# jeuneS2/csolve

Measured on AMD Instinct MI355X. Metric: constraint propagations/sec + nodes/sec, queens-N, 1/2/4/8 MI355X, higher is better.
Workload: dtype int32

## Files before the change

csolve_amd/_lib.py:

```python
from __future__ import annotations

import ctypes as C
import os
import re

_HERE = os.path.dirname(os.path.abspath(__file__))
LIB_PATH = os.environ.get("CSOLVE_HIP_LIB") or os.path.join(_HERE, "libcsolve_hip.so")
HEADER_PATH = os.path.join(os.path.dirname(_HERE), "include", "csolve_gpu.h")


class CsolveError(RuntimeError):
    def __init__(self, code: int, message: str):
        super().__init__(f"csolve_gpu error {code}: {message}")
        self.code = code


class Val(C.Structure):
    _fields_ = [("lo", C.c_int32), ("hi", C.c_int32)]


class Node(C.Structure):
    _fields_ = [("var", C.c_int32), ("lo", C.c_int32), ("hi", C.c_int32), ("parent", C.c_int32)]


class SearchStats(C.Structure):
    _fields_ = [("nodes", C.c_uint64), ("cuts", C.c_uint64), ("props", C.c_uint64), ("revisions", C.c_uint64),
                ("solutions", C.c_uint64), ("iterations", C.c_uint64), ("restarts", C.c_uint64), ("pool", C.c_int64), ("pool_peak", C.c_int64),
                ("best", C.c_int32), ("done", C.c_int32)]


SHARD_SOLUTION_FN = C.CFUNCTYPE(None, C.c_void_p, C.c_int, C.POINTER(C.c_int32), C.c_int64, C.c_int32)


class ShardOptions(C.Structure):
    _fields_ = [("slice_iterations", C.c_int64), ("poll_iterations", C.c_int64), ("seed_states_per_rank", C.c_int64),
                ("low_water", C.c_int64), ("time_limit", C.c_double), ("on_solution", SHARD_SOLUTION_FN),
                ("user", C.c_void_p)]


class Result(C.Structure):
    _fields_ = [("status", C.c_int32), ("props", C.c_int32), ("revisions", C.c_int32), ("rounds", C.c_int32)]


MANY_DONE, MANY_LIMIT, MANY_BAD_ROOT = 0, 1, 2


class ManyResult(C.Structure):
    _fields_ = [("status", C.c_int32), ("root_props", C.c_int32), ("nodes", C.c_int64), ("cuts", C.c_int64),
                ("props", C.c_int64), ("solutions", C.c_int64)]


class ManyOptions(C.Structure):
    _fields_ = [("objective", C.c_int32), ("reserved", C.c_int32), ("max_nodes", C.c_int64)]


def declared_symbols(header: str = HEADER_PATH):
    text = re.sub(r"/\*.*?\*/", "", open(header).read(), flags=re.S)
    return sorted(set(re.findall(r"\b(csgpu_\w+)\s*\(", text)))


PLAN_FAMILIES = ("events", "traced", "rounds", "lds", "bitset", "regs0", "regs1", "regs2", "regs3", "packed",
                 "shave", "shave_trace", "server", "step_shave", "step_packed", "step_import")

_lib = None
_demangler = None


def demangle(symbol: str) -> str:
    global _demangler
    if _demangler is None:
        cxx = C.CDLL("libstdc++.so.6")
        cxx.__cxa_demangle.argtypes = [C.c_char_p, C.c_void_p, C.c_void_p, C.POINTER(C.c_int)]
        cxx.__cxa_demangle.restype = C.c_void_p
        libc = C.CDLL(None)
        libc.free.argtypes = [C.c_void_p]
        _demangler = (cxx.__cxa_demangle, libc.free)
    fn, free = _demangler
    status = C.c_int()
    p = fn(symbol.encode(), None, None, C.byref(status))
    if status.value != 0 or not p:
        raise ValueError(f"cannot demangle {symbol!r}")
    try:
        text = C.string_at(p).decode()
    finally:
        free(p)
    if text.startswith("void "):
        text = text[5:]
    depth = 0
    for i, ch in enumerate(text):
        depth += ch == "<"
        depth -= ch == ">"
        if ch == "(" and depth == 0:
            return text[:i]
    return text


def load_library():
    global _lib
    if _lib is not None:
        return _lib
    if not os.path.exists(LIB_PATH):
        raise ImportError(
            f"{LIB_PATH} is missing: build it with `python -c 'import __graft_entry__ as g; g.build()'` "
            "or `make -C csolve_amd/csrc` (hipcc --offload-arch=gfx950). There is no CPU fallback.")
    try:
        import torch
    except ImportError:
        pass
    L = C.CDLL(LIB_PATH)
    vp, i32, i64 = C.c_void_p, C.c_int32, C.c_int64
    L.csgpu_last_error.restype = C.c_char_p
    L.csgpu_device_count.restype = C.c_int
    L.csgpu_set_device.argtypes = [C.c_int]
    L.csgpu_model_from_text.argtypes = [C.c_char_p, C.c_int, C.POINTER(vp)]
    L.csgpu_model_from_file.argtypes = [C.c_char_p, C.c_int, C.POINTER(vp)]
    L.csgpu_model_from_dump.argtypes = [C.c_char_p, C.POINTER(vp)]
    L.csgpu_model_free.argtypes = [vp]
    L.csgpu_model_free.restype = None
    for f in ("csgpu_model_num_vars", "csgpu_model_num_clauses", "csgpu_model_objective",
              "csgpu_model_objective_var"):
        getattr(L, f).argtypes = [vp]
    L.csgpu_model_var_name.argtypes = [vp, C.c_int]
    L.csgpu_model_var_name.restype = C.c_char_p
    L.csgpu_model_get_domains.argtypes = [vp, vp]
    L.csgpu_model_set_domains.argtypes = [vp, vp]
    L.csgpu_model_device_info.argtypes = [vp, C.POINTER(i64)]
    L.csgpu_model_root_propagate.argtypes = [vp, C.POINTER(i32)]
    L.csgpu_model_finalize.argtypes = [vp]
    L.csgpu_model_normalize.argtypes = [vp]
    L.csgpu_model_specialize.argtypes = [vp, vp, C.POINTER(vp)]
    L.csgpu_model_build_tables.argtypes = [vp]
    L.csgpu_model_eval_clauses_host.argtypes = [vp, vp]
    L.csgpu_model_set_kernel.argtypes = [vp, C.c_int]
    L.csgpu_model_qualifies.argtypes = [vp, C.c_int]
    L.csgpu_set_linear_fast_paths.argtypes = [C.c_int]
    L.csgpu_sets_pack.argtypes = [vp, vp, vp, i64, vp]
    L.csgpu_sets_unpack.argtypes = [vp, vp, vp, i64, vp]
    L.csgpu_propagate_batch_sets.argtypes = [vp, vp, vp, vp, vp, i64, vp]
    L.csgpu_set_linear_fast_paths.restype = None
    L.csgpu_model_get_kernel.argtypes = [vp]
    L.csgpu_propagate_batch.argtypes = [vp, vp, vp, vp, vp, i64, vp]
    L.csgpu_propagate_batch_obj.argtypes = [vp, vp, vp, vp, vp, i64, i32, i32, vp]
    L.csgpu_model_forbidden_words.argtypes = [vp]
    L.csgpu_propagate_batch_fb.argtypes = [vp, vp, vp, vp, vp, vp, vp, i64, vp]
    L.csgpu_eval_batch.argtypes = [vp, vp, vp, i64, vp]
    L.csgpu_eval_clauses.argtypes = [vp, vp, vp, vp]
    L.csgpu_search_create.argtypes = [vp, i64, i64, C.POINTER(vp)]
    L.csgpu_search_free.argtypes = [vp]
    L.csgpu_search_free.restype = None
    L.csgpu_search_reset.argtypes = [vp]
    L.csgpu_search_put.argtypes = [vp, vp, i64]
    L.csgpu_search_put_host.argtypes = [vp, vp, i64]
    L.csgpu_search_take.argtypes = [vp, vp, i64, C.POINTER(i64)]
    L.csgpu_search_take_host.argtypes = [vp, vp, i64, C.POINTER(i64)]
    L.csgpu_plan_transfers.argtypes = [vp, C.c_int, i64, i64, vp, C.POINTER(C.c_int)]
    L.csgpu_shard_region_size.argtypes = [C.c_int, C.c_int, i64, C.POINTER(C.c_size_t)]
    L.csgpu_shard_region_init.argtypes = [vp, C.c_size_t, C.c_int, C.c_int, i64]
    L.csgpu_shard_barrier.argtypes = [vp]
    L.csgpu_text_num_vars.argtypes = [C.c_char_p, C.c_int, C.POINTER(C.c_int)]
    L.csgpu_shard_default_options.argtypes = [C.POINTER(ShardOptions)]
    L.csgpu_shard_default_options.restype = None
    L.csgpu_shard_run.argtypes = [vp, vp, C.c_int, vp, C.POINTER(ShardOptions), C.POINTER(SearchStats),
                                  C.POINTER(SearchStats)]
    L.csgpu_search_set_best.argtypes = [vp, i32]
    L.csgpu_model_add_conflict.argtypes = [vp, i32, vp, vp]
    L.csgpu_search_put_cost.argtypes = [vp, C.POINTER(C.c_double), C.POINTER(i64)]
    L.csgpu_objective_better.argtypes = [C.c_int, Val, i32]
    L.csgpu_objective_bound.argtypes = [C.c_int, Val, i32]
    L.csgpu_objective_bound.restype = Val
    L.csgpu_objective_best.argtypes = [C.c_int, Val, i32]
    L.csgpu_objective_best.restype = i32
    L.csgpu_luby_next.argtypes = [C.POINTER(C.c_uint64), C.POINTER(C.c_uint64)]
    L.csgpu_luby_next.restype = None
    L.csgpu_step_check.argtypes = [Val, C.c_uint32]
    L.csgpu_step_val.argtypes = [Val, C.c_uint32, C.c_uint32]
    L.csgpu_step_val.restype = i32
    L.csgpu_search_share_incumbent.argtypes = [vp, vp]
    L.csgpu_search_set_parents.argtypes = [vp, i64]
    L.csgpu_search_set_restart.argtypes = [vp, i64]
    L.csgpu_search_run.argtypes = [vp, i64, C.POINTER(SearchStats)]
    L.csgpu_search_solutions.argtypes = [vp, vp, i64]
    L.csgpu_search_best_solution.argtypes = [vp, vp]
    L.csgpu_search_solutions.restype = i64
    L.csgpu_search_set_solution_stream.argtypes = [vp, i64]
    L.csgpu_search_drain_solutions.argtypes = [vp, vp, i64, C.POINTER(i64)]
    L.csgpu_search_drain_solutions_device.argtypes = [vp, vp, i64, C.POINTER(i64), vp]
    L.csgpu_search_pending_solutions.argtypes = [vp, C.POINTER(i64), C.POINTER(i64)]
    L.csgpu_propagate_one.argtypes = [vp, vp, Node, vp, C.POINTER(Result)]
    L.csgpu_propagate_one_traced.argtypes = [vp, vp, Node, vp, C.POINTER(Result), vp, i32, C.POINTER(i32)]
    L.csgpu_propagate_one_causes.argtypes = [vp, vp, Node, vp, C.POINTER(Result), vp, i32, C.POINTER(i32)]
    L.csgpu_propagate_values.argtypes = [vp, vp, i32, vp, i32, vp, vp]
    L.csgpu_model_root_propagate_limit.argtypes = [vp, i64, C.POINTER(i32), C.POINTER(i32)]
    L.csgpu_propagate_one_chain.argtypes = [vp, vp, Node, C.POINTER(i32), C.POINTER(i32), vp, i32, C.POINTER(i32)]
    L.csgpu_search_set_strategy.argtypes = [vp, C.c_int, C.c_int]
    L.csgpu_search_set_restart_on_improvement.argtypes = [vp, C.c_int]
    L.csgpu_internal_plan_symbol.argtypes = [vp, C.c_int, C.c_char_p, C.c_size_t]
    L.csgpu_solve_many.argtypes = [vp, vp, i64, C.POINTER(ManyOptions), vp, vp, vp]
    L.csgpu_internal_many_symbol.argtypes = [vp, C.c_char_p, C.c_size_t]
    L.csgpu_internal_many_waves.argtypes = [vp, i64]
    L.csgpu_internal_many_waves.restype = i64
    L.csgpu_debug_one_timing.argtypes = [vp, C.POINTER(C.c_double), C.POINTER(C.c_uint64), C.POINTER(C.c_uint64)]
    _lib = L
    return L


def check(rc: int):
    if rc < 0:
        raise CsolveError(rc, load_library().csgpu_last_error().decode())
    return rc
```

csolve_amd/csrc/cs_capi.hip:

```cpp
#include <hip/hip_runtime.h>
#include <chrono>

#include <dlfcn.h>
#include <stdarg.h>
#include <stdio.h>
#include <stdlib.h>
#include <string.h>

#include <mutex>

#include "../../include/csolve_gpu.h"
#include "cs_kernels.hip.h"
#include "cs_shave.hip.h"
#include "cs_step.hip.h"
#include "cs_dive.hip.h"
#include "cs_chain.hip.h"
#include "cs_internal.h"

static thread_local char g_err[512] = "";

static int set_err(int code, const char *fmt, ...) {
  va_list ap;
  va_start(ap, fmt);
  vsnprintf(g_err, sizeof g_err, fmt, ap);
  va_end(ap);
  return code;
}

extern "C" int csgpu_internal_set_error(int code, const char *msg) { return set_err(code, "%s", msg); }

#define HIP_TRY(expr)                                                          \
  do {                                                                         \
    hipError_t e_ = (expr);                                                    \
    if (e_ != hipSuccess)                                                      \
      return set_err(CSGPU_E_HIP, "%s: %s", #expr, hipGetErrorString(e_));     \
  } while (0)

#define CS_TICKET_SLOTS 1024
#define CS_TICKET_STREAMS 64
#define CS_TICKET_SLOT_WORDS (CS_SHAVE_SHARDS * CS_SHAVE_TICKET_STRIDE)

#define CS_CU_LDS (160u * 1024u)

struct cs_planned {
  const void *fn;
  size_t lds;
  int waves;
  int per_cu;
};

struct cs_kernel_plan {
  cs_planned events, traced;
  cs_planned rounds;
  int rounds_cpl;
  cs_planned lds;
  cs_planned bitset;
  cs_planned regs[4];
  cs_planned packed;
  int packed_nodes;
  cs_planned shave, shave_trace;
  cs_planned server;
  cs_planned step_shave, step_packed, step_import;
  cs_planned dive;
  int full;
  int step_kind;
  int max_width;
};

struct csgpu_model {
  cs_model *host;
  int from_dump;
  int not_root;
  int finalized;
  cs_dev_image *img;
  int *d_adj_off, *d_adj, *d_clause, *d_tree_off, *d_tnode, *d_tkid, *d_tree_want, *d_lit, *d_clause_by_kind;
  cs_tables tab;
  size_t slice;
  int has_tree_adj;
  int packed_bias;
  int packed_nw;
  int kernel_choice;
  cs_kernel_plan plan;
  void *d_adj_packed;
  int lds_adj_global;
  int k2_csz;
  int shave_static;
  int step_chunk_max;
  size_t k1_tab_bytes;
  int fb_words;
  size_t dense_bytes;
  void *d_dense_tab;
  void *d_packed_tab;
  int *d_root_lo;
  int *d_root_hi;
  void *d_many_stack;
  int64_t many_stack_waves;
  unsigned *d_many_tickets;
  int *d_sym_off;
  void *d_sym_packed;
  int n_cus;
  unsigned *d_tickets;
  int ticket_slots, ticket_streams, ticket_reserved;
  void *ticket_stream[CS_TICKET_STREAMS];
  unsigned char *h_one;
  int *d_adj_clause;
  int32_t *h_trace;
  unsigned *h_trace_n;
  int trace_cap;
  cs_val *d_one_in, *d_one_out;
  cs_node_in *d_one_node;
  cs_node_out *d_one_res;
  int engines;
  int chain_state;
  cs_chain_clause *d_chain_cl;
  int *d_chain_off, *d_chain_list;
  cs_chain_frame *d_chain_frames;
  int *h_chain_out;
  unsigned char *h_box;
  size_t box_state_off, box_out_off, box_trace_off;
  hipStream_t srv_stream;
  unsigned srv_seq;
  int srv_off, srv_launched;
  double srv_seconds[4];
  uint64_t srv_calls, srv_starts;
  unsigned char *h_values, *d_values;
  size_t values_cap;
};

extern "C" const char *csgpu_last_error(void) { return g_err; }

static int wait_null_stream(void) {
  for (;;) {
    const hipError_t e = hipStreamQuery(NULL);
    if (e == hipSuccess) return CSGPU_OK;
    if (e != hipErrorNotReady) return set_err(CSGPU_E_HIP, "hipStreamQuery: %s", hipGetErrorString(e));
  }
}

extern "C" int csgpu_device_count(void) {
  int n = 0;
  hipError_t e = hipGetDeviceCount(&n);
  if (e != hipSuccess) return set_err(CSGPU_E_HIP, "hipGetDeviceCount: %s", hipGetErrorString(e));
  return n;
}

extern "C" int csgpu_set_device(int device) {
  HIP_TRY(hipSetDevice(device));
  return CSGPU_OK;
}


static int objective_sense(int objective) { return objective == CS_OBJ_MIN ? 1 : (objective == CS_OBJ_MAX ? 2 : 0); }

extern "C" int csgpu_objective_better(int objective, csgpu_val value, int32_t best) {
  return cs_objective_better(objective_sense(objective), cs_interval(value.lo, value.hi), best);
}
extern "C" csgpu_val csgpu_objective_bound(int objective, csgpu_val value, int32_t best) {
  const cs_val v = cs_objective_bound(objective_sense(objective), cs_interval(value.lo, value.hi), best);
  csgpu_val out;
  out.lo = v.lo;
  out.hi = v.hi;
  return out;
}
extern "C" int32_t csgpu_objective_best(int objective, csgpu_val value, int32_t best) {
  return cs_objective_best(objective_sense(objective), cs_interval(value.lo, value.hi), best);
}
extern "C" void csgpu_luby_next(uint64_t *threshold, uint64_t *counter) {
  if (threshold != NULL && counter != NULL) cs_luby_next(threshold, counter);
}
extern "C" int csgpu_step_check(csgpu_val bounds, uint32_t iter) {
  return cs_step_check(cs_interval(bounds.lo, bounds.hi), iter);
}
extern "C" uint64_t csgpu_branch_key(int order, int prefer_failing, csgpu_val value, int64_t prio, int32_t index) {
  return cs_branch_key_of(order, prefer_failing, cs_interval(value.lo, value.hi), prio, index);
}
extern "C" int32_t csgpu_step_val(csgpu_val bounds, uint32_t iter, uint32_t seed) {
  return cs_step_val(cs_interval(bounds.lo, bounds.hi), iter, seed);
}


static int wrap_model(cs_model *host, int from_dump, csgpu_model **out) {
  csgpu_model *m = (csgpu_model *)calloc(1, sizeof *m);
  if (m == NULL) { cs_model_free(host); return set_err(CSGPU_E_ARG, "out of memory"); }
  m->host = host;
  m->from_dump = from_dump;
  *out = m;
  return CSGPU_OK;
}

extern "C" int csgpu_model_from_text(const char *text, int weights_on, csgpu_model **out) {
  if (text == NULL || out == NULL) return set_err(CSGPU_E_ARG, "null argument");
  char err[256];
  cs_model *host = cs_model_parse(text, weights_on, err, sizeof err);
  if (host == NULL) return set_err(CSGPU_E_PARSE, "%s", err);
  return wrap_model(host, 0, out);
}

extern "C" int csgpu_model_from_file(const char *path, int weights_on, csgpu_model **out) {
  if (path == NULL || out == NULL) return set_err(CSGPU_E_ARG, "null argument");
  FILE *f = fopen(path, "rb");
  if (f == NULL) return set_err(CSGPU_E_ARG, "%s: cannot open", path);
  fseek(f, 0, SEEK_END);
  long len = ftell(f);
  fseek(f, 0, SEEK_SET);
  char *text = (char *)malloc((size_t)len + 1);
  size_t got = fread(text, 1, (size_t)len, f);
  fclose(f);
  text[got] = '\0';
  int rc = csgpu_model_from_text(text, weights_on, out);
  free(text);
  return rc;
}

extern "C" int csgpu_model_from_dump(const char *path, csgpu_model **out) {
  if (path == NULL || out == NULL) return set_err(CSGPU_E_ARG, "null argument");
  char err[256];
  cs_model *host = cs_model_load(path, err, sizeof err);
  if (host == NULL) return set_err(CSGPU_E_ARG, "%s", err);
  if (host->clause_node == NULL) {
    cs_model_free(host);
    return set_err(CSGPU_E_ARG, "%s: model file has no clause index", path);
  }
  return wrap_model(host, 1, out);
}

extern "C" int csgpu_model_from_host(cs_model *host, int lists_final, int domains_are_root, csgpu_model **out) {
  if (host == NULL || out == NULL) return set_err(CSGPU_E_ARG, "null argument");
  int rc = wrap_model(host, lists_final, out);
  if (rc == CSGPU_OK) (*out)->not_root = !domains_are_root;
  return rc;
}

extern "C" cs_model *csgpu_model_host(csgpu_model *m) { return m ? m->host : NULL; }

static void server_stop(csgpu_model *m);
static void server_reap(csgpu_model *m);
static csgpu_model *g_srv_models[16];
static void quiesce_servers(void) {
  for (int i = 0; i < 16; i++)
    if (g_srv_models[i] != NULL) server_stop(g_srv_models[i]);
}

static void free_device(csgpu_model *m) {
  (void)hipFree(m->d_chain_cl); (void)hipFree(m->d_chain_off); (void)hipFree(m->d_chain_list); (void)hipFree(m->d_chain_frames);
  if (m->h_chain_out != NULL) (void)hipHostFree(m->h_chain_out);
  m->d_chain_cl = NULL; m->d_chain_off = NULL; m->d_chain_list = NULL; m->d_chain_frames = NULL; m->h_chain_out = NULL;
  m->chain_state = 0;
  quiesce_servers();
  for (int i = 0; i < 16; i++)
    if (g_srv_models[i] == m) g_srv_models[i] = NULL;
  if (m->h_box != NULL) (void)hipHostFree(m->h_box);
  m->h_box = NULL;
  if (m->srv_stream != NULL) (void)hipStreamDestroy(m->srv_stream);
  m->srv_stream = NULL;
  m->srv_off = 0;
  (void)hipFree(m->d_adj_off); (void)hipFree(m->d_adj); (void)hipFree(m->d_clause); (void)hipFree(m->d_clause_by_kind);
  (void)hipFree(m->d_tree_off); (void)hipFree(m->d_tnode); (void)hipFree(m->d_tkid); (void)hipFree(m->d_tree_want);
  (void)hipFree(m->d_lit);
  m->d_tree_want = NULL;
  m->d_lit = NULL;
  (void)hipFree(m->d_adj_packed);
  (void)hipFree(m->d_root_lo);
  (void)hipFree(m->d_root_hi);
  (void)hipFree(m->d_many_stack);
  (void)hipFree(m->d_many_tickets);
  m->d_root_hi = NULL;
  m->d_many_stack = NULL;
  m->d_many_tickets = NULL;
  m->many_stack_waves = 0;
  (void)hipFree(m->d_sym_off);
  (void)hipFree(m->d_sym_packed);
  (void)hipFree(m->d_dense_tab);
  (void)hipFree(m->d_packed_tab);
  m->d_packed_tab = NULL;
  (void)hipFree(m->d_tickets);
  m->d_tickets = NULL;
  m->ticket_slots = m->ticket_streams = m->ticket_reserved = 0;
  m->d_sym_off = NULL;
  m->d_sym_packed = NULL;
  m->d_dense_tab = NULL;
  m->d_adj_packed = NULL;
  m->d_root_lo = NULL;
  memset(&m->plan, 0, sizeof m->plan);
  m->fb_words = 0;
  (void)hipHostFree(m->h_one);
  m->h_one = NULL;
  (void)hipFree(m->d_adj_clause);
  m->d_adj_clause = NULL;
  if (m->h_trace != NULL) (void)hipHostFree(m->h_trace);
  m->h_trace = NULL;
  m->h_trace_n = NULL;
  m->trace_cap = 0;
  if (m->h_values != NULL) (void)hipHostFree(m->h_values);
  m->h_values = m->d_values = NULL;
  m->values_cap = 0;
  m->d_adj_off = m->d_adj = m->d_clause = m->d_tree_off = m->d_tnode = m->d_tkid = m->d_clause_by_kind = NULL;
  m->d_one_in = m->d_one_out = NULL;
  m->d_one_node = NULL;
  m->d_one_res = NULL;
  cs_dev_image_free(m->img);
  m->img = NULL;
}

extern "C" void csgpu_model_free(csgpu_model *m) {
  if (m == NULL) return;
  free_device(m);
  cs_model_free(m->host);
  free(m);
}

extern "C" int csgpu_model_num_vars(const csgpu_model *m) { return m ? m->host->n_vars : CSGPU_E_ARG; }
extern "C" int csgpu_model_num_clauses(const csgpu_model *m) {
  if (m == NULL) return CSGPU_E_ARG;
  if (m->host->clause_node == NULL && m->host->root >= 0 && cs_model_index(m->host) != 0) return CSGPU_E_ARG;
  return m->host->n_clauses;
}
extern "C" int csgpu_model_objective(const csgpu_model *m) { return m ? m->host->objective : CSGPU_E_ARG; }
extern "C" int csgpu_model_objective_var(const csgpu_model *m) { return m ? m->host->obj_var : CSGPU_E_ARG; }

extern "C" const char *csgpu_model_var_name(const csgpu_model *m, int var) {
  if (m == NULL || var < 0 || var >= m->host->n_vars) return NULL;
  return m->host->names[var];
}

extern "C" int csgpu_model_get_domains(const csgpu_model *m, csgpu_val *out) {
  if (m == NULL || out == NULL) return set_err(CSGPU_E_ARG, "null argument");
  memcpy(out, m->host->dom, (size_t)m->host->n_vars * sizeof(cs_val));
  return CSGPU_OK;
}

extern "C" int csgpu_model_set_domains(csgpu_model *m, const csgpu_val *in) {
  if (m == NULL || in == NULL) return set_err(CSGPU_E_ARG, "null argument");
  memcpy(m->host->dom, in, (size_t)m->host->n_vars * sizeof(cs_val));
  return CSGPU_OK;
}

extern "C" void csgpu_set_linear_fast_paths(int on) { cs_dev_linear_fast_paths = on != 0; }

extern "C" int csgpu_model_device_info(const csgpu_model *m, int64_t info[8]) {
  if (m == NULL || info == NULL) return set_err(CSGPU_E_ARG, "null argument");
  if (m->img == NULL) return set_err(CSGPU_E_STATE, "device tables are not built");
  info[0] = m->img->n_adj;
  info[1] = m->img->n_ne;
  info[2] = m->img->n_tree_clauses;
  info[3] = m->img->n_tnodes;
  info[4] = (int64_t)m->slice;
  info[5] = m->img->max_list;
  info[6] = m->img->n_skip;
  info[7] = m->img->max_tree;
  return CSGPU_OK;
}


struct dev_tables_owner {
  int *adj_off, *adj, *clause, *tree_off, *tnode, *tkid, *tree_want, *lit, *clause_by_kind;
};

static int upload(const void *src, size_t bytes, int **dst) {
  HIP_TRY(hipMalloc((void **)dst, bytes ? bytes : 16));
  if (bytes) HIP_TRY(hipMemcpy(*dst, src, bytes, hipMemcpyHostToDevice));
  return CSGPU_OK;
}

static int upload_image(const cs_dev_image *g, dev_tables_owner *o, cs_tables *t) {
  int rc;
  memset(o, 0, sizeof *o);
  if ((rc = upload(g->adj_off, ((size_t)g->n_vars + 1) * 4, &o->adj_off))) return rc;
  if ((rc = upload(g->adj, (size_t)(g->n_adj ? g->n_adj : 1) * 8, &o->adj))) return rc;
  if ((rc = upload(g->clause, (size_t)(g->n_clauses ? g->n_clauses : 1) * 16, &o->clause))) return rc;
  {
    const int32_t nc = g->n_clauses;
    int32_t *sorted = (int32_t *)malloc((size_t)(nc ? nc : 1) * 16);
    if (sorted == NULL) return set_err(CSGPU_E_LIMIT, "out of memory");
    static const int order[] = { CS_CL_EQ, CS_CL_LT, CS_CL_NE, CS_CL_OR2, CS_CL_TREE, CS_CL_SKIP };
    int32_t k = 0;
    for (size_t q = 0; q < sizeof order / sizeof order[0]; q++)
      for (int32_t c = 0; c < nc; c++)
        if (g->clause[4 * c] == order[q]) { memcpy(sorted + 4 * k, g->clause + 4 * c, 16); k++; }
    rc = k == nc ? upload(sorted, (size_t)(nc ? nc : 1) * 16, &o->clause_by_kind) : set_err(CSGPU_E_STATE, "clause of unknown kind");
    free(sorted);
    if (rc) return rc;
  }
  if ((rc = upload(g->tree_off, ((size_t)g->n_trees + 1) * 4, &o->tree_off))) return rc;
  if ((rc = upload(g->tnode, (size_t)(g->n_tnodes ? g->n_tnodes : 1) * 16, &o->tnode))) return rc;
  if ((rc = upload(g->tkid, (size_t)(g->n_tkids ? g->n_tkids : 1) * 4, &o->tkid))) return rc;
  if ((rc = upload(g->tree_want, (size_t)(g->n_trees ? g->n_trees : 1) * 8, &o->tree_want))) return rc;
  if ((rc = upload(g->lit, (size_t)(g->n_lits ? g->n_lits : 1) * 16, &o->lit))) return rc;
  t->n_vars = g->n_vars;
  t->n_clauses = g->n_clauses;
  t->n_words = (g->n_vars + 31) / 32;
  t->adj_off = o->adj_off;
  t->adj = (const int2 *)o->adj;
  t->clause = (const int4 *)o->clause;
  t->clause_by_kind = (const int4 *)o->clause_by_kind;
  t->tree_off = o->tree_off;
  t->tnode = (const int4 *)o->tnode;
  t->tkid = o->tkid;
  t->tree_want = (const int2 *)o->tree_want;
  t->lit = (const int4 *)o->lit;
  t->n_lits = g->n_lits;
  t->obj_var = -1;
  t->obj_lo = CS_DOM_MIN;
  t->obj_hi = CS_DOM_MAX;
  t->obj_best_dev = NULL;
  t->obj_sense = 0;
  return CSGPU_OK;
}

static void free_tables(dev_tables_owner *o) {
  (void)hipFree(o->adj_off); (void)hipFree(o->adj); (void)hipFree(o->clause); (void)hipFree(o->clause_by_kind);
  (void)hipFree(o->tree_off); (void)hipFree(o->tnode); (void)hipFree(o->tkid); (void)hipFree(o->tree_want);
  (void)hipFree(o->lit);
}

static int lds_limit(size_t bytes, const void *func) {
  if (bytes > CS_CU_LDS) return set_err(CSGPU_E_LIMIT, "%zu bytes of LDS per workgroup exceed the 160 KiB of a CU", bytes);
  if (bytes > 48u * 1024u)
    HIP_TRY(hipFuncSetAttribute(func, hipFuncAttributeMaxDynamicSharedMemorySize, (int)bytes));
  return CSGPU_OK;
}


extern "C" int csgpu_model_root_propagate(csgpu_model *m, int32_t *status) {
  return csgpu_model_root_propagate_limit(m, -1, status, NULL);
}

extern "C" int csgpu_model_root_propagate_limit(csgpu_model *m, int64_t limit, int32_t *status, int32_t *rounds) {
  if (m == NULL || status == NULL) return set_err(CSGPU_E_ARG, "null argument");
  quiesce_servers();
  cs_model *h = m->host;
  if (h->root < 0) return set_err(CSGPU_E_STATE, "model has no root");
  if (!m->from_dump && cs_model_index(h) != 0) return set_err(CSGPU_E_ARG, "%s", h->err);
  char err[200];
  cs_dev_image *g = cs_dev_image_build(h, 0, NULL, err, sizeof err);
  if (g == NULL) return set_err(CSGPU_E_LIMIT, "%s", err);

  dev_tables_owner own;
  cs_tables tab;
  int rc = upload_image(g, &own, &tab);
  cs_val *d_in = NULL, *d_out = NULL;
  cs_node_out *d_res = NULL;
  int *d_conv = NULL, conv = 1;
  cs_node_out res;
  const size_t nbytes = (size_t)(h->n_vars ? h->n_vars : 1) * sizeof(cs_val);
  const size_t lds = (size_t)h->n_vars * sizeof(cs_val) + 4 * sizeof(unsigned);
  hipError_t e = hipSuccess;
  if (rc == CSGPU_OK) rc = lds_limit(lds, (const void *)cs_propagate_sweeps);
  if (rc == CSGPU_OK) {
    if ((e = hipMalloc((void **)&d_in, nbytes)) != hipSuccess || (e = hipMalloc((void **)&d_out, nbytes)) != hipSuccess ||
        (e = hipMalloc((void **)&d_res, sizeof res)) != hipSuccess || (e = hipMalloc((void **)&d_conv, sizeof(int))) != hipSuccess ||
        (e = hipMemcpy(d_in, h->dom, (size_t)h->n_vars * sizeof(cs_val), hipMemcpyHostToDevice)) != hipSuccess)
      rc = set_err(CSGPU_E_HIP, "root propagate setup: %s", hipGetErrorString(e));
  }
  if (rc == CSGPU_OK) {
    const int max_rounds = limit < 0 || limit >= 0x7ffffffe ? 0x7fffffff : (int)limit + 1;
    hipLaunchKernelGGL(cs_propagate_sweeps, dim3(1), dim3(CS_BLOCK), lds, 0, tab, d_in, d_out, d_res, max_rounds, 0, d_conv);
    if ((e = hipGetLastError()) != hipSuccess || (e = hipDeviceSynchronize()) != hipSuccess ||
        (e = hipMemcpy(&res, d_res, sizeof res, hipMemcpyDeviceToHost)) != hipSuccess ||
        (e = hipMemcpy(&conv, d_conv, sizeof conv, hipMemcpyDeviceToHost)) != hipSuccess)
      rc = set_err(CSGPU_E_HIP, "root propagate: %s", hipGetErrorString(e));
    if (rc == CSGPU_OK && res.status >= 0 && !conv) {
      hipLaunchKernelGGL(cs_propagate_sweeps, dim3(1), dim3(CS_BLOCK), lds, 0, tab, d_in, d_out, d_res, max_rounds, 1, d_conv);
      if ((e = hipGetLastError()) != hipSuccess || (e = hipDeviceSynchronize()) != hipSuccess ||
          (e = hipMemcpy(&res, d_res, sizeof res, hipMemcpyDeviceToHost)) != hipSuccess)
        rc = set_err(CSGPU_E_HIP, "root propagate (sequential sweeps): %s", hipGetErrorString(e));
    }
    if (rc == CSGPU_OK && (e = hipMemcpy(h->dom, d_out, (size_t)h->n_vars * sizeof(cs_val), hipMemcpyDeviceToHost)) != hipSuccess)
      rc = set_err(CSGPU_E_HIP, "root propagate: %s", hipGetErrorString(e));
    if (rc != CSGPU_OK) {  }
    else {
      *status = res.status < 0 ? -1 : res.props;
      if (rounds != NULL) *rounds = res.rounds;
    }
  }
  (void)hipFree(d_in); (void)hipFree(d_out); (void)hipFree(d_res); (void)hipFree(d_conv);
  free_tables(&own);
  cs_dev_image_free(g);
  return rc;
}

extern "C" int csgpu_model_normalize(csgpu_model *m) {
  if (m == NULL) return set_err(CSGPU_E_ARG, "null argument");
  if (m->from_dump) return set_err(CSGPU_E_STATE, "a dumped model is already normalised");
  if (m->finalized) return set_err(CSGPU_E_STATE, "model is already finalized");
  if (cs_model_normalize(m->host) < 0) return set_err(CSGPU_E_STATE, "model has no root");
  return CSGPU_OK;
}

extern "C" int csgpu_model_specialize(const csgpu_model *m, const csgpu_val *state, csgpu_model **out) {
  if (m == NULL || state == NULL || out == NULL) return set_err(CSGPU_E_ARG, "null argument");
  const cs_model *h = m->host;
  if (h->root < 0) return set_err(CSGPU_E_STATE, "model has no root");
  for (int32_t v = 0; v < h->n_vars; v++) {
    if (state[v].lo > state[v].hi) return set_err(CSGPU_E_ARG, "variable %d: empty interval", v);
    if (state[v].lo < h->dom[v].lo || state[v].hi > h->dom[v].hi)
      return set_err(CSGPU_E_ARG, "variable %d: [%d, %d] is not inside the model's [%d, %d]", v, state[v].lo, state[v].hi,
                     h->dom[v].lo, h->dom[v].hi);
  }
  cs_model *copy = cs_model_clone(h);
  if (copy == NULL) return set_err(CSGPU_E_LIMIT, "out of memory");
  memcpy(copy->dom, state, (size_t)h->n_vars * sizeof(cs_val));
  return wrap_model(copy, 0, out);
// ... 341 lines not shown
    if (m->img->adj[2 * i] < 0 && m->img->adj[2 * i + 1] == 0) { m->has_tree_adj = 1; break; }
  const size_t tb = ((((size_t)h->n_vars + 1) * 4 + 15) & ~(size_t)15) + (((size_t)m->img->n_adj * 8 + 15) & ~(size_t)15) +
                    (((size_t)m->img->n_lits * 16 + 15) & ~(size_t)15);
  m->k1_tab_bytes = (tb <= 32u * 1024u && m->img->n_adj > 0) ? tb : 0;
  const void *k1 = m->has_tree_adj ? (m->k1_tab_bytes ? (const void *)cs_propagate_events<true, true>
                                                      : (const void *)cs_propagate_events<true, false>)
                                   : (m->k1_tab_bytes ? (const void *)cs_propagate_events<false, true>
                                                      : (const void *)cs_propagate_events<false, false>);
  int rc;
  if ((rc = plan_kernel(&m->plan.events, k1, m->slice * CS_WAVES_PER_BLOCK + m->k1_tab_bytes, CS_WAVES_PER_BLOCK)))
    return rc;
  if (m->plan.events.per_cu < 1) m->plan.events.per_cu = 1;
  if ((rc = lds_limit((size_t)h->n_vars * sizeof(cs_val) + 16, (const void *)cs_eval_root))) return rc;
  if ((rc = lds_limit((size_t)h->n_vars * sizeof(cs_val) + 16, (const void *)cs_eval_clauses))) return rc;
  if ((rc = plan_kernel(&m->plan.traced, (const void *)cs_propagate_events<true, false, true>, m->slice * CS_WAVES_PER_BLOCK,
                        CS_WAVES_PER_BLOCK)))
    return rc;
  const int per = (m->img->n_clauses + CS_WAVE - 1) / CS_WAVE;
  m->plan.rounds_cpl = m->img->n_clauses <= 0 || per > 8 ? 0 : (per <= 1 ? 1 : (per <= 2 ? 2 : (per <= 4 ? 4 : 8)));
  if (m->plan.rounds_cpl) {
#define CS_PICK6(CPL)                                                                              \
  m->plan.rounds.fn = m->has_tree_adj ? (const void *)cs_propagate_clause_rounds<CPL, true>         \
                                      : (const void *)cs_propagate_clause_rounds<CPL, false>
    switch (m->plan.rounds_cpl) {
    case 1: CS_PICK6(1); break;
    case 2: CS_PICK6(2); break;
    case 4: CS_PICK6(4); break;
    default: CS_PICK6(8); break;
    }
#undef CS_PICK6
    m->plan.rounds.lds = ((((size_t)h->n_vars * sizeof(cs_val) + 16 + 15) & ~(size_t)15)) * CS_WAVES_PER_BLOCK;
    m->plan.rounds.waves = CS_WAVES_PER_BLOCK;
    m->plan.rounds.per_cu = 8;
  }
  m->plan.max_width = 2;
  for (int32_t v = 0; v < h->n_vars; v++) {
    const int64_t w = (int64_t)h->dom[v].hi - (int64_t)h->dom[v].lo + 1;
    if (w > m->plan.max_width) m->plan.max_width = w > 0x7fffffff ? 0x7fffffff : (int)w;
  }
  return CSGPU_OK;
}

static int plan_lds_resident(csgpu_model *m) {
  const cs_model *h = m->host;
  if (m->img->packed_width == 0) return CSGPU_OK;
  const size_t off_bytes = (((size_t)h->n_vars * 2 * sizeof(int)) + 15) & ~(size_t)15;
  const size_t adj_bytes = (((size_t)m->img->n_adj * (size_t)m->img->packed_width) + 15) & ~(size_t)15;
  const size_t lds_slice = ((size_t)h->n_vars * sizeof(cs_val) + (2 * (size_t)m->tab.n_words + 1) * sizeof(unsigned) + 15) & ~(size_t)15;
  m->lds_adj_global = 0;
  int waves_max = 16, waves = 0;
  size_t bytes = 0;
  { const char *e = getenv("CSGPU_K2_WAVES"); if (e != NULL && atoi(e) >= 4 && atoi(e) <= 16) waves_max = atoi(e); }
  for (int w = waves_max; w >= 4; w--) {
    const size_t need = off_bytes + adj_bytes + (size_t)w * lds_slice;
    if (need <= CS_CU_LDS) {
      waves = w;
      bytes = need;
      break;
    }
  }
  const char *force = getenv("CSGPU_K2_ADJ");
  const int want_global = force != NULL && force[0] == 'g';
  if (want_global && 8 * lds_slice <= CS_CU_LDS) {
    m->lds_adj_global = 1;
    waves = 8;
    bytes = 8 * lds_slice;
  }
  { const char *e = getenv("CSGPU_K2_CSZ"); m->k2_csz = e != NULL && atoi(e) >= 1 && atoi(e) <= CS_CHUNK ? atoi(e) : 0; }
  if (!waves) return CSGPU_OK;
  int rc;
  if ((rc = upload(m->img->adj_packed, (size_t)m->img->n_adj * (size_t)m->img->packed_width, (int **)&m->d_adj_packed)))
    return rc;
  if ((rc = plan_kernel(&m->plan.lds, ne_lds_kernel(m->img->packed_width, h->n_vars, m->lds_adj_global), bytes, waves)))
    return rc;
  if (m->plan.lds.per_cu < 1) m->plan.lds.per_cu = 1;
  return CSGPU_OK;
}

static int plan_forbidden_sets(csgpu_model *m) {
  const cs_model *h = m->host;
  if (m->img->sym_width == 0 || m->not_root) return CSGPU_OK;
  int64_t width = 1;
  for (int32_t v = 0; v < h->n_vars; v++) {
    const int64_t w = (int64_t)h->dom[v].hi - (int64_t)h->dom[v].lo + 1;
    if (w > width) width = w;
  }
  const int fw = width <= 64 ? 1 : (width <= 128 ? 2 : (width <= 256 ? 4 : 0));
  if (!fw) return CSGPU_OK;
  const size_t off_bytes = (((size_t)h->n_vars * 2 * sizeof(int)) + 15) & ~(size_t)15;
  const size_t base_bytes = (((size_t)h->n_vars * sizeof(int)) + 15) & ~(size_t)15;
  const size_t adj_bytes = (((size_t)m->img->sym_n_adj * (size_t)m->img->sym_width) + 15) & ~(size_t)15;
  const size_t sl = ((size_t)h->n_vars * sizeof(cs_val) + (size_t)h->n_vars * fw * 8 +
                     (2 * (size_t)m->tab.n_words + 2) * sizeof(unsigned) + 15) & ~(size_t)15;
  int waves = 16;
  for (; waves >= 1; waves--)
    if (off_bytes + base_bytes + adj_bytes + (size_t)waves * sl <= CS_CU_LDS) break;
  if (waves < 1) return CSGPU_OK;
  m->fb_words = fw;
  int *lo = (int *)malloc((size_t)(h->n_vars ? h->n_vars : 1) * sizeof(int));
  for (int32_t v = 0; v < h->n_vars; v++) lo[v] = h->dom[v].lo;
  int rc = upload(lo, (size_t)h->n_vars * sizeof(int), &m->d_root_lo);
  free(lo);
  if (rc) return rc;
  if ((rc = upload(m->img->sym_off, ((size_t)h->n_vars + 1) * sizeof(int), &m->d_sym_off))) return rc;
  if ((rc = upload(m->img->sym_packed, (size_t)m->img->sym_n_adj * (size_t)m->img->sym_width, (int **)&m->d_sym_packed)))
    return rc;
  if ((rc = plan_kernel(&m->plan.bitset, ne_bitset_kernel(m->img->sym_width, fw, h->n_vars),
                        off_bytes + base_bytes + adj_bytes + (size_t)waves * sl, waves)))
    return rc;
  if (m->plan.bitset.per_cu < 1) m->plan.bitset.per_cu = 1;
  return CSGPU_OK;
}

static int plan_dense_table(csgpu_model *m) {
  const cs_model *h = m->host;
  if (!m->fb_words || m->img->dense_width == 0) return CSGPU_OK;
  const int n = h->n_vars, width = m->img->dense_width, slots = m->img->dense_slots;
  const size_t bytes = (size_t)n * slots * m->img->dense_cols * width;
  int best = 0, waves = 0;
  for (int w = 4; w <= 16; w <<= 1)
    if (resident_per_cu(bytes, w) * w > best) { best = resident_per_cu(bytes, w) * w; waves = w; }
  if (!waves) return CSGPU_OK;
  m->dense_bytes = bytes;
  int rc;
  if ((rc = upload(m->img->dense_tab, bytes, (int **)&m->d_dense_tab))) return rc;
  for (int variant = 0; variant < 4; variant++)
    if ((rc = plan_kernel(&m->plan.regs[variant], ne_regs_kernel(width, m->fb_words, n, variant & 1, variant >> 1), bytes, waves)))
      return rc;
  m->plan.full = n == cs_dense_strides(n) * CS_WAVE;
  if ((rc = plan_kernel(&m->plan.shave, ne_shave_kernel(width, n, slots, m->plan.full), bytes, waves))) return rc;
  const size_t table = (bytes + 15) & ~(size_t)15;
  if (table + (size_t)waves * 32 <= CS_CU_LDS &&
      (rc = plan_kernel(&m->plan.step_shave, step_shave_kernel(width, n, slots, m->plan.full), table + (size_t)waves * 32, waves)))
    return rc;
  if (table + CS_SHAVE_TRACE_LDS * 16 <= CS_CU_LDS) {
    if ((rc = plan_kernel(&m->plan.shave_trace, ne_shave_trace_kernel(width, n, slots), table + CS_SHAVE_TRACE_LDS * 16, waves)))
      return rc;
    m->plan.server = m->plan.shave_trace;
    m->plan.server.fn = shave_server_kernel(width, n, slots);
  }
  if ((rc = plan_kernel(&m->plan.dive, dive_kernel(width, n), table, waves))) return rc;
  {
    int *hi = (int *)malloc((size_t)n * sizeof(int));
    if (hi == NULL) return set_err(CSGPU_E_ARG, "out of memory");
    for (int32_t v = 0; v < n; v++) hi[v] = h->dom[v].hi;
    rc = upload(hi, (size_t)n * sizeof(int), &m->d_root_hi);
    free(hi);
    if (rc) return rc;
  }
  HIP_TRY(hipMalloc((void **)&m->d_tickets, (size_t)CS_TICKET_SLOTS * CS_TICKET_SLOT_WORDS * sizeof(unsigned)));
  HIP_TRY(hipMemset(m->d_tickets, 0, (size_t)CS_TICKET_SLOTS * CS_TICKET_SLOT_WORDS * sizeof(unsigned)));
  m->ticket_slots = CS_TICKET_SLOTS;
  m->shave_static = getenv("CSGPU_SHAVE_STATIC") != NULL;
  return CSGPU_OK;
}

static int plan_packed(csgpu_model *m) {
  const cs_model *h = m->host;
  if (m->plan.shave.fn == NULL) return CSGPU_OK;
  const int n = h->n_vars, s3 = m->img->dense_slots == 3;
  m->packed_nw = 1;
  for (int32_t v = 0; v < n; v++)
    if ((int64_t)h->dom[v].hi - (int64_t)h->dom[v].lo + 1 > 32) m->packed_nw = 2;
  m->packed_bias = 0;
  for (int32_t v = 0; v < n; v++)
    if (h->dom[v].lo - m->img->dense_dmin > m->packed_bias) m->packed_bias = h->dom[v].lo - m->img->dense_dmin;
  m->plan.packed_nodes = packed_nodes_per_wave(m->fb_words, n, m->img->dense_width);
  if (!m->plan.packed_nodes) return CSGPU_OK;
  const size_t bytes = m->dense_bytes;
  int rc;
  if ((rc = plan_kernel(&m->plan.packed, ne_packed_kernel(n, m->packed_nw, s3), 2 * bytes, m->plan.regs[0].waves))) return rc;
  m->plan.packed.per_cu = m->plan.regs[0].per_cu;
  const size_t per_row = (size_t)m->img->dense_slots * m->img->dense_cols, total = (size_t)n * per_row;
  uint16_t *rel = (uint16_t *)malloc(total * sizeof(uint16_t));
  const uint8_t *src = (const uint8_t *)m->img->dense_tab;
  for (size_t i = 0; i < total; i++) {
    const int32_t u = (int32_t)(i / per_row);
    rel[i] = src[i] == 0xffu ? (uint16_t)0xffffu : (uint16_t)((int)src[i] - (h->dom[u].lo - m->img->dense_dmin) + m->packed_bias);
  }
  rc = upload(rel, total * sizeof(uint16_t), (int **)&m->d_packed_tab);
  free(rel);
  if (rc) return rc;
  if (step_packed_lds(m, 16) <= 80u * 1024u &&
      ((rc = plan_kernel(&m->plan.step_packed, step_packed_kernel(n, m->packed_nw, s3), step_packed_lds(m, 16), 16)) ||
       (rc = plan_kernel(&m->plan.step_import, step_import_kernel(n, m->packed_nw, s3), (2 * bytes + 15) & ~(size_t)15, 4))))
    return rc;
  m->step_chunk_max = 128;
  { const char *e = getenv("CSGPU_STEP_CHUNK_MAX"); if (e != NULL && atoi(e) > 0) m->step_chunk_max = atoi(e); }
  return CSGPU_OK;
}

static int stage_single_node(csgpu_model *m) {
  int dev = 0;
  hipDeviceProp_t prop;
  HIP_TRY(hipGetDevice(&dev));
  HIP_TRY(hipGetDeviceProperties(&prop, dev));
  m->n_cus = prop.multiProcessorCount;
  const size_t nbytes = (size_t)(m->host->n_vars ? m->host->n_vars : 1) * sizeof(cs_val);
  const size_t part = (nbytes + 63) & ~(size_t)63;
  unsigned char *d = NULL;
  HIP_TRY(hipHostMalloc((void **)&m->h_one, 2 * part + 128, hipHostMallocMapped));
  HIP_TRY(hipHostGetDevicePointer((void **)&d, m->h_one, 0));
  m->d_one_in = (cs_val *)d;
  m->d_one_node = (cs_node_in *)(d + part);
  m->d_one_res = (cs_node_out *)(d + part + 64);
  m->d_one_out = (cs_val *)(d + part + 128);
  return CSGPU_OK;
}

extern "C" int csgpu_model_finalize(csgpu_model *m) {
  if (m == NULL) return set_err(CSGPU_E_ARG, "null argument");
  free_device(m);
  int rc;
  if ((rc = csgpu_model_build_tables(m)) || (rc = drop_entailed_clauses(m)) || (rc = plan_general(m)) ||
      (rc = plan_lds_resident(m)) || (rc = plan_forbidden_sets(m)) || (rc = plan_dense_table(m)) || (rc = plan_packed(m)) ||
      (rc = stage_single_node(m)))
    return rc;
  m->plan.step_kind = m->plan.step_packed.fn != NULL ? 1
                      : (m->plan.step_shave.fn != NULL && m->host->n_vars <= 256 && m->plan.max_width <= 256 ? 2 : 0);
  m->finalized = 1;
  return CSGPU_OK;
}

static int kernel_qualifies(const csgpu_model *m, int which) {
  if (!m->finalized) return 0;
  switch (which) {
  case 1: return 1;
  case 2: return m->plan.lds.fn != NULL;
  case 3: return m->plan.bitset.fn != NULL;
  case 4: return m->plan.regs[0].fn != NULL;
  case 5: return m->plan.packed.fn != NULL;
  case 6: return m->plan.rounds.fn != NULL;
  case 7: return m->plan.shave.fn != NULL;
  default: return 0;
  }
}

extern "C" int csgpu_model_set_kernel(csgpu_model *m, int which) {
  static const char *const kernel_name[8] = {
    NULL, NULL, "the LDS-resident kernel", "the forbidden-set kernel", "the register-resident forbidden-set kernel",
    "the several-nodes-per-wave kernel (at most 32 variables, 64 values)", "the clause-resident kernel (at most 512 clauses)",
    "the interval-only shaving kernel (dense pair table in LDS)" };
  if (m == NULL || which < 0 || which > 7) return set_err(CSGPU_E_ARG, "bad argument");
  if (which >= 2) {
    if (!m->finalized) return set_err(CSGPU_E_STATE, "model is not finalized");
    if (!kernel_qualifies(m, which)) return set_err(CSGPU_E_LIMIT, "model does not qualify for %s", kernel_name[which]);
  }
  m->kernel_choice = which;
  return CSGPU_OK;
}

extern "C" int csgpu_model_qualifies(const csgpu_model *m, int which) { return m != NULL && kernel_qualifies(m, which); }

extern "C" int csgpu_internal_plan_symbol(const csgpu_model *m, int family, char *buf, size_t len) {
  if (m == NULL || buf == NULL || len == 0) return set_err(CSGPU_E_ARG, "null argument");
  if (!m->finalized) return set_err(CSGPU_E_STATE, "model is not finalized");
  const cs_kernel_plan *p = &m->plan;
  const cs_planned *fam[] = { &p->events, &p->traced, &p->rounds, &p->lds, &p->bitset, &p->regs[0], &p->regs[1],
                              &p->regs[2], &p->regs[3], &p->packed, &p->shave, &p->shave_trace, &p->server,
                              &p->step_shave, &p->step_packed, &p->step_import };
  if (family < 0 || family >= (int)(sizeof fam / sizeof fam[0])) return set_err(CSGPU_E_ARG, "no plan family %d", family);
  buf[0] = '\0';
  const void *fn = fam[family]->fn;
  if (fn == NULL) return CSGPU_OK;
  Dl_info info;
  if (dladdr(fn, &info) == 0 || info.dli_sname == NULL || info.dli_saddr != fn)
    return set_err(CSGPU_E_STATE, "plan family %d: the kernel handle has no dynamic symbol", family);
  if (strlen(info.dli_sname) >= len) return set_err(CSGPU_E_LIMIT, "plan family %d: symbol longer than the buffer", family);
  strcpy(buf, info.dli_sname);
  return CSGPU_OK;
}

extern "C" int csgpu_internal_many_symbol(const csgpu_model *m, char *buf, size_t len) {
  if (m == NULL || buf == NULL || len == 0) return set_err(CSGPU_E_ARG, "null argument");
  if (!m->finalized) return set_err(CSGPU_E_STATE, "model is not finalized");
  buf[0] = '\0';
  const void *fn = m->plan.dive.fn;
  if (fn == NULL) return CSGPU_OK;
  Dl_info info;
  if (dladdr(fn, &info) == 0 || info.dli_sname == NULL || info.dli_saddr != fn)
    return set_err(CSGPU_E_STATE, "cs_dive_shave: the kernel handle has no dynamic symbol");
  if (strlen(info.dli_sname) >= len) return set_err(CSGPU_E_LIMIT, "cs_dive_shave: symbol longer than the buffer");
  strcpy(buf, info.dli_sname);
  return CSGPU_OK;
}

extern "C" void csgpu_internal_engine_ref(const csgpu_model *m, int delta) {
  if (m != NULL) const_cast<csgpu_model *>(m)->engines += delta;
}

extern "C" const int32_t *csgpu_internal_root_lo(const csgpu_model *m) {
  return m != NULL && m->finalized && m->fb_words ? m->d_root_lo : NULL;
}

extern "C" int csgpu_model_forbidden_words(const csgpu_model *m) { return m && m->finalized ? m->fb_words : 0; }

extern "C" int csgpu_internal_step_kind(const csgpu_model *m) { return m == NULL || !m->finalized ? 0 : m->plan.step_kind; }

static int64_t step_shave_waves(const csgpu_model *m, int64_t stage_rows) {
  const cs_planned *k = &m->plan.step_shave;
  int64_t waves = (int64_t)m->n_cus * (int64_t)k->per_cu * k->waves;
  const int64_t by_stage = stage_rows / (4 * (int64_t)m->plan.max_width);
  if (waves > by_stage) waves = by_stage / k->waves * k->waves;
  return waves;
}

// ... 67 lines not shown
  const int64_t by_stage = L->stage_rows / (2 * (int64_t)G * maxw);
  if (waves > by_stage) waves = by_stage;
  const int64_t by_parents = ((int64_t)L->parents + G - 1) / G;
  if (waves > by_parents) waves = by_parents;
  if (waves < 1) return set_err(CSGPU_E_LIMIT, "step kernel: staging buffer too small");
  int wg_waves = 16;
  while (wg_waves > waves) wg_waves >>= 1;
  const int64_t grid = waves / wg_waves;
  waves = grid * wg_waves;
  const int64_t K = L->stage_rows / waves;
  int64_t chunk = (int64_t)L->parents / (waves * 8);
  if (chunk > m->step_chunk_max) chunk = m->step_chunk_max;
  if (chunk * maxw > K / 2) chunk = K / (2 * maxw);
  chunk = chunk / G * G;
  if (chunk < G) chunk = G;
  cs_step_io io;
  io.pool = (const uint2 *)L->pool;
  io.first_row = (long long)L->first_row;
  io.parents = L->parents;
  io.chunk = (int)chunk;
  io.maxw = maxw;
  io.stage = (uint2 *)L->stage;
  io.K = (int)(K > 0x7fffffff ? 0x7fffffff : K);
  io.fill = L->fill;
  io.wstat = (unsigned long long *)L->wstat;
  io.ticket = L->ticket;
  io.solutions = L->solutions;
  io.stored = (unsigned long long *)L->stored;
  io.max_solutions = (long long)L->max_solutions;
  io.store_open = L->store_open;
  io.stream_on = L->stream != NULL;
  int nn = n, slots = m->img->dense_slots, bias = m->packed_bias;
  const void *tab_d = m->d_packed_tab;
  const int *root_lo_d = m->d_root_lo, *sym_off = m->d_sym_off;
  size_t tab_bytes = 2 * m->dense_bytes;
  void *args[] = { &nn, &tab_d, &slots, &root_lo_d, &sym_off, &bias, &tab_bytes, &io };
  HIP_TRY(hipLaunchKernel(m->plan.step_packed.fn, dim3((unsigned)grid), dim3((unsigned)(wg_waves * CS_WAVE)), args,
                          step_packed_lds(m, wg_waves), (hipStream_t)stream));
  hipLaunchKernelGGL(cs_collect, dim3((unsigned)waves), dim3(256), 0, (hipStream_t)stream, (const unsigned *)L->fill, (int)waves,
                     (const uint2 *)L->stage, io.K, n, (uint2 *)L->pool, (long long)L->first_row, (int)L->parents,
                     (int)chunk, (const unsigned *)L->ticket, (const unsigned long long *)L->wstat,
                     (unsigned long long *)L->out, (const unsigned long long *)L->stored,
                     L->stream, (long long)L->stream_base, (long long)L->stream_limit, (long long)L->stream_cap,
                     (unsigned long long *)L->stream_err);
  HIP_TRY(hipGetLastError());
  return CSGPU_OK;
}

extern "C" int csgpu_internal_step_import(const csgpu_model *m, csgpu_val *d_rows, int64_t first_row, int64_t count,
                                          void *stream) {
  const int kind = csgpu_internal_step_kind(m);
  if (kind == 2) return CSGPU_OK;
  if (kind != 1 || d_rows == NULL || count < 0) return set_err(CSGPU_E_ARG, "bad argument");
  if (count == 0) return CSGPU_OK;
  const cs_planned *k = &m->plan.step_import;
  const int n = m->host->n_vars, G = m->plan.packed_nodes;
  int nn = n, slots = m->img->dense_slots, bias = m->packed_bias;
  const void *tab_d = m->d_packed_tab;
  const int *root_lo_d = m->d_root_lo;
  size_t tab_bytes = 2 * m->dense_bytes;
  long long fr = first_row, cnt = count;
  int64_t grid = (count + (int64_t)G * k->waves - 1) / ((int64_t)G * k->waves);
  if (grid > (int64_t)m->n_cus * 8) grid = (int64_t)m->n_cus * 8;
  void *args[] = { &nn, &tab_d, &slots, &root_lo_d, &bias, &tab_bytes, &d_rows, &fr, &cnt };
  HIP_TRY(hipLaunchKernel(k->fn, dim3((unsigned)grid), dim3((unsigned)(k->waves * CS_WAVE)), args, k->lds, (hipStream_t)stream));
  return CSGPU_OK;
}

extern "C" int csgpu_internal_step_export(const csgpu_model *m, csgpu_val *d_rows, int64_t first_row, int64_t count,
                                          void *stream) {
  const int kind = csgpu_internal_step_kind(m);
  if (kind == 2) return CSGPU_OK;
  if (kind != 1 || d_rows == NULL || count < 0) return set_err(CSGPU_E_ARG, "bad argument");
  if (count == 0) return CSGPU_OK;
  const int n = m->host->n_vars;
  const long long elements = (long long)count * n;
  uint2 *rows = (uint2 *)d_rows + (size_t)first_row * n;
  const unsigned grid = (unsigned)((elements + 255) / 256);
  if (m->packed_nw == 1)
    hipLaunchKernelGGL(cs_step_export<1>, dim3(grid), dim3(256), 0, (hipStream_t)stream, n, (const int *)m->d_root_lo, rows, elements);
  else
    hipLaunchKernelGGL(cs_step_export<2>, dim3(grid), dim3(256), 0, (hipStream_t)stream, n, (const int *)m->d_root_lo, rows, elements);
  HIP_TRY(hipGetLastError());
  return CSGPU_OK;
}

static int launch_regs(const csgpu_model *m, const csgpu_val *d_states_in, const uint64_t *d_forb_in,
                       const csgpu_node *d_nodes, csgpu_val *d_states_out, uint64_t *d_forb_out, csgpu_result *d_results,
                       int64_t batch, const uint64_t *d_batch, int sets_only, int flags, void *stream) {
  int csz = shrink_chunk(CS_CHUNK, batch, (int64_t)m->n_cus * 32);
  int n = m->host->n_vars, slots = m->img->dense_slots, dmin_d = m->img->dense_dmin;
  const void *tab_d = m->d_dense_tab;
  const int *root_lo_d = m->d_root_lo, *sym_off = m->d_sym_off;
  long long nb_d = (long long)batch;
  void *args_d[] = { &n, &tab_d, &slots, &dmin_d, &root_lo_d, &sym_off, &d_states_in, &d_forb_in, &d_nodes,
                     &d_states_out, &d_forb_out, &d_results, &nb_d, &d_batch, &csz, &flags };
  if (!sets_only && m->kernel_choice != 4 && kernel_qualifies(m, 5)) {
    const cs_planned *k = &m->plan.packed;
    const int64_t groups = (batch + m->plan.packed_nodes - 1) / m->plan.packed_nodes;
    int64_t gp = (int64_t)m->n_cus * (int64_t)k->per_cu * 2;
    const int64_t need_gp = (groups + k->waves - 1) / k->waves;
    if (gp > need_gp) gp = need_gp;
    csz = m->packed_bias;
    tab_d = m->d_packed_tab;
    HIP_TRY(hipLaunchKernel(k->fn, dim3((unsigned)gp), dim3((unsigned)(k->waves * CS_WAVE)), args_d, k->lds, (hipStream_t)stream));
    return CSGPU_OK;
  }
  const int fast = m->plan.full && d_forb_in != NULL && d_forb_out != NULL && flags == 0;
  const cs_planned *k = &m->plan.regs[fast | sets_only << 1];
  const int64_t chunks = (batch + csz - 1) / csz;
  int64_t g = (int64_t)m->n_cus * (int64_t)k->per_cu;
  const int64_t need_wg = (chunks + k->waves - 1) / k->waves;
  g *= 2;
  if (g > need_wg) g = need_wg;
  HIP_TRY(hipLaunchKernel(k->fn, dim3((unsigned)g), dim3((unsigned)(k->waves * CS_WAVE)), args_d, k->lds, (hipStream_t)stream));
  return CSGPU_OK;
}

static std::mutex g_ticket_mutex;

static unsigned *ticket_slot(csgpu_model *m, void *stream) {
  if (m->d_tickets == NULL) return NULL;
  std::lock_guard<std::mutex> lock(g_ticket_mutex);
  hipStreamCaptureStatus cap = hipStreamCaptureStatusNone;
  if (stream != NULL && hipStreamIsCapturing((hipStream_t)stream, &cap) != hipSuccess) cap = hipStreamCaptureStatusNone;
  int slot = -1;
  if (cap == hipStreamCaptureStatusActive) {
    if (m->ticket_reserved < m->ticket_slots - CS_TICKET_STREAMS) slot = m->ticket_slots - 1 - m->ticket_reserved++;
  } else {
    for (int i = 0; i < m->ticket_streams; i++)
      if (m->ticket_stream[i] == stream) slot = i;
    if (slot < 0 && m->ticket_streams < CS_TICKET_STREAMS) {
      slot = m->ticket_streams++;
      m->ticket_stream[slot] = stream;
    }
  }
  return slot < 0 ? NULL : m->d_tickets + (size_t)slot * CS_TICKET_SLOT_WORDS;
}

static int launch_shave(const csgpu_model *m, const csgpu_val *d_states_in, const csgpu_node *d_nodes,
                        csgpu_val *d_states_out, csgpu_result *d_results, int64_t batch, const uint64_t *d_batch,
                        void *stream) {
  const cs_planned *k = &m->plan.shave;
  int csz = shrink_chunk(m->host->n_vars <= CS_WAVE ? 2 * CS_SHAVE_CHUNK : CS_SHAVE_CHUNK, batch, 4 * (int64_t)m->n_cus * 32);
  const int64_t chunks = (batch + csz - 1) / csz;
  int64_t g = (int64_t)m->n_cus * (int64_t)k->per_cu;
  const int64_t need_wg = (chunks + k->waves - 1) / k->waves;
  if (g > need_wg) g = need_wg;
  int n = m->host->n_vars, slots = m->img->dense_slots, dmin_d = m->img->dense_dmin;
  const void *tab_d = m->d_dense_tab;
  const int *root_lo_d = m->d_root_lo, *sym_off = m->d_sym_off;
  long long nb_d = (long long)batch;
  unsigned *tickets = m->shave_static ? NULL : ticket_slot((csgpu_model *)m, stream);
  int4 *no_trace = NULL;
  unsigned *no_trace_n = NULL;
  unsigned no_trace_cap = 0u;
  void *args[] = { &n, &tab_d, &slots, &dmin_d, &root_lo_d, &sym_off, &d_states_in, &d_nodes, &d_states_out, &d_results,
                   &nb_d, &d_batch, &csz, &tickets, &no_trace, &no_trace_n, &no_trace_cap };
  HIP_TRY(hipLaunchKernel(k->fn, dim3((unsigned)g), dim3((unsigned)(k->waves * CS_WAVE)), args, k->lds, (hipStream_t)stream));
  return CSGPU_OK;
}


static_assert(sizeof(csgpu_many_result) == sizeof(cs_dive_result) && sizeof(csgpu_many_result) == 40, "csgpu_many_result layout");

extern "C" int64_t csgpu_internal_many_waves(const csgpu_model *m, int64_t count) {
  if (m == NULL || !m->finalized || m->plan.dive.fn == NULL || count < 1) return 0;
  const cs_planned *k = &m->plan.dive;
  int64_t grid = (int64_t)m->n_cus * k->per_cu;
  const int64_t by_count = (count + k->waves - 1) / k->waves;
  if (grid > by_count) grid = by_count;
  return grid * k->waves;
}

extern "C" int csgpu_solve_many(const csgpu_model *m, const csgpu_val *d_roots, int64_t count, const csgpu_many_options *options,
                                csgpu_many_result *d_results, int32_t *d_solutions, void *stream) {
  if (m == NULL || d_roots == NULL || d_results == NULL || options == NULL) return set_err(CSGPU_E_ARG, "null argument");
  if (count < 0) return set_err(CSGPU_E_ARG, "negative instance count");
  if (options->max_nodes <= 0) return set_err(CSGPU_E_ARG, "max_nodes must be positive: every instance has a budget");
  if (options->objective == CS_OBJ_MIN || options->objective == CS_OBJ_MAX)
    return set_err(CSGPU_E_LIMIT, "csgpu_solve_many searches with ANY or ALL: MIN / MAX are not supported");
  if (options->objective != CS_OBJ_ANY && options->objective != CS_OBJ_ALL) return set_err(CSGPU_E_ARG, "no objective %d", options->objective);
  if (!m->finalized) return set_err(CSGPU_E_STATE, "model is not finalized");
  if (m->plan.dive.fn == NULL)
    return set_err(CSGPU_E_LIMIT, "model does not qualify for the interval-only shaving kernel (a pure != network of at most 256 "
                                  "variables whose dense pair table fits LDS), which csgpu_solve_many is built on");
  if (count > 0x7fffffff - CS_DIVE_SHARDS) return set_err(CSGPU_E_LIMIT, "more than 2^31 - 65 instances in one call");
  if (count == 0) return CSGPU_OK;
  csgpu_model *mm = const_cast<csgpu_model *>(m);
  const cs_planned *k = &m->plan.dive;
  const int n = m->host->n_vars;
  const int64_t waves = csgpu_internal_many_waves(m, count);
  const int frames = n;
  if (mm->d_many_tickets == NULL) {
    quiesce_servers();
    HIP_TRY(hipMalloc((void **)&mm->d_many_tickets, (size_t)CS_DIVE_SHARDS * CS_DIVE_TICKET_STRIDE * sizeof(unsigned)));
    HIP_TRY(hipMemset(mm->d_many_tickets, 0, (size_t)CS_DIVE_SHARDS * CS_DIVE_TICKET_STRIDE * sizeof(unsigned)));
  }
  if (mm->many_stack_waves < waves) {
    quiesce_servers();
    if (mm->d_many_stack != NULL) (void)hipFree(mm->d_many_stack);
    mm->d_many_stack = NULL;
    mm->many_stack_waves = 0;
    HIP_TRY(hipMalloc(&mm->d_many_stack, (size_t)waves * (size_t)frames * ((size_t)n + 1) * sizeof(cs_val)));
    mm->many_stack_waves = waves;
  }
  cs_dive_io io;
  io.roots = (const cs_val *)d_roots;
  io.count = (int)count;
  io.all = options->objective == CS_OBJ_ALL;
  io.max_nodes = (long long)options->max_nodes;
  io.results = (cs_dive_result *)d_results;
  io.solutions = d_solutions;
  io.stack = (cs_val *)mm->d_many_stack;
  io.frames = frames;
  io.tickets = mm->d_many_tickets;
  int nn = n, slots = m->img->dense_slots, dmin_d = m->img->dense_dmin;
  const void *tab_d = m->d_dense_tab;
  const int *root_lo_d = m->d_root_lo, *root_hi_d = m->d_root_hi, *sym_off = m->d_sym_off;
  size_t tab_bytes = m->dense_bytes;
  void *args[] = { &nn, &tab_d, &slots, &dmin_d, &root_lo_d, &root_hi_d, &sym_off, &tab_bytes, &io };
  HIP_TRY(hipLaunchKernel(k->fn, dim3((unsigned)(waves / k->waves)), dim3((unsigned)(k->waves * CS_WAVE)), args, k->lds, (hipStream_t)stream));
  return CSGPU_OK;
}

#ifdef CS_SHAVE_TIMELINE
extern "C" int csgpu_debug_shave_timeline(unsigned long long *out, int waves) {
  HIP_TRY(hipDeviceSynchronize());
  HIP_TRY(hipMemcpyFromSymbol(out, HIP_SYMBOL(cs_shave_tl), (size_t)waves * 3 * sizeof(unsigned long long)));
  return CSGPU_OK;
}
#endif

extern "C" int csgpu_propagate_batch_fb(const csgpu_model *m, const csgpu_val *d_states_in, const uint64_t *d_forb_in,
                                        const csgpu_node *d_nodes, csgpu_val *d_states_out, uint64_t *d_forb_out,
                                        csgpu_result *d_results, int64_t batch, void *stream) {
  return csgpu_internal_propagate_fb(m, d_states_in, d_forb_in, d_nodes, d_states_out, d_forb_out, d_results, batch, NULL,
                                     stream);
}

extern "C" int csgpu_internal_propagate_fb(const csgpu_model *m, const csgpu_val *d_states_in, const uint64_t *d_forb_in,
                                           const csgpu_node *d_nodes, csgpu_val *d_states_out, uint64_t *d_forb_out,
                                           csgpu_result *d_results, int64_t batch, const uint64_t *d_batch,
                                           void *stream) {
  if (m == NULL || batch < 0) return set_err(CSGPU_E_ARG, "null argument");
  if (!m->finalized) return set_err(CSGPU_E_STATE, "model is not finalized");
  if (!kernel_qualifies(m, 3)) return set_err(CSGPU_E_LIMIT, "model does not qualify for the forbidden-set kernel");
  if (batch == 0) return CSGPU_OK;
  if (d_states_in == NULL || d_nodes == NULL || d_states_out == NULL || d_results == NULL)
    return set_err(CSGPU_E_ARG, "null argument");
  if (kernel_qualifies(m, 4) && m->kernel_choice != 3)
    return launch_regs(m, d_states_in, d_forb_in, d_nodes, d_states_out, d_forb_out, d_results, batch, d_batch, 0, 0, stream);
  const cs_planned *k = &m->plan.bitset;
  int csz = shrink_chunk(CS_CHUNK, batch, (int64_t)m->n_cus * 32);
  const int64_t chunks = (batch + csz - 1) / csz;
  int64_t grid = (int64_t)m->n_cus * (int64_t)k->per_cu;
  const int64_t need = (chunks + k->waves - 1) / k->waves;
  if (grid > need) grid = need;
  cs_tables tab = m->tab;
  tab.adj_off = m->d_sym_off;
  const void *packed = m->d_sym_packed;
  int n_adj = m->img->sym_n_adj, obits = m->img->sym_obits, dmin = m->img->sym_dmin;
  const int *root_lo = m->d_root_lo;
  long long nb = (long long)batch;
  void *args[] = { &tab, &packed, &n_adj, &obits, &dmin, &root_lo, &d_states_in, &d_forb_in, &d_nodes,
                   &d_states_out, &d_forb_out, &d_results, &nb, &d_batch, &csz };
  HIP_TRY(hipLaunchKernel(k->fn, dim3((unsigned)grid), dim3((unsigned)(k->waves * CS_WAVE)), args, k->lds, (hipStream_t)stream));
  return CSGPU_OK;
}


__global__ void cs_fill_identity_nodes(cs_node_in *nodes, long long count) {
  const long long i = (long long)blockIdx.x * blockDim.x + threadIdx.x;
  if (i < count) {
    cs_node_in nd;
    nd.var = -1; nd.lo = 0; nd.hi = 0; nd.parent = (int)i;
    nodes[i] = nd;
  }
}

static int sets_ready(const csgpu_model *m) {
  if (m == NULL) return set_err(CSGPU_E_ARG, "null argument");
  if (!m->finalized) return set_err(CSGPU_E_STATE, "model is not finalized");
  if (!kernel_qualifies(m, 4)) return set_err(CSGPU_E_LIMIT, "model does not qualify for the register-resident forbidden-set kernel");
  return CSGPU_OK;
}

extern "C" int csgpu_sets_pack(const csgpu_model *m, const csgpu_val *d_states, uint64_t *d_sets, int64_t count, void *stream) {
  int rc = sets_ready(m);
  if (rc != CSGPU_OK) return rc;
  if (count < 0) return set_err(CSGPU_E_ARG, "bad argument");
  if (count == 0) return CSGPU_OK;
  if (d_states == NULL || d_sets == NULL) return set_err(CSGPU_E_ARG, "null argument");
  if (count > 0x7fffffff) return set_err(CSGPU_E_LIMIT, "too many states");
  cs_node_in *d_nodes = NULL;
  cs_node_out *d_res = NULL;
  HIP_TRY(hipMalloc((void **)&d_nodes, (size_t)count * sizeof(cs_node_in)));
  if (hipMalloc((void **)&d_res, (size_t)count * sizeof(cs_node_out)) != hipSuccess) {
    (void)hipFree(d_nodes);
    return set_err(CSGPU_E_HIP, "out of device memory");
  }
  hipLaunchKernelGGL(cs_fill_identity_nodes, dim3((unsigned)((count + 255) / 256)), dim3(256), 0, (hipStream_t)stream, d_nodes, (long long)count);
  rc = launch_regs(m, d_states, NULL, (const csgpu_node *)d_nodes, NULL, d_sets, (csgpu_result *)d_res, count, NULL, 0,
                   CS_K4_OUT_RESTRICT, stream);
  hipError_t e = hipStreamSynchronize((hipStream_t)stream);
  (void)hipFree(d_nodes);
  (void)hipFree(d_res);
  if (rc != CSGPU_OK) return rc;
  if (e != hipSuccess) return set_err(CSGPU_E_HIP, "%s", hipGetErrorString(e));
  return CSGPU_OK;
}
// ... 160 lines not shown

extern "C" int csgpu_internal_eval_list(const csgpu_model *m, const csgpu_val *d_states, const int32_t *d_list,
                                        const uint64_t *d_count, int64_t bound, int32_t *d_truth, void *stream) {
  if (m == NULL || d_states == NULL || d_list == NULL || d_count == NULL || d_truth == NULL || bound < 0)
    return set_err(CSGPU_E_ARG, "null argument");
  if (!m->finalized) return set_err(CSGPU_E_STATE, "model is not finalized");
  if (bound == 0) return CSGPU_OK;
  if (bound > 0x7fffffff) return set_err(CSGPU_E_LIMIT, "batch too large");
  return launch_eval_root(m, d_states, d_list, d_count, bound, d_truth, stream);
}

extern "C" int csgpu_eval_clauses(const csgpu_model *m, const csgpu_val *d_state, csgpu_val *d_vals, void *stream) {
  if (m == NULL || d_state == NULL || d_vals == NULL) return set_err(CSGPU_E_ARG, "null argument");
  if (!m->finalized) return set_err(CSGPU_E_STATE, "model is not finalized");
  if (m->host->n_clauses == 0) return CSGPU_OK;
  const size_t lds = (size_t)m->host->n_vars * sizeof(cs_val) + 16;
  unsigned blocks = (unsigned)((m->host->n_clauses + CS_BLOCK - 1) / CS_BLOCK);
  if (blocks > 1024u) blocks = 1024u;
  hipLaunchKernelGGL(cs_eval_clauses, dim3(blocks), dim3(CS_BLOCK), lds, (hipStream_t)stream, m->tab,
                     (const cs_val *)d_state, (cs_val *)d_vals);
  HIP_TRY(hipGetLastError());
  return CSGPU_OK;
}

extern "C" int csgpu_propagate_values(const csgpu_model *cm, const csgpu_val *state, int32_t var, const int32_t *values,
                                      int32_t count, csgpu_val *states_out, csgpu_result *results) {
  csgpu_model *m = (csgpu_model *)cm;
  if (m == NULL || state == NULL || values == NULL || states_out == NULL || results == NULL)
    return set_err(CSGPU_E_ARG, "null argument");
  if (!m->finalized) return set_err(CSGPU_E_STATE, "model is not finalized");
  const int n = m->host->n_vars;
  if (var < 0 || var >= n || count < 0 || count > (1 << 20)) return set_err(CSGPU_E_ARG, "bad argument");
  if (count == 0) return CSGPU_OK;
  const size_t row = (size_t)n * sizeof(cs_val);
  const size_t off_nodes = (row + 255) & ~(size_t)255;
  const size_t off_res = off_nodes + (((size_t)count * sizeof(cs_node_in) + 255) & ~(size_t)255);
  const size_t off_out = off_res + (((size_t)count * sizeof(cs_node_out) + 255) & ~(size_t)255);
  const size_t need = off_out + (size_t)count * row;
  if (need > m->values_cap) {
    if (m->h_values != NULL) (void)hipHostFree(m->h_values);
    m->h_values = NULL;
    m->values_cap = 0;
    HIP_TRY(hipHostMalloc((void **)&m->h_values, need * 2, hipHostMallocMapped));
    HIP_TRY(hipHostGetDevicePointer((void **)&m->d_values, m->h_values, 0));
    m->values_cap = need * 2;
  }
  memcpy(m->h_values, state, row);
  cs_node_in *nd = (cs_node_in *)(m->h_values + off_nodes);
  for (int32_t i = 0; i < count; i++) { nd[i].var = var; nd[i].lo = nd[i].hi = values[i]; nd[i].parent = 0; }
  int rc = csgpu_propagate_batch(m, (const csgpu_val *)m->d_values, (const csgpu_node *)(m->d_values + off_nodes),
                                 (csgpu_val *)(m->d_values + off_out), (csgpu_result *)(m->d_values + off_res), count, NULL);
  if (rc != CSGPU_OK) return rc;
  { const int rcw = wait_null_stream(); if (rcw != CSGPU_OK) return rcw; }
  memcpy(results, m->h_values + off_res, (size_t)count * sizeof *results);
  memcpy(states_out, m->h_values + off_out, (size_t)count * row);
  return CSGPU_OK;
}

extern "C" int csgpu_propagate_one_traced(const csgpu_model *cm, const csgpu_val *state, csgpu_node node,
                                          csgpu_val *state_out, csgpu_result *result, int32_t *trace, int32_t cap,
                                          int32_t *count) {
  csgpu_model *m = const_cast<csgpu_model *>(cm);
  if (m == NULL || state == NULL || state_out == NULL || result == NULL || trace == NULL || cap < 1 || count == NULL)
    return set_err(CSGPU_E_ARG, "bad argument");
  if (!m->finalized) return set_err(CSGPU_E_STATE, "model is not finalized");
  if (m->d_adj_clause == NULL) {
    int rc = upload(m->img->adj_clause, (size_t)(m->img->n_adj ? m->img->n_adj : 1) * 4, &m->d_adj_clause);
    if (rc != CSGPU_OK) return rc;
  }
  if (m->trace_cap < cap) {
    if (m->h_trace != NULL) (void)hipHostFree(m->h_trace);
    m->h_trace = NULL;
    HIP_TRY(hipHostMalloc((void **)&m->h_trace, (size_t)cap * 16 + 16, hipHostMallocMapped));
    m->h_trace_n = (unsigned *)(m->h_trace + (size_t)cap * 4);
    m->trace_cap = cap;
  }
  const size_t nbytes = (size_t)m->host->n_vars * sizeof(cs_val);
  const size_t part = (nbytes + 63) & ~(size_t)63;
  node.parent = 0;
  memcpy(m->h_one, state, nbytes);
  memcpy(m->h_one + part, &node, sizeof node);
  *m->h_trace_n = 0u;
  cs_tables tab = m->tab;
  tab.adj_clause = m->d_adj_clause;
  void *dev = NULL;
  HIP_TRY(hipHostGetDevicePointer(&dev, m->h_trace, 0));
  tab.trace_log = (int4 *)dev;
  tab.trace_n = (unsigned *)((int32_t *)dev + (size_t)m->trace_cap * 4);
  tab.trace_cap = (unsigned)cap;
  const cs_val *in = m->d_one_in;
  const cs_node_in *nd = m->d_one_node;
  cs_val *out = m->d_one_out;
  cs_node_out *res = m->d_one_res;
  long long one = 1;
  const unsigned long long *no_count = NULL;
  void *args[] = { &tab, &in, &nd, &out, &res, &one, &no_count };
  HIP_TRY(hipLaunchKernel(m->plan.traced.fn, dim3(1), dim3(CS_BLOCK), args, m->plan.traced.lds, (hipStream_t)NULL));
  { const int rcw = wait_null_stream(); if (rcw != CSGPU_OK) return rcw; }
  memcpy(result, m->h_one + part + 64, sizeof *result);
  if (result->status >= 0) memcpy(state_out, m->h_one + part + 128, nbytes);
  const unsigned n = *m->h_trace_n;
  *count = (int32_t)n;
  memcpy(trace, m->h_trace, (size_t)(n < (unsigned)cap ? n : (unsigned)cap) * 16);
  return CSGPU_OK;
}

static double srv_now(void) {
  return std::chrono::duration<double>(std::chrono::steady_clock::now().time_since_epoch()).count();
}

static cs_mailbox_head *srv_box(const csgpu_model *m) { return (cs_mailbox_head *)m->h_box; }

static int server_usable(csgpu_model *m) {
  if (m->srv_off) return 0;
  if (m->h_box != NULL) return 1;
  const char *e = getenv("CSGPU_SERVER");
  if ((e != NULL && e[0] == '0') || m->plan.server.fn == NULL) { m->srv_off = 1; return 0; }
  const size_t nbytes = ((size_t)m->host->n_vars * sizeof(cs_val) + 63) & ~(size_t)63;
  m->box_state_off = (sizeof(cs_mailbox_head) + 63) & ~(size_t)63;
  m->box_out_off = m->box_state_off + nbytes;
  m->box_trace_off = m->box_out_off + nbytes;
  const size_t total = m->box_trace_off + (size_t)CS_SHAVE_TRACE_LDS * 16;
  if (hipHostMalloc((void **)&m->h_box, total, hipHostMallocMapped | hipHostMallocCoherent) != hipSuccess ||
      hipStreamCreateWithFlags(&m->srv_stream, hipStreamNonBlocking) != hipSuccess ||
      hipFuncSetAttribute(m->plan.server.fn, hipFuncAttributeMaxDynamicSharedMemorySize, (int)m->plan.server.lds) != hipSuccess) {
    (void)hipGetLastError();
    if (m->h_box != NULL) (void)hipHostFree(m->h_box);
    m->h_box = NULL;
    m->srv_off = 1;
    return 0;
  }
  memset(m->h_box, 0, total);
  m->srv_seq = 0;
  for (int i = 0; i < 16; i++)
    if (g_srv_models[i] == NULL) { g_srv_models[i] = m; break; }
  return 1;
}

static int server_start(csgpu_model *m) {
  cs_mailbox_head *box = srv_box(m);
  if (m->srv_launched) server_reap(m);
  void *dev = NULL;
  HIP_TRY(hipHostGetDevicePointer(&dev, m->h_box, 0));
  cs_mailbox_head *d_box = (cs_mailbox_head *)dev;
  unsigned long long *d_in = (unsigned long long *)((unsigned char *)dev + m->box_state_off);
  unsigned long long *d_out = (unsigned long long *)((unsigned char *)dev + m->box_out_off);
  int4 *d_trace = (int4 *)((unsigned char *)dev + m->box_trace_off);
  int n = m->host->n_vars, slots = m->img->dense_slots, dmin_d = m->img->dense_dmin;
  const void *tab_d = m->d_dense_tab;
  const int *root_lo_d = m->d_root_lo, *sym_off = m->d_sym_off;
  unsigned cap = CS_SHAVE_TRACE_LDS;
  unsigned long long idle = 200000ull;
  { const char *e = getenv("CSGPU_SERVER_IDLE_US"); if (e != NULL && atoll(e) > 0) idle = (unsigned long long)atoll(e) * 100ull; }
  void *args[] = { &n, &tab_d, &slots, &dmin_d, &root_lo_d, &sym_off, &d_box, &d_in, &d_out, &d_trace, &cap, &idle };
  const cs_planned *k = &m->plan.server;
  HIP_TRY(hipLaunchKernel(k->fn, dim3(1), dim3((unsigned)(k->waves * CS_WAVE)), args, k->lds, m->srv_stream));
  m->srv_launched = 1;
  m->srv_starts++;
  const double t0 = srv_now();
  while (__atomic_load_n(&box->alive, __ATOMIC_ACQUIRE) == 0u) {
    if (__atomic_load_n(&box->ack_seq, __ATOMIC_ACQUIRE) == m->srv_seq && hipStreamQuery(m->srv_stream) == hipSuccess) break;
    if (srv_now() - t0 > 10.0) return set_err(CSGPU_E_HIP, "the single-node server did not start");
  }
  return CSGPU_OK;
}

static void server_reap(csgpu_model *m) {
  const double t0 = srv_now();
  for (;;) {
    const hipError_t e = hipStreamQuery(m->srv_stream);
    if (e != hipErrorNotReady) break;
    if (srv_now() - t0 > 5.0) { (void)hipStreamSynchronize(m->srv_stream); break; }
  }
}

static void server_stop(csgpu_model *m) {
  if (m->h_box == NULL || !m->srv_launched) return;
  cs_mailbox_head *box = srv_box(m);
  __atomic_store_n(&box->stop, 1u, __ATOMIC_RELEASE);
  server_reap(m);
  __atomic_store_n(&box->stop, 0u, __ATOMIC_RELEASE);
  m->srv_launched = 0;
}

static int server_call(csgpu_model *m, const csgpu_val *state, csgpu_node node, csgpu_val *state_out, csgpu_result *result,
                       int32_t *trace, int32_t cap, int32_t *count) {
  cs_mailbox_head *box = srv_box(m);
  const size_t nbytes = (size_t)m->host->n_vars * sizeof(cs_val);
  const double t0 = srv_now();
  memcpy(m->h_box + m->box_state_off, state, nbytes);
  box->node.var = node.var; box->node.lo = node.lo; box->node.hi = node.hi; box->node.parent = 0;
  box->want_trace = trace != NULL ? 1u : 0u;
  const unsigned seq = ++m->srv_seq;
  const double t1 = srv_now();
  __atomic_store_n(&box->req_seq, seq, __ATOMIC_RELEASE);
  double t_start = 0.0;
  if (__atomic_load_n(&box->alive, __ATOMIC_ACQUIRE) == 0u) {
    const double ts = srv_now();
    const int rc = server_start(m);
    if (rc != CSGPU_OK) return rc;
    t_start = srv_now() - ts;
  }
  unsigned spins = 0;
  while (__atomic_load_n(&box->ack_seq, __ATOMIC_ACQUIRE) != seq) {
    if ((++spins & 0xfffu) == 0u) {
      if (__atomic_load_n(&box->alive, __ATOMIC_ACQUIRE) == 0u && __atomic_load_n(&box->ack_seq, __ATOMIC_ACQUIRE) != seq) {
        const double ts = srv_now();
        const int rc = server_start(m);
        if (rc != CSGPU_OK) return rc;
        t_start += srv_now() - ts;
      }
      if (srv_now() - t1 > 30.0) return set_err(CSGPU_E_HIP, "the single-node server does not answer");
    }
  }
  const double t2 = srv_now();
  result->status = box->result.status; result->props = box->result.props;
  result->revisions = box->result.revisions; result->rounds = box->result.rounds;
  if (result->status >= 0) memcpy(state_out, m->h_box + m->box_out_off, nbytes);
  if (trace != NULL) {
    const unsigned made = box->trace_n;
    *count = (int32_t)made;
    unsigned kept = made < CS_SHAVE_TRACE_LDS ? made : CS_SHAVE_TRACE_LDS;
    if (kept > (unsigned)cap) kept = (unsigned)cap;
    memcpy(trace, m->h_box + m->box_trace_off, (size_t)kept * 16);
  }
  const double t3 = srv_now();
  m->srv_seconds[0] += t1 - t0;
  m->srv_seconds[1] += t2 - t1 - t_start;
  m->srv_seconds[2] += t3 - t2;
  m->srv_seconds[3] += t_start;
  m->srv_calls++;
  return CSGPU_OK;
}

extern "C" int csgpu_internal_server_warm(csgpu_model *m) {
  if (m == NULL || !m->finalized || !server_usable(m)) return CSGPU_OK;
  if (__atomic_load_n(&srv_box(m)->alive, __ATOMIC_ACQUIRE) != 0u) return CSGPU_OK;
  return server_start(m);
}

extern "C" int csgpu_debug_one_timing(const csgpu_model *m, double *seconds, uint64_t *calls, uint64_t *starts) {
  if (m == NULL || seconds == NULL || calls == NULL || starts == NULL) return set_err(CSGPU_E_ARG, "null argument");
  for (int i = 0; i < 4; i++) seconds[i] = m->srv_seconds[i];
  *calls = m->srv_calls;
  *starts = m->srv_starts;
  return CSGPU_OK;
}

extern "C" int csgpu_propagate_one_causes(const csgpu_model *cm, const csgpu_val *state, csgpu_node node,
                                          csgpu_val *state_out, csgpu_result *result, int32_t *trace, int32_t cap,
                                          int32_t *count) {
  csgpu_model *m = const_cast<csgpu_model *>(cm);
  if (m == NULL || state == NULL || state_out == NULL || result == NULL || trace == NULL || cap < 1 || count == NULL)
    return set_err(CSGPU_E_ARG, "bad argument");
  if (!m->finalized) return set_err(CSGPU_E_STATE, "model is not finalized");
  if (!kernel_qualifies(m, 7)) return set_err(CSGPU_E_LIMIT, "model does not qualify for the interval-only shaving kernel");
  if (server_usable(m)) return server_call(m, state, node, state_out, result, trace, cap, count);
  if (m->trace_cap < cap) {
    if (m->h_trace != NULL) (void)hipHostFree(m->h_trace);
    m->h_trace = NULL;
    HIP_TRY(hipHostMalloc((void **)&m->h_trace, (size_t)cap * 16 + 16, hipHostMallocMapped));
    m->h_trace_n = (unsigned *)(m->h_trace + (size_t)cap * 4);
    m->trace_cap = cap;
  }
  const size_t nbytes = (size_t)m->host->n_vars * sizeof(cs_val);
  const size_t part = (nbytes + 63) & ~(size_t)63;
  node.parent = 0;
  const double tl0 = srv_now();
  memcpy(m->h_one, state, nbytes);
  memcpy(m->h_one + part, &node, sizeof node);
  *m->h_trace_n = 0u;
  void *dev = NULL;
  HIP_TRY(hipHostGetDevicePointer(&dev, m->h_trace, 0));
  int4 *d_trace = (int4 *)dev;
  unsigned *d_trace_n = (unsigned *)((int32_t *)dev + (size_t)m->trace_cap * 4);
  unsigned ucap = (unsigned)cap;
  int n = m->host->n_vars, slots = m->img->dense_slots, dmin_d = m->img->dense_dmin, csz = 1;
  const void *tab_d = m->d_dense_tab;
  const int *root_lo_d = m->d_root_lo, *sym_off = m->d_sym_off;
  long long nb_d = 1;
  const uint64_t *d_batch = NULL;
  unsigned *tickets = NULL;
  const csgpu_val *d_in = (const csgpu_val *)m->d_one_in;
  const csgpu_node *d_node = (const csgpu_node *)m->d_one_node;
  csgpu_val *d_out = (csgpu_val *)m->d_one_out;
  csgpu_result *d_res = (csgpu_result *)m->d_one_res;
  void *args[] = { &n, &tab_d, &slots, &dmin_d, &root_lo_d, &sym_off, &d_in, &d_node, &d_out, &d_res,
                   &nb_d, &d_batch, &csz, &tickets, &d_trace, &d_trace_n, &ucap };
  const cs_planned *k = &m->plan.shave_trace;
  if (k->fn == NULL) return set_err(CSGPU_E_LIMIT, "no room in LDS for the trail next to the pair table");
  const double tl1 = srv_now();
  HIP_TRY(hipLaunchKernel(k->fn, dim3(1), dim3((unsigned)(k->waves * CS_WAVE)), args, k->lds, (hipStream_t)NULL));
  const double tl2 = srv_now();
  { const int rcw = wait_null_stream(); if (rcw != CSGPU_OK) return rcw; }
  const double tl3 = srv_now();
  memcpy(result, m->h_one + part + 64, sizeof *result);
  if (result->status >= 0) memcpy(state_out, m->h_one + part + 128, nbytes);
  const unsigned made = *m->h_trace_n;
  *count = (int32_t)made;
  unsigned kept = made < CS_SHAVE_TRACE_LDS ? made : CS_SHAVE_TRACE_LDS;
  if (kept > (unsigned)cap) kept = (unsigned)cap;
  memcpy(trace, m->h_trace, (size_t)kept * 16);
  m->srv_seconds[0] += tl1 - tl0; m->srv_seconds[1] += tl2 - tl1; m->srv_seconds[2] += tl3 - tl2; m->srv_seconds[3] += srv_now() - tl3;
  m->srv_calls++;
  return CSGPU_OK;
}

#define CS_CHAIN_FRAMES (1 << 16)
#define CS_CHAIN_BUMPS 4096

static int chain_operand(const cs_model *h, int32_t node, int *x, int *c) {
  const cs_node *nd = &h->nodes[node];
  if (nd->op == CS_OP_VAR) { *x = nd->a; *c = 0; return 1; }
  if (nd->op == CS_OP_ADD) {
    const cs_node *l = &h->nodes[nd->a], *r = &h->nodes[nd->b];
    if (l->op == CS_OP_VAR && r->op == CS_OP_CONST && r->a == r->b) { *x = l->a | CS_CHAIN_ADD; *c = r->a; return 1; }
  }
  return 0;
}

static int chain_build(csgpu_model *m) {
  if (m->chain_state != 0) return m->chain_state;
  const cs_model *h = m->host;
  m->chain_state = -1;
  if (!m->finalized || h->n_clauses < 1 || h->n_clauses > 60000 || h->n_vars < 1 || h->list_off == NULL) return -1;
  if ((size_t)h->n_vars * sizeof(cs_val) + (size_t)h->n_clauses * 2 + 64 > CS_CU_LDS) return -1;
  cs_chain_clause *cl = (cs_chain_clause *)malloc((size_t)h->n_clauses * sizeof *cl);
  if (cl == NULL) return -1;
  for (int32_t c = 0; c < h->n_clauses; c++) {
    const cs_node *top = &h->nodes[h->clause_node[c]];
    if (top->op == CS_OP_CONST) {
      cl[c].lx = -1; cl[c].lc = 0; cl[c].rx = -1; cl[c].rc = 0;
      continue;
    }
    int ok = top->op == CS_OP_NOT && h->nodes[top->a].op == CS_OP_EQ;
    if (ok) {
      const cs_node *eq = &h->nodes[top->a];
      ok = chain_operand(h, eq->a, &cl[c].lx, &cl[c].lc) && chain_operand(h, eq->b, &cl[c].rx, &cl[c].rc);
    }
    if (!ok) { free(cl); return -1; }
  }
  int rc = upload(cl, (size_t)h->n_clauses * sizeof *cl, (int **)&m->d_chain_cl);
  free(cl);
  if (rc == CSGPU_OK) rc = upload(h->list_off, ((size_t)h->n_vars + 1) * sizeof(int32_t), &m->d_chain_off);
  if (rc == CSGPU_OK) rc = upload(h->list, (size_t)(h->list_off[h->n_vars] ? h->list_off[h->n_vars] : 1) * sizeof(int32_t), &m->d_chain_list);
  if (rc != CSGPU_OK) return -1;
  if (hipMalloc((void **)&m->d_chain_frames, (size_t)CS_CHAIN_FRAMES * sizeof(cs_chain_frame)) != hipSuccess ||
      hipHostMalloc((void **)&m->h_chain_out, (4 + CS_CHAIN_BUMPS) * sizeof(int), hipHostMallocMapped) != hipSuccess ||
      hipFuncSetAttribute((const void *)cs_ne_chain, hipFuncAttributeMaxDynamicSharedMemorySize, (int)CS_CU_LDS) != hipSuccess) {
    (void)hipGetLastError();
    return -1;
  }
  m->chain_state = 1;
  return 1;
}

extern "C" int csgpu_propagate_one_chain(const csgpu_model *cm, const csgpu_val *state, csgpu_node node, int32_t *status,
                                         int32_t *props_out, int32_t *bumps, int32_t cap, int32_t *count) {
  csgpu_model *m = const_cast<csgpu_model *>(cm);
  if (m == NULL || state == NULL || status == NULL || props_out == NULL || bumps == NULL || count == NULL || cap < 0)
    return set_err(CSGPU_E_ARG, "bad argument");
  if (!m->finalized) return set_err(CSGPU_E_STATE, "model is not finalized");
  if (node.var < 0 || node.var >= m->host->n_vars) return set_err(CSGPU_E_ARG, "no such variable");
  if (chain_build(m) != 1)
    return set_err(CSGPU_E_LIMIT, "the model is not a network of NOT(EQ(x [+ c], y [+ d])) clauses: no reference-order walk");
  const size_t nbytes = (size_t)m->host->n_vars * sizeof(cs_val);
  memcpy(m->h_one, state, nbytes);
  void *dev = NULL;
  HIP_TRY(hipHostGetDevicePointer(&dev, m->h_chain_out, 0));
  int *d_out = (int *)dev, *d_bumps = (int *)dev + 4;
  cs_node_in nd;
  nd.var = node.var; nd.lo = node.lo; nd.hi = node.hi; nd.parent = 0;
  const size_t lds = ((nbytes + 15) & ~(size_t)15) + (((size_t)m->host->n_clauses * 2 + 15) & ~(size_t)15);
  hipLaunchKernelGGL(cs_ne_chain, dim3(1), dim3(64), lds, (hipStream_t)NULL, m->host->n_vars, m->host->n_clauses,
                     (const cs_chain_clause *)m->d_chain_cl, (const int *)m->d_chain_off, (const int *)m->d_chain_list,
                     (const cs_val *)m->d_one_in, nd, m->d_chain_frames, (int)CS_CHAIN_FRAMES, d_out, d_bumps, (int)CS_CHAIN_BUMPS);
  HIP_TRY(hipGetLastError());
  { const int rcw = wait_null_stream(); if (rcw != CSGPU_OK) return rcw; }
  if (m->h_chain_out[3] != 0) return set_err(CSGPU_E_LIMIT, "the reference-order walk overflowed its frame stack or its bump list");
  *status = m->h_chain_out[0];
  *props_out = m->h_chain_out[1];
  const int made = m->h_chain_out[2];
  *count = made;
  memcpy(bumps, m->h_chain_out + 4, (size_t)(made < cap ? made : cap) * sizeof(int32_t));
  return CSGPU_OK;
}

extern "C" int csgpu_propagate_one(const csgpu_model *m, const csgpu_val *state, csgpu_node node, csgpu_val *state_out,
                                   csgpu_result *result) {
  if (m == NULL || state == NULL || state_out == NULL || result == NULL) return set_err(CSGPU_E_ARG, "null argument");
  if (!m->finalized) return set_err(CSGPU_E_STATE, "model is not finalized");
  if ((m->kernel_choice == 0 || m->kernel_choice == 7) && kernel_qualifies(m, 7) && server_usable(const_cast<csgpu_model *>(m)))
    return server_call(const_cast<csgpu_model *>(m), state, node, state_out, result, NULL, 0, NULL);
  const size_t nbytes = (size_t)m->host->n_vars * sizeof(cs_val);
  const size_t part = (nbytes + 63) & ~(size_t)63;
  node.parent = 0;
  memcpy(m->h_one, state, nbytes);
  memcpy(m->h_one + part, &node, sizeof node);
  int rc = csgpu_propagate_batch(m, (const csgpu_val *)m->d_one_in, (const csgpu_node *)m->d_one_node,
                                 (csgpu_val *)m->d_one_out, (csgpu_result *)m->d_one_res, 1, NULL);
  if (rc != CSGPU_OK) return rc;
  { const int rcw = wait_null_stream(); if (rcw != CSGPU_OK) return rcw; }
  memcpy(result, m->h_one + part + 64, sizeof *result);
  if (result->status >= 0) memcpy(state_out, m->h_one + part + 128, nbytes);
  return CSGPU_OK;
}
```

csolve_amd/csrc/cs_device.c:

```c
#include "cs_device.h"

#include <stdio.h>
#include <stdlib.h>
#include <string.h>

#define NE_LIMIT (1 << 30)

typedef struct {
  int32_t *v;
  int32_t n, cap;
} ibuf;

static void ibuf_push(ibuf *b, int32_t x) {
  if (b->n == b->cap) {
    b->cap = b->cap ? b->cap * 2 : 256;
    b->v = (int32_t *)realloc(b->v, (size_t)b->cap * sizeof(int32_t));
    if (b->v == NULL) { fprintf(stderr, "csolve_amd: error: out of memory\n"); exit(EXIT_FAILURE); }
  }
  b->v[b->n++] = x;
}

static int small(int64_t x) { return x > -(int64_t)NE_LIMIT && x < (int64_t)NE_LIMIT; }

static int const_value(const cs_model *m, int32_t node, int64_t *c) {
  const cs_node *n = &m->nodes[node];
  if (n->op == CS_OP_CONST && n->a == n->b && small(n->a)) { *c = n->a; return 1; }
  if (n->op == CS_OP_NEG && const_value(m, n->a, c)) { *c = -*c; return 1; }
  return 0;
}

static int affine(const cs_model *m, int32_t node, int32_t *var, int64_t *k) {
  const cs_node *n = &m->nodes[node];
  if (n->op == CS_OP_VAR) {
    cs_val d = m->dom[n->a];
    if (!small(d.lo) || !small(d.hi)) return 0;
    *var = n->a; *k = 0;
    return 1;
  }
  if (n->op == CS_OP_ADD) {
    int64_t c;
    if (const_value(m, n->b, &c) && affine(m, n->a, var, k)) { *k += c; return small(*k); }
    if (const_value(m, n->a, &c) && affine(m, n->b, var, k)) { *k += c; return small(*k); }
  }
  return 0;
}

static int match_ne(const cs_model *m, int32_t root, int32_t *a, int32_t *b, int32_t *d) {
  const cs_node *n = &m->nodes[root];
  if (n->op != CS_OP_NOT) return 0;
  const cs_node *e = &m->nodes[n->a];
  if (e->op != CS_OP_EQ) return 0;
  int64_t ka, kb;
  if (!affine(m, e->a, a, &ka) || !affine(m, e->b, b, &kb) || *a == *b) return 0;
  if (!small(kb - ka)) return 0;
  *d = (int32_t)(kb - ka);
  return 1;
}

int cs_dev_linear_fast_paths = 1;

static int affine_wide(const cs_model *m, int32_t node, int32_t *var, int64_t *k) {
  const cs_node *n = &m->nodes[node];
  if (n->op == CS_OP_VAR) {
    cs_val d = m->dom[n->a];
    if (d.lo == CS_DOM_MIN || d.hi == CS_DOM_MAX) return 0;
    *var = n->a; *k = 0;
    return 1;
  }
  if (n->op == CS_OP_ADD) return affine(m, node, var, k);
  return 0;
}

static int lt_literal(const cs_model *m, int32_t lt_node, int negated, int32_t *a, int32_t *b, int32_t *d) {
  const cs_node *e = &m->nodes[lt_node];
  if (e->op != CS_OP_LT) return 0;
  int32_t va, vb;
  int64_t ka, kb;
  if (!affine_wide(m, e->a, &va, &ka) || !affine_wide(m, e->b, &vb, &kb) || va == vb) return 0;
  const int64_t dd = negated ? ka - kb + 1 : kb - ka;
  if (!small(dd)) return 0;
  if (negated) { *a = vb; *b = va; } else { *a = va; *b = vb; }
  *d = (int32_t)dd;
  return 1;
}

static int match_lt(const cs_model *m, int32_t root, int want_true, int32_t *a, int32_t *b, int32_t *d) {
  const cs_node *n = &m->nodes[root];
  if (n->op == CS_OP_LT) return lt_literal(m, root, !want_true, a, b, d);
  if (n->op == CS_OP_NOT) return lt_literal(m, n->a, want_true, a, b, d);
  return 0;
}

static int match_eq(const cs_model *m, int32_t root, int32_t *a, int32_t *b, int32_t *d) {
  const cs_node *e = &m->nodes[root];
  if (e->op != CS_OP_EQ) return 0;
  int64_t ka, kb;
  if (!affine_wide(m, e->a, a, &ka) || !affine_wide(m, e->b, b, &kb) || *a == *b) return 0;
  if (!small(kb - ka)) return 0;
  *d = (int32_t)(kb - ka);
  return 1;
}

typedef struct {
  const cs_model *m;
  ibuf tnode, tkid;
  int32_t *local;
  ibuf touched;
  int32_t base;
  int bad;
} tree_ctx;

static int32_t emit_tree(tree_ctx *t, int32_t node) {
  if (t->local[node] >= 0) return t->local[node];
  const cs_node *n = &t->m->nodes[node];
  int32_t a = n->a, b = n->b;
  switch (n->op) {
  case CS_OP_VAR: case CS_OP_CONST:
    break;
  case CS_OP_NEG: case CS_OP_NOT:
    a = emit_tree(t, n->a); b = -1;
    break;
  case CS_OP_EQ: case CS_OP_LT: case CS_OP_ADD: case CS_OP_MUL: case CS_OP_AND: case CS_OP_OR:
    a = emit_tree(t, n->a);
    b = emit_tree(t, t->m->nodes[node].b);
    break;
  case CS_OP_WAND: {
    int32_t cnt = n->b, off = n->a;
    int32_t *loc = (int32_t *)malloc((size_t)(cnt ? cnt : 1) * sizeof(int32_t));
    for (int32_t i = 0; i < cnt; i++) loc[i] = emit_tree(t, t->m->kids[off + i]);
    a = t->tkid.n;
    for (int32_t i = 0; i < cnt; i++) ibuf_push(&t->tkid, loc[i]);
    b = cnt;
    free(loc);
    break;
  }
  case CS_OP_CONFL: {
    int32_t cnt = n->b, off = n->a;
    int32_t *loc = (int32_t *)malloc((size_t)(cnt ? cnt : 1) * sizeof(int32_t));
    for (int32_t i = 0; i < cnt; i++) loc[i] = emit_tree(t, t->m->kids[off + 2 * i]);
    a = t->tkid.n;
    for (int32_t i = 0; i < cnt; i++) {
      ibuf_push(&t->tkid, loc[i]);
      ibuf_push(&t->tkid, t->m->kids[off + 2 * i + 1]);
    }
    b = cnt;
    free(loc);
    break;
  }
  default:
    t->bad = 1;
    break;
  }
  int32_t idx = t->tnode.n / 4 - t->base;
  ibuf_push(&t->tnode, t->m->nodes[node].op);
  ibuf_push(&t->tnode, a);
  ibuf_push(&t->tnode, b);
  ibuf_push(&t->tnode, 0);
  t->local[node] = idx;
  ibuf_push(&t->touched, node);
  return idx;
}

void cs_dev_image_free(cs_dev_image *g) {
  if (g == NULL) return;
  free(g->adj_off); free(g->adj); free(g->adj_clause); free(g->clause); free(g->tree_off); free(g->tnode); free(g->tkid); free(g->tree_want); free(g->lit); free(g->adj_packed); free(g->sym_off); free(g->sym_packed); free(g->dense_tab);
  free(g);
}

cs_dev_image *cs_dev_image_build(const cs_model *m, int with_lists, const unsigned char *entailed, char *err,
                                 size_t errlen) {
  if (m->clause_node == NULL || (with_lists && m->list_off == NULL)) {
    if (err) snprintf(err, errlen, "model has no clause index");
    return NULL;
  }
  {
    const char *e = getenv("CSGPU_LINEAR_FAST_PATHS");
    if (e != NULL && e[0] == '0') cs_dev_linear_fast_paths = 0;
  }
  cs_dev_image *g = (cs_dev_image *)calloc(1, sizeof *g);
  g->n_vars = m->n_vars;
  g->n_clauses = m->n_clauses;
  g->clause = (int32_t *)calloc((size_t)(m->n_clauses ? m->n_clauses : 1) * 4, sizeof(int32_t));

  tree_ctx t;
  memset(&t, 0, sizeof t);
  t.m = m;
  t.local = (int32_t *)malloc((size_t)(m->n_nodes ? m->n_nodes : 1) * sizeof(int32_t));
  for (int32_t i = 0; i < m->n_nodes; i++) t.local[i] = -1;
  ibuf tree_off = { 0 };
  ibuf want = { 0 };
  ibuf lits = { 0 };

  for (int32_t c = 0; c < m->n_clauses; c++) {
    int32_t root = m->clause_node[c];
    const cs_node *rn = &m->nodes[root];
    int32_t *rec = &g->clause[4 * c];
    int32_t a, b, d;
    const int want_true = m->clause_want == NULL || (m->clause_want[c].lo == 1 && m->clause_want[c].hi == 1);
    if (want_true && ((entailed != NULL && entailed[c]) || (rn->op == CS_OP_CONST && rn->a == 1 && rn->b == 1))) {
      rec[0] = CS_CL_SKIP;
      g->n_skip++;
    } else if (want_true && match_ne(m, root, &a, &b, &d)) {
      rec[0] = CS_CL_NE; rec[1] = a; rec[2] = b; rec[3] = d;
      g->n_ne++;
    } else if (cs_dev_linear_fast_paths && want_true && match_eq(m, root, &a, &b, &d)) {
      rec[0] = CS_CL_EQ; rec[1] = a; rec[2] = b; rec[3] = d;
      g->n_lin++;
    } else if (cs_dev_linear_fast_paths && (want_true || (m->clause_want[c].lo == 0 && m->clause_want[c].hi == 0)) &&
               match_lt(m, root, want_true, &a, &b, &d)) {
      rec[0] = CS_CL_LT; rec[1] = a; rec[2] = b; rec[3] = d;
      g->n_lin++;
    } else if (cs_dev_linear_fast_paths && want_true && rn->op == CS_OP_OR) {
      int32_t a2, b2, d2;
      if (match_lt(m, rn->a, 1, &a, &b, &d) && match_lt(m, rn->b, 1, &a2, &b2, &d2)) {
        rec[0] = CS_CL_OR2; rec[1] = lits.n / 4;
        ibuf_push(&lits, a); ibuf_push(&lits, b); ibuf_push(&lits, d); ibuf_push(&lits, 0);
        ibuf_push(&lits, a2); ibuf_push(&lits, b2); ibuf_push(&lits, d2); ibuf_push(&lits, 0);
        g->n_or2++;
      } else {
        goto as_tree;
      }
    } else {
    as_tree:
      ibuf_push(&tree_off, t.tnode.n / 4);
      t.base = t.tnode.n / 4;
      t.touched.n = 0;
      emit_tree(&t, root);
      int32_t len = t.tnode.n / 4 - t.base;
      for (int32_t i = 0; i < t.touched.n; i++) t.local[t.touched.v[i]] = -1;
      if (len > g->max_tree) g->max_tree = len;
      rec[0] = CS_CL_TREE; rec[1] = g->n_trees;
      ibuf_push(&want, m->clause_want ? m->clause_want[c].lo : 1);
      ibuf_push(&want, m->clause_want ? m->clause_want[c].hi : 1);
      g->n_trees++;
      g->n_tree_clauses++;
    }
  }
  ibuf_push(&tree_off, t.tnode.n / 4);
  g->tree_off = tree_off.v;
  g->tnode = t.tnode.v ? t.tnode.v : (int32_t *)calloc(4, sizeof(int32_t));
  g->n_tnodes = t.tnode.n / 4;
  g->tkid = t.tkid.v ? t.tkid.v : (int32_t *)calloc(1, sizeof(int32_t));
  g->n_tkids = t.tkid.n;
  g->tree_want = want.v ? want.v : (int32_t *)calloc(2, sizeof(int32_t));
  g->lit = lits.v ? lits.v : (int32_t *)calloc(4, sizeof(int32_t));
  g->n_lits = lits.n / 4;
  free(t.local);
  free(t.touched.v);

  if (t.bad) {
    if (err) snprintf(err, errlen, "constraint type without a device implementation");
    cs_dev_image_free(g);
    return NULL;
  }
  if (g->max_tree > CS_MAX_TREE_NODES) {
    if (err) snprintf(err, errlen, "a clause has %d nodes, device limit is %d", g->max_tree, CS_MAX_TREE_NODES);
    cs_dev_image_free(g);
    return NULL;
  }

  g->adj_off = (int32_t *)calloc((size_t)m->n_vars + 1, sizeof(int32_t));
  if (with_lists) {
    ibuf adj = { 0 };
    ibuf adjc = { 0 };
    for (int32_t v = 0; v < m->n_vars; v++) {
      g->adj_off[v] = adj.n / 2;
      for (int32_t i = m->list_off[v]; i < m->list_off[v + 1]; i++) {
        const int32_t *rec = &g->clause[4 * m->list[i]];
        if (rec[0] != CS_CL_SKIP) ibuf_push(&adjc, m->list[i]);
        if (rec[0] == CS_CL_NE) {
          if (rec[1] == v) { ibuf_push(&adj, rec[2]); ibuf_push(&adj, rec[3]); }
          else { ibuf_push(&adj, rec[1]); ibuf_push(&adj, -rec[3]); }
        } else if (rec[0] == CS_CL_EQ) {
          if (rec[1] == v) { ibuf_push(&adj, rec[2] | (CS_REL_EQ << 28)); ibuf_push(&adj, rec[3]); }
          else { ibuf_push(&adj, rec[1] | (CS_REL_EQ << 28)); ibuf_push(&adj, -rec[3]); }
        } else if (rec[0] == CS_CL_LT) {
          if (rec[1] == v) { ibuf_push(&adj, rec[2] | (CS_REL_LT << 28)); ibuf_push(&adj, rec[3]); }
          else { ibuf_push(&adj, rec[1] | (CS_REL_GT << 28)); ibuf_push(&adj, -rec[3]); }
        } else if (rec[0] == CS_CL_OR2) {
          ibuf_push(&adj, ~rec[1]); ibuf_push(&adj, 1);
        } else if (rec[0] == CS_CL_TREE) {
          ibuf_push(&adj, ~rec[1]); ibuf_push(&adj, 0);
        }
      }
      int32_t len = adj.n / 2 - g->adj_off[v];
      if (len > g->max_list) g->max_list = len;
    }
    g->adj_off[m->n_vars] = adj.n / 2;
    g->n_adj = adj.n / 2;
    g->adj = adj.v ? adj.v : (int32_t *)calloc(2, sizeof(int32_t));
    g->adj_clause = adjc.v ? adjc.v : (int32_t *)calloc(1, sizeof(int32_t));
    if (g->n_tree_clauses == 0 && g->n_lin == 0 && g->n_or2 == 0 && g->n_adj > 0) {
      int32_t dmin = g->adj[1], dmax = g->adj[1];
      for (int32_t i = 0; i < g->n_adj; i++) {
        if (g->adj[2 * i + 1] < dmin) dmin = g->adj[2 * i + 1];
        if (g->adj[2 * i + 1] > dmax) dmax = g->adj[2 * i + 1];
      }
      int obits = 1, dbits = 1;
      while ((1 << obits) < m->n_vars) obits++;
      while (((int64_t)1 << dbits) <= (int64_t)dmax - (int64_t)dmin) dbits++;
      const int width = obits + dbits <= 16 ? 2 : (obits + dbits <= 32 ? 4 : 0);
      if (width != 0) {
        g->packed_width = width;
        g->packed_obits = obits;
        g->packed_dmin = dmin;
        g->adj_packed = malloc((size_t)g->n_adj * (size_t)width);
        for (int32_t i = 0; i < g->n_adj; i++) {
          uint32_t e = (uint32_t)g->adj[2 * i] | ((uint32_t)(g->adj[2 * i + 1] - dmin) << obits);
          if (width == 2) ((uint16_t *)g->adj_packed)[i] = (uint16_t)e;
          else ((uint32_t *)g->adj_packed)[i] = e;
        }
      }
    }
  } else {
    g->adj = (int32_t *)calloc(2, sizeof(int32_t));
  }
  if (with_lists && g->n_tree_clauses == 0 && g->n_lin == 0 && g->n_or2 == 0 && g->n_ne > 0) {
    const int32_t n = m->n_vars;
    int32_t *cnt = (int32_t *)calloc((size_t)n + 1, sizeof(int32_t));
    int64_t dmin64 = 0, dmax64 = 0;
    int first = 1;
    for (int32_t c = 0; c < g->n_clauses; c++) {
      const int32_t *rec = &g->clause[4 * c];
      if (rec[0] != CS_CL_NE) continue;
      cnt[rec[1] + 1]++;
      cnt[rec[2] + 1]++;
      const int64_t da = (int64_t)rec[3] + m->dom[rec[2]].lo, db = (int64_t)-rec[3] + m->dom[rec[1]].lo;
      if (first) { dmin64 = dmax64 = da; first = 0; }
      if (da < dmin64) dmin64 = da;
      if (db < dmin64) dmin64 = db;
      if (da > dmax64) dmax64 = da;
      if (db > dmax64) dmax64 = db;
    }
    const int32_t dmin = (int32_t)dmin64, dmax = (int32_t)dmax64;
    for (int32_t v = 0; v < n; v++) cnt[v + 1] += cnt[v];
    int obits = 1, dbits = 1;
    while ((1 << obits) < n) obits++;
    while (((int64_t)1 << dbits) <= (int64_t)dmax - (int64_t)dmin) dbits++;
    const int width = obits + dbits <= 16 ? 2 : (obits + dbits <= 32 ? 4 : 0);
    if (width != 0) {
      g->sym_n_adj = cnt[n];
      g->sym_width = width;
      g->sym_obits = obits;
      g->sym_dmin = dmin;
      g->sym_off = (int32_t *)malloc(((size_t)n + 1) * sizeof(int32_t));
      memcpy(g->sym_off, cnt, ((size_t)n + 1) * sizeof(int32_t));
      g->sym_packed = malloc((size_t)(cnt[n] ? cnt[n] : 1) * (size_t)width);
      int32_t *fill = (int32_t *)malloc(((size_t)n + 1) * sizeof(int32_t));
      memcpy(fill, cnt, ((size_t)n + 1) * sizeof(int32_t));
      for (int32_t c = 0; c < g->n_clauses; c++) {
        const int32_t *rec = &g->clause[4 * c];
        if (rec[0] != CS_CL_NE) continue;
        const uint32_t ea = (uint32_t)rec[2] | ((uint32_t)(rec[3] + m->dom[rec[2]].lo - dmin) << obits);
        const uint32_t eb = (uint32_t)rec[1] | ((uint32_t)(-rec[3] + m->dom[rec[1]].lo - dmin) << obits);
        const int32_t ia = fill[rec[1]]++, ib = fill[rec[2]]++;
        if (width == 2) { ((uint16_t *)g->sym_packed)[ia] = (uint16_t)ea; ((uint16_t *)g->sym_packed)[ib] = (uint16_t)eb; }
        else { ((uint32_t *)g->sym_packed)[ia] = ea; ((uint32_t *)g->sym_packed)[ib] = eb; }
      }
      free(fill);
    }
    free(cnt);
    if (width != 0 && n <= 256) {
      const int32_t cols = cs_dense_strides(n) * 64;
      uint8_t *mult = (uint8_t *)calloc((size_t)n * (size_t)n, 1);
      int slots = 0, ok = 1;
      for (int32_t c = 0; c < g->n_clauses && ok; c++) {
        const int32_t *rec = &g->clause[4 * c];
        if (rec[0] != CS_CL_NE) continue;
        if (rec[1] == rec[2]) { ok = 0; break; }
        const int k = ++mult[(size_t)rec[1] * n + rec[2]];
        mult[(size_t)rec[2] * n + rec[1]] = (uint8_t)k;
        if (k > slots) slots = k;
        if (k >= 32) ok = 0;
      }
      int64_t cmax = 0;
      for (int32_t v = 0; v < n; v++) if (m->dom[v].hi > cmax) cmax = m->dom[v].hi;
      const int64_t span = (cmax - dmin64 > dmax64 - dmin64 ? cmax - dmin64 : dmax64 - dmin64);
      const int dw = span < 255 ? 1 : (span < 65535 ? 2 : 0);
      if (ok && slots > 0 && dw != 0 && (size_t)n * slots * cols * dw <= 144u * 1024u) {
        const size_t total = (size_t)n * slots * cols;
        g->dense_width = dw;
        g->dense_slots = slots;
        g->dense_cols = cols;
        g->dense_dmin = dmin;
        g->dense_tab = malloc(total * (size_t)dw);
        memset(g->dense_tab, 0xff, total * (size_t)dw);
        memset(mult, 0, (size_t)n * (size_t)n);
        for (int32_t c = 0; c < g->n_clauses; c++) {
          const int32_t *rec = &g->clause[4 * c];
          if (rec[0] != CS_CL_NE) continue;
          const int k = mult[(size_t)rec[1] * n + rec[2]];
          mult[(size_t)rec[1] * n + rec[2]] = mult[(size_t)rec[2] * n + rec[1]] = (uint8_t)(k + 1);
          const uint32_t ea = (uint32_t)(rec[3] + m->dom[rec[2]].lo - dmin);
          const uint32_t eb = (uint32_t)(-rec[3] + m->dom[rec[1]].lo - dmin);
          const size_t ia = ((size_t)rec[1] * slots + k) * cols + rec[2];
          const size_t ib = ((size_t)rec[2] * slots + k) * cols + rec[1];
          if (dw == 1) { ((uint8_t *)g->dense_tab)[ia] = (uint8_t)ea; ((uint8_t *)g->dense_tab)[ib] = (uint8_t)eb; }
          else { ((uint16_t *)g->dense_tab)[ia] = (uint16_t)ea; ((uint16_t *)g->dense_tab)[ib] = (uint16_t)eb; }
        }
      }
      free(mult);
    }
  }
  return g;
}
```

csolve_amd/csrc/cs_device.h:

```cpp
#ifndef CS_DEVICE_H
#define CS_DEVICE_H

#include "cs_model.h"

#ifdef __cplusplus
extern "C" {
#endif

enum { CS_CL_SKIP = 0, CS_CL_NE = 1, CS_CL_TREE = 2, CS_CL_EQ = 3, CS_CL_LT = 4, CS_CL_OR2 = 5 };
enum { CS_REL_NE = 0, CS_REL_EQ = 1, CS_REL_LT = 2, CS_REL_GT = 3 };
#define CS_ADJ_VAR_MASK 0x0fffffff

static inline int cs_dense_strides(int32_t n_vars) { return n_vars <= 64 ? 1 : (n_vars <= 128 ? 2 : 4); }

#define CS_MAX_TREE_NODES 256

typedef struct cs_dev_image {
  int32_t n_vars, n_clauses;
  int32_t n_adj;
  int32_t n_ne, n_tree_clauses, n_skip;
  int32_t n_lin, n_or2;
  int32_t n_lits;
  int32_t *lit;
  int32_t max_list;
  int32_t *adj_off;
  int32_t *adj;
  int32_t *adj_clause;
  int32_t *clause;
  int32_t n_trees, n_tnodes, n_tkids, max_tree;
  int32_t *tree_off;
  int32_t *tnode;
  int32_t *tkid;
  int32_t *tree_want;
  int32_t packed_width, packed_obits, packed_dmin;
  void *adj_packed;
  int32_t sym_n_adj, sym_width, sym_obits, sym_dmin;
  int32_t *sym_off;
  void *sym_packed;
  int32_t dense_width, dense_slots, dense_cols, dense_dmin;
  void *dense_tab;
} cs_dev_image;

extern int cs_dev_linear_fast_paths;

cs_dev_image *cs_dev_image_build(const cs_model *m, int with_lists, const unsigned char *entailed, char *err,
                                 size_t errlen);
void cs_dev_image_free(cs_dev_image *img);

#ifdef __cplusplus
}
#endif
#endif
```

csolve_amd/csrc/cs_shave.hip.h:

```cpp
#ifndef CS_SHAVE_HIP_H
#define CS_SHAVE_HIP_H

#include "cs_kernels.hip.h"

#ifdef CS_SHAVE_TIMELINE
__device__ unsigned long long cs_shave_tl[3 * 65536];
#endif

__device__ __forceinline__ unsigned long long cs_bitset0(unsigned long long m, int i) {
  asm("s_bitset0_b64 %0, %1" : "+s"(m) : "s"(i));
  return m;
}

__device__ __forceinline__ int cs_inc_if_eq(int x, int f) {
  int r;
  asm("v_cmp_eq_u32 vcc, %1, %2\n\tv_addc_co_u32 %0, vcc, 0, %1, vcc" : "=v"(r) : "v"(x), "v"(f) : "vcc");
  return r;
}
__device__ __forceinline__ int cs_dec_if_eq(int x, int f) {
  int r;
  asm("v_cmp_eq_u32 vcc, %1, %2\n\tv_subb_co_u32 %0, vcc, %1, 0, vcc" : "=v"(r) : "v"(x), "v"(f) : "vcc");
  return r;
}

template <int L>
__device__ __forceinline__ int cs_writelane(int v, int x) {
  x = __builtin_amdgcn_readfirstlane(x);
  asm("v_writelane_b32 %0, %1, %2" : "+v"(v) : "s"(x), "n"(L));
  return v;
}

__device__ __forceinline__ int cs_writelane_at(int lane, int v, int x) {
  switch (lane) {
  case 0: return cs_writelane<0>(v, x);
  case 1: return cs_writelane<1>(v, x);
  case 2: return cs_writelane<2>(v, x);
  default: return cs_writelane<3>(v, x);
  }
}

#define CS_SHAVE_TRACE_LDS 2048u
#define CS_SHAVE_CHUNK 2
#define CS_SHAVE_SHARDS 64
#define CS_SHAVE_TICKET_STRIDE 16

template <typename E, int R, int SL, bool TRACE>
struct cs_shave_core {
  typedef unsigned long long u64;
  static constexpr int W = CS_WAVE * R;
  const E *s_tab;
  int slots, lane;
  int kb[R], deg[R], b0[R];
  u64 livemask[R];
  int4 *s_trace;
  unsigned tcount;

  __device__ __forceinline__ void trace_lanes(u64 mask, int r2, int kind, int value, int cause) {
    if (mask == 0ull) return;
    const unsigned at = tcount + __builtin_amdgcn_mbcnt_hi((unsigned)(mask >> 32), __builtin_amdgcn_mbcnt_lo((unsigned)mask, 0u));
    if (__builtin_amdgcn_inverse_ballot_w64(mask) && at < CS_SHAVE_TRACE_LDS)
      s_trace[at] = make_int4(lane + r2 * CS_WAVE, kind, value + b0[r2], cause);
    tcount += (unsigned)__builtin_popcountll(mask);
  }

  __device__ __forceinline__ void push_var(int r, int ul, int cd, int (&rlo)[R], int (&rhi)[R], u64 (&dl)[R], u64 (&dh)[R],
                                           int &revisions) {
    revisions += __builtin_amdgcn_readlane(deg[r], ul);
    const E *row = s_tab + (size_t)(ul + r * CS_WAVE) * slots * W + lane;
    int plo[R], phi[R];
#pragma unroll
    for (int r2 = 0; r2 < R; r2++) { plo[r2] = rlo[r2]; phi[r2] = rhi[r2]; }
    if (SL != 0) {
#pragma unroll
      for (int k = 0; k < (SL ? SL : 1); k++) {
#pragma unroll
        for (int r2 = 0; r2 < R; r2++) {
          const int f = cd - (int)row[k * W + r2 * CS_WAVE];
          rlo[r2] = cs_inc_if_eq(rlo[r2], f);
          rhi[r2] = cs_dec_if_eq(rhi[r2], f);
        }
      }
    } else {
      for (int k = 0; k < slots; k++) {
#pragma unroll
        for (int r2 = 0; r2 < R; r2++) {
          const int f = cd - (int)row[k * W + r2 * CS_WAVE];
          rlo[r2] = cs_inc_if_eq(rlo[r2], f);
          rhi[r2] = cs_dec_if_eq(rhi[r2], f);
        }
      }
    }
#pragma unroll
    for (int r2 = 0; r2 < R; r2++) {
      const u64 ml = __ballot(rlo[r2] != plo[r2]), mh = __ballot(rhi[r2] != phi[r2]);
      dl[r2] |= ml;
      dh[r2] |= mh;
      if (TRACE) {
        trace_lanes(ml, r2, 0, rlo[r2], ul + r * CS_WAVE);
        trace_lanes(mh, r2, 1, rhi[r2], ul + r * CS_WAVE);
      }
    }
  }

  __device__ __forceinline__ int settle(const int (&rlo)[R], const int (&rhi)[R], u64 (&val)[R]) const {
    int bad = -1;
#pragma unroll
    for (int r = R - 1; r >= 0; r--) {
      const u64 c = __ballot(rlo[r] > rhi[r]);
      if (c != 0ull) bad = __builtin_ctzll(c) + r * CS_WAVE;
      val[r] = __ballot(rlo[r] == rhi[r]) & livemask[r];
    }
    return bad;
  }

  __device__ __forceinline__ int fixpoint(int (&rlo)[R], int (&rhi)[R], u64 (&pushed)[R], u64 (&push)[R], u64 (&dl)[R],
                                          u64 (&dh)[R], u64 (&val)[R], int &rounds, int &revisions) {
    int fail_v = -1;
    for (;;) {
      int cdv[R];
#pragma unroll
      for (int r = 0; r < R; r++) cdv[r] = rlo[r] + kb[r];
#pragma unroll
      for (int r = 0; r < R; r++) {
        u64 bits = push[r];
        pushed[r] |= bits;
        while (bits != 0ull) {
          const int ul = __builtin_ctzll(bits);
          bits = cs_bitset0(bits, ul);
          push_var(r, ul, __builtin_amdgcn_readlane(cdv[r], ul), rlo, rhi, dl, dh, revisions);
        }
      }
      fail_v = settle(rlo, rhi, val);
      if (fail_v >= 0) return fail_v;
      for (;;) {
        int n_dirty = 0, n_val = 0;
#pragma unroll
        for (int r = 0; r < R; r++) { n_dirty += __popcll(dl[r] | dh[r]); n_val += __popcll(val[r]); }
        if (n_dirty <= n_val) break;
#pragma unroll
        for (int r = 0; r < R; r++) { cdv[r] = rlo[r] + kb[r]; dl[r] = 0ull; dh[r] = 0ull; }
#pragma unroll
        for (int r = 0; r < R; r++) {
          u64 bits = val[r];
          pushed[r] |= bits;
          while (bits != 0ull) {
            const int ul = __builtin_ctzll(bits);
            bits = cs_bitset0(bits, ul);
            push_var(r, ul, __builtin_amdgcn_readlane(cdv[r], ul), rlo, rhi, dl, dh, revisions);
          }
        }
        fail_v = settle(rlo, rhi, val);
        if (fail_v >= 0) return fail_v;
      }
#pragma unroll
      for (int side = 0; side < 2; side++) {
#pragma unroll
        for (int r = 0; r < R; r++) {
          u64 bits = side == 0 ? dl[r] : dh[r];
          if (side == 0) dl[r] = 0ull; else dh[r] = 0ull;
          while (bits != 0ull) {
            const int wl = __builtin_ctzll(bits);
            bits = cs_bitset0(bits, wl);
            int cand = __builtin_amdgcn_readlane(side == 0 ? rlo[r] : rhi[r], wl);
            const int ckw = cand + __builtin_amdgcn_readlane(kb[r], wl);
            revisions += __builtin_amdgcn_readlane(deg[r], wl);
            const E *row = s_tab + (size_t)(wl + r * CS_WAVE) * slots * W + lane;
            u64 hit = 0ull;
            if (SL != 0) {
              int e[SL ? SL : 1][R];
#pragma unroll
              for (int k = 0; k < (SL ? SL : 1); k++)
#pragma unroll
                for (int r2 = 0; r2 < R; r2++) e[k][r2] = (int)row[k * W + r2 * CS_WAVE];
              int cause = -1;
#pragma unroll
              for (int r2 = 0; r2 < R; r2++) {
                const int t = ckw - rlo[r2];
                u64 h = 0ull;
#pragma unroll
                for (int k = 0; k < (SL ? SL : 1); k++) h |= __ballot(e[k][r2] == t);
                hit |= h & val[r2];
                if (TRACE && cause < 0 && (h & val[r2]) != 0ull) cause = __builtin_ctzll(h & val[r2]) + r2 * CS_WAVE;
              }
              if (hit == 0ull) continue;
              const int other = __builtin_amdgcn_readlane(side == 0 ? rhi[r] : rlo[r], wl);
              int step = 0;
              for (;;) {
                step++;
                if (side == 0 ? cand + step > other : cand - step < other) break;
                hit = 0ull;
#pragma unroll
                for (int r2 = 0; r2 < R; r2++) {
                  const int t = ckw + (side == 0 ? step : -step) - rlo[r2];
                  u64 h = 0ull;
#pragma unroll
                  for (int k = 0; k < (SL ? SL : 1); k++) h |= __ballot(e[k][r2] == t);
                  hit |= h & val[r2];
                }
                if (hit == 0ull) break;
              }
              cand += side == 0 ? step : -step;
              if (lane == wl) { if (side == 0) rlo[r] = cand; else rhi[r] = cand; }
              if (TRACE) trace_lanes(1ull << wl, r, side, cand, cause);
              if (side == 0 ? cand > other : cand < other) fail_v = wl + r * CS_WAVE;
              if (cand == other) val[r] |= 1ull << wl;
            } else {
              const int other = __builtin_amdgcn_readlane(side == 0 ? rhi[r] : rlo[r], wl);
              int step = 0;
              int cause = -1;
              for (;;) {
                hit = 0ull;
                for (int k = 0; k < slots; k++) {
#pragma unroll
                  for (int r2 = 0; r2 < R; r2++) {
                    const u64 h = __ballot((int)row[k * W + r2 * CS_WAVE] == ckw + (side == 0 ? step : -step) - rlo[r2]) & val[r2];
                    hit |= h;
                    if (TRACE && cause < 0 && h != 0ull) cause = __builtin_ctzll(h) + r2 * CS_WAVE;
                  }
                }
                if (hit == 0ull) break;
                step++;
                if (side == 0 ? cand + step > other : cand - step < other) break;
              }
              if (step != 0) {
                cand += side == 0 ? step : -step;
                if (lane == wl) { if (side == 0) rlo[r] = cand; else rhi[r] = cand; }
                if (TRACE) trace_lanes(1ull << wl, r, side, cand, cause);
                if (side == 0 ? cand > other : cand < other) fail_v = wl + r * CS_WAVE;
                if (cand == other) val[r] |= 1ull << wl;
              }
            }
          }
        }
      }
      if (fail_v >= 0) return fail_v;
      u64 any_push = 0ull;
#pragma unroll
      for (int r = 0; r < R; r++) {
        push[r] = val[r] & ~pushed[r];
        any_push |= push[r];
      }
      if (any_push == 0ull) return -1;
      if (rounds == 0) __builtin_amdgcn_s_setprio(3);
      rounds++;
    }
  }
};

template <typename E, int R, int SL, bool FULL, bool TRACE = false>
__global__ __launch_bounds__(1024, (R <= 2 ? 8 : 4)) void cs_propagate_ne_shave(
    int n, const E *__restrict__ tab_g, int slots, int dmin, const int *__restrict__ root_lo,
    const int *__restrict__ sym_off, const cs_val *__restrict__ states_in, const cs_node_in *__restrict__ nodes,
    cs_val *__restrict__ states_out, cs_node_out *__restrict__ results, long long batch,
    const unsigned long long *__restrict__ batch_dev, int csz , unsigned *tickets,
    int4 *__restrict__ trace, unsigned *__restrict__ trace_n, unsigned trace_cap) {
  extern __shared__ __attribute__((aligned(16))) unsigned char cs_lds[];
  typedef unsigned long long u64;
  constexpr int W = CS_WAVE * R;
  constexpr int D = R == 1 && !TRACE ? 2 * CS_SHAVE_CHUNK : CS_SHAVE_CHUNK;
  if (batch_dev != nullptr && (long long)*batch_dev < batch) batch = (long long)*batch_dev;
  const int nbatch = __builtin_amdgcn_readfirstlane((int)batch);
  const int lane = threadIdx.x & (CS_WAVE - 1);
  const int wave_in_block = __builtin_amdgcn_readfirstlane(threadIdx.x >> 6);
  const int waves_per_block = blockDim.x >> 6;
  const int chunks = (nbatch + csz - 1) / csz;
  const int nsh = (int)gridDim.x < CS_SHAVE_SHARDS ? (int)gridDim.x : CS_SHAVE_SHARDS;
  const int shard = (int)(blockIdx.x % nsh);
  const int count_x = chunks > shard ? (chunks - 1 - shard) / nsh + 1 : 0;
  const int waves_x = (((int)gridDim.x - 1 - shard) / nsh + 1) * waves_per_block;
  const int wave_local = (int)(blockIdx.x / nsh) * waves_per_block + wave_in_block;
  const bool dynamic = tickets != nullptr && count_x > waves_x;
  if ((int)(blockIdx.x / nsh) * waves_per_block >= count_x) return;
  if (SL != 0) slots = SL;
  const E *s_tab = (const E *)cs_lds;
  int4 *s_trace = (int4 *)(cs_lds + ((((size_t)n * slots * W * sizeof(E)) + 15) & ~(size_t)15));
  {
    const int vecs = (int)(((size_t)n * slots * W * sizeof(E)) / 16);
    const uint4 *src = (const uint4 *)tab_g;
    uint4 *dst = (uint4 *)cs_lds;
    for (int i = threadIdx.x; i < vecs; i += blockDim.x) dst[i] = src[i];
  }
#ifdef CS_SHAVE_TIMELINE
  const unsigned long long tl_start = __builtin_amdgcn_s_memrealtime();
  unsigned long long tl_nodes = 0;
#endif
  __syncthreads();
  if (wave_local >= count_x) return;

  int b0[R], kb[R], deg[R], vcl[R];
  bool live[R];
#pragma unroll
  for (int r = 0; r < R; r++) {
    const int v = lane + r * CS_WAVE;
    live[r] = FULL || v < n;
    vcl[r] = live[r] ? v : n - 1;
    b0[r] = live[r] ? root_lo[vcl[r]] : 0;
    kb[r] = b0[r] - dmin;
    deg[r] = live[r] ? sym_off[vcl[r] + 1] - sym_off[vcl[r]] : 0;
  }
  u64 livemask[R];
#pragma unroll
  for (int r = 0; r < R; r++) livemask[r] = FULL ? ~0ull : __ballot(live[r]);
  cs_shave_core<E, R, SL, TRACE> C;
  C.s_tab = s_tab; C.slots = slots; C.lane = lane; C.s_trace = s_trace; C.tcount = 0u;
#pragma unroll
  for (int r = 0; r < R; r++) { C.kb[r] = kb[r]; C.deg[r] = deg[r]; C.b0[r] = b0[r]; C.livemask[r] = livemask[r]; }
  unsigned *my_ticket = tickets + (size_t)shard * CS_SHAVE_TICKET_STRIDE;

  auto load_rec = [&](int i) {
    cs_node_in rec;
    rec.var = -1; rec.lo = 0; rec.hi = 0; rec.parent = 0;
    const int node = (i * nsh + shard) * csz + lane;
    if (lane < csz && node < nbatch) rec = nodes[node];
    return rec;
  };
  auto next_index = [&](int i_prev, unsigned tk_v) -> int {
    if (!dynamic) return i_prev + waves_x;
    const int t = __builtin_amdgcn_readfirstlane((int)tk_v);
    if (t == count_x - 1 && lane == 0) __hip_atomic_store(my_ticket, 0u, __ATOMIC_RELAXED, __HIP_MEMORY_SCOPE_AGENT);
    return waves_x + t;
  };
  auto draw = [&]() -> unsigned {
    unsigned tk_v = 0;
    if (lane == 0) tk_v = __hip_atomic_fetch_add(my_ticket, 1u, __ATOMIC_RELAXED, __HIP_MEMORY_SCOPE_AGENT);
    return tk_v;
  };

  int i_cur = wave_local;
  cs_node_in rec_cur = load_rec(i_cur);
  unsigned tk = dynamic ? draw() : 0u;
  cs_val pd[D][R];
#pragma unroll
  for (int d = 0; d < D; d++) {
    const size_t prow = (size_t)__builtin_amdgcn_readlane(rec_cur.parent, d) * n;
#pragma unroll
    for (int r = 0; r < R; r++) pd[d][r] = states_in[prow + vcl[r]];
  }
  int i_next = next_index(i_cur, tk);
  int have_next = i_next < count_x;
  cs_node_in rec_next = load_rec(have_next ? i_next : i_cur);

  for (;;) {
    i_cur = __builtin_amdgcn_readfirstlane(i_cur);
    i_next = __builtin_amdgcn_readfirstlane(i_next);
    have_next = i_next < count_x;
    if (have_next && dynamic) tk = draw();
    cs_val pn[D][R];
#pragma unroll
    for (int d = 0; d < D; d++)
#pragma unroll
      for (int r = 0; r < R; r++) pn[d][r] = pd[d][r];
    if (have_next) {
#pragma unroll
      for (int d = 0; d < D; d++) {
        const size_t prow = (size_t)__builtin_amdgcn_readlane(rec_next.parent, d) * n;
#pragma unroll
        for (int r = 0; r < R; r++) pn[d][r] = states_in[prow + vcl[r]];
      }
    }
    const int base = (i_cur * nsh + shard) * csz;
    const int cnt = nbatch - base < csz ? nbatch - base : csz;
#ifdef CS_SHAVE_TIMELINE
    tl_nodes += cnt;
#endif
    cs_node_out my_result;
    my_result.status = 0; my_result.props = 0; my_result.revisions = 0; my_result.rounds = 0;
#pragma unroll
    for (int dd = 0; dd < D; dd++) {
      const int j = dd;
      if (j >= cnt) continue;
      const int nvar = __builtin_amdgcn_readlane(rec_cur.var, j);
      const int nlo = __builtin_amdgcn_readlane(rec_cur.lo, j), nhi = __builtin_amdgcn_readlane(rec_cur.hi, j);
      int rlo[R], rhi[R];
#pragma unroll
      for (int r = 0; r < R; r++) {
        rlo[r] = live[r] ? pd[dd][r].lo - b0[r] : 0;
        rhi[r] = live[r] ? pd[dd][r].hi - b0[r] : 0;
      }

      u64 pushed[R], push[R], dl[R], dh[R];
#pragma unroll
      for (int r = 0; r < R; r++) {
        pushed[r] = nvar < 0 ? ~livemask[r] : __ballot(rlo[r] == rhi[r]);
        dl[r] = 0ull; dh[r] = 0ull;
      }
#pragma unroll
      for (int r = 0; r < R; r++) {
        if (nvar >= 0 && (nvar >> 6) == r) {
          const u64 bit = 1ull << (nvar & 63);
          if (lane == (nvar & 63)) { rlo[r] = nlo - b0[r]; rhi[r] = nhi - b0[r]; }
          pushed[r] &= ~bit;
          if (nlo != nhi) { dl[r] |= bit; dh[r] |= bit; }
        }
      }
      int lo0[R], hi0[R];
#pragma unroll
      for (int r = 0; r < R; r++) { lo0[r] = rlo[r]; hi0[r] = rhi[r]; }
      u64 val[R];
#pragma unroll
      for (int r = 0; r < R; r++) {
        val[r] = __ballot(rlo[r] == rhi[r]) & livemask[r];
        push[r] = val[r] & ~pushed[r];
      }

      C.tcount = 0u;
      int rounds = 0, revisions = 0;
      const int fail_var = C.fixpoint(rlo, rhi, pushed, push, dl, dh, val, rounds, revisions);
      const int failed = fail_var >= 0;
      if (TRACE) {
        const unsigned keep = C.tcount < CS_SHAVE_TRACE_LDS ? C.tcount : CS_SHAVE_TRACE_LDS;
        for (unsigned i = lane; i < keep && i < trace_cap; i += CS_WAVE) trace[i] = s_trace[i];
        if (lane == 0) *trace_n = C.tcount;
      }
      if (rounds != 0) __builtin_amdgcn_s_setprio(0);

      int open_vars = 0, shaved = 0;
#pragma unroll
      for (int r = 0; r < R; r++) {
        open_vars += __popcll(__ballot(rlo[r] != rhi[r]));
        shaved += (rlo[r] - lo0[r]) + (hi0[r] - rhi[r]);
      }
      const int props = cs_wave_sum(shaved);
      const size_t orow = (size_t)(unsigned)(base + j) * (unsigned)n;
#ifndef CS_SHAVE_STORE_FAILED
#define CS_SHAVE_STORE_FAILED 0
#endif
      if (FULL && (CS_SHAVE_STORE_FAILED || !failed)) {
#pragma unroll
        for (int r = 0; r < R; r++) states_out[orow + lane + r * CS_WAVE] = cs_interval(rlo[r] + b0[r], rhi[r] + b0[r]);
      } else if (!FULL && !failed) {
#pragma unroll
        for (int r = 0; r < R; r++)
          if (live[r]) states_out[orow + lane + r * CS_WAVE] = cs_interval(rlo[r] + b0[r], rhi[r] + b0[r]);
      }
      my_result.status = cs_writelane_at(dd, my_result.status, failed ? -1 : open_vars);
      my_result.props = cs_writelane_at(dd, my_result.props, props);
      my_result.revisions = cs_writelane_at(dd, my_result.revisions, revisions);
      my_result.rounds = cs_writelane_at(dd, my_result.rounds, failed ? fail_var : rounds);
    }
    if (lane < cnt) results[base + lane] = my_result;

    if (!have_next) break;
    const int i_nn = next_index(i_next, tk);
    const int have_nn = i_nn < count_x;
    i_cur = i_next;
    rec_cur = rec_next;
#pragma unroll
    for (int d = 0; d < D; d++)
#pragma unroll
      for (int r = 0; r < R; r++) pd[d][r] = pn[d][r];
    rec_next = load_rec(have_nn ? i_nn : i_next);
    i_next = i_nn;
    have_next = have_nn;
  }
#ifdef CS_SHAVE_TIMELINE
  if (lane == 0) {
    const size_t w = ((size_t)blockIdx.x * (blockDim.x >> 6) + (threadIdx.x >> 6)) % 65536;
    cs_shave_tl[3 * w] = tl_start;
    cs_shave_tl[3 * w + 1] = __builtin_amdgcn_s_memrealtime();
    cs_shave_tl[3 * w + 2] = tl_nodes;
  }
#endif
}

struct cs_mailbox_head {
  unsigned req_seq; unsigned pad0[15];
  unsigned ack_seq; unsigned alive; unsigned pad1[14];
  unsigned stop; unsigned pad2[15];
  cs_node_in node; unsigned want_trace; unsigned pad3[11];
  cs_node_out result; unsigned trace_n; unsigned pad4[11];
};

template <typename E, int R, int SL>
__global__ __launch_bounds__(1024) void cs_shave_server(int n, const E *__restrict__ tab_g, int slots, int dmin,
                                                        const int *__restrict__ root_lo, const int *__restrict__ sym_off,
                                                        cs_mailbox_head *box, unsigned long long *state_in ,
                                                        unsigned long long *state_out , int4 *trace ,
                                                        unsigned trace_cap, unsigned long long idle_ticks) {
  extern __shared__ __attribute__((aligned(16))) unsigned char cs_lds[];
  typedef unsigned long long u64;
  constexpr int W = CS_WAVE * R;
  const int lane = threadIdx.x & (CS_WAVE - 1);
  if (SL != 0) slots = SL;
  {
    const int vecs = (int)(((size_t)n * slots * W * sizeof(E)) / 16);
    const uint4 *src = (const uint4 *)tab_g;
    uint4 *dst = (uint4 *)cs_lds;
    for (int i = threadIdx.x; i < vecs; i += blockDim.x) dst[i] = src[i];
  }
  int4 *s_trace = (int4 *)(cs_lds + ((((size_t)n * slots * W * sizeof(E)) + 15) & ~(size_t)15));
  __syncthreads();
  if (threadIdx.x >= CS_WAVE) return;

  cs_shave_core<E, R, SL, true> C;
  C.s_tab = (const E *)cs_lds; C.slots = slots; C.lane = lane; C.s_trace = s_trace; C.tcount = 0u;
  int b0[R];
  bool live[R];
#pragma unroll
  for (int r = 0; r < R; r++) {
    const int v = lane + r * CS_WAVE;
    live[r] = v < n;
    const int vc = live[r] ? v : n - 1;
    b0[r] = live[r] ? root_lo[vc] : 0;
    C.b0[r] = b0[r];
    C.kb[r] = b0[r] - dmin;
    C.deg[r] = live[r] ? sym_off[vc + 1] - sym_off[vc] : 0;
    C.livemask[r] = __ballot(live[r]);
  }
  unsigned last = __hip_atomic_load(&box->ack_seq, __ATOMIC_RELAXED, __HIP_MEMORY_SCOPE_SYSTEM);
  if (lane == 0) __hip_atomic_store(&box->alive, 1u, __ATOMIC_RELEASE, __HIP_MEMORY_SCOPE_SYSTEM);
  u64 idle_since = __builtin_amdgcn_s_memrealtime();
  for (;;) {
    const unsigned seq = __hip_atomic_load(&box->req_seq, __ATOMIC_ACQUIRE, __HIP_MEMORY_SCOPE_SYSTEM);
    if (seq == last) {
      if (__hip_atomic_load(&box->stop, __ATOMIC_RELAXED, __HIP_MEMORY_SCOPE_SYSTEM) != 0u) break;
      if (__builtin_amdgcn_s_memrealtime() - idle_since > idle_ticks) break;
      __builtin_amdgcn_s_sleep(2);
      continue;
    }
    const int nvar = (int)__hip_atomic_load((unsigned *)&box->node.var, __ATOMIC_RELAXED, __HIP_MEMORY_SCOPE_SYSTEM);
    const int nlo = (int)__hip_atomic_load((unsigned *)&box->node.lo, __ATOMIC_RELAXED, __HIP_MEMORY_SCOPE_SYSTEM);
    const int nhi = (int)__hip_atomic_load((unsigned *)&box->node.hi, __ATOMIC_RELAXED, __HIP_MEMORY_SCOPE_SYSTEM);
    const unsigned want_trace = __hip_atomic_load(&box->want_trace, __ATOMIC_RELAXED, __HIP_MEMORY_SCOPE_SYSTEM);
    int rlo[R], rhi[R];
#pragma unroll
    for (int r = 0; r < R; r++) {
      const int v = lane + r * CS_WAVE;
      const u64 e = __hip_atomic_load(&state_in[live[r] ? v : n - 1], __ATOMIC_RELAXED, __HIP_MEMORY_SCOPE_SYSTEM);
      rlo[r] = live[r] ? (int)(unsigned)e - b0[r] : 0;
      rhi[r] = live[r] ? (int)(unsigned)(e >> 32) - b0[r] : 0;
    }
    u64 pushed[R], push[R], dl[R], dh[R], val[R];
#pragma unroll
    for (int r = 0; r < R; r++) {
      pushed[r] = nvar < 0 ? ~C.livemask[r] : __ballot(rlo[r] == rhi[r]);
      dl[r] = 0ull; dh[r] = 0ull;
    }
#pragma unroll
    for (int r = 0; r < R; r++) {
      if (nvar >= 0 && (nvar >> 6) == r) {
        const u64 bit = 1ull << (nvar & 63);
        if (lane == (nvar & 63)) { rlo[r] = nlo - b0[r]; rhi[r] = nhi - b0[r]; }
        pushed[r] &= ~bit;
        if (nlo != nhi) { dl[r] |= bit; dh[r] |= bit; }
      }
    }
    int lo0[R], hi0[R];
#pragma unroll
    for (int r = 0; r < R; r++) {
      lo0[r] = rlo[r]; hi0[r] = rhi[r];
      val[r] = __ballot(rlo[r] == rhi[r]) & C.livemask[r];
      push[r] = val[r] & ~pushed[r];
    }
    C.tcount = 0u;
    int rounds = 0, revisions = 0;
    const int fail_var = C.fixpoint(rlo, rhi, pushed, push, dl, dh, val, rounds, revisions);
    if (rounds != 0) __builtin_amdgcn_s_setprio(0);
    const int failed = fail_var >= 0;
    int open_vars = 0, shaved = 0;
#pragma unroll
    for (int r = 0; r < R; r++) {
      open_vars += __popcll(__ballot(rlo[r] != rhi[r]));
      shaved += (rlo[r] - lo0[r]) + (hi0[r] - rhi[r]);
    }
    const int props = cs_wave_sum(shaved);
    if (!failed) {
#pragma unroll
      for (int r = 0; r < R; r++)
        if (live[r]) {
          const u64 e = (u64)(unsigned)(rlo[r] + b0[r]) | ((u64)(unsigned)(rhi[r] + b0[r]) << 32);
          __hip_atomic_store(&state_out[lane + r * CS_WAVE], e, __ATOMIC_RELAXED, __HIP_MEMORY_SCOPE_SYSTEM);
        }
    }
    if (want_trace != 0u) {
      const unsigned keep = C.tcount < CS_SHAVE_TRACE_LDS ? C.tcount : CS_SHAVE_TRACE_LDS;
      for (unsigned i = lane; i < keep && i < trace_cap; i += CS_WAVE) trace[i] = s_trace[i];
    }
    if (lane == 0) {
      box->result.status = failed ? -1 : open_vars;
      box->result.props = props;
      box->result.revisions = revisions;
      box->result.rounds = failed ? fail_var : rounds;
      box->trace_n = C.tcount;
    }
    __builtin_amdgcn_fence(__ATOMIC_RELEASE, "");
    if (lane == 0) __hip_atomic_store(&box->ack_seq, seq, __ATOMIC_RELEASE, __HIP_MEMORY_SCOPE_SYSTEM);
    last = seq;
    idle_since = __builtin_amdgcn_s_memrealtime();
  }
  if (lane == 0) __hip_atomic_store(&box->alive, 0u, __ATOMIC_RELEASE, __HIP_MEMORY_SCOPE_SYSTEM);
}

#endif
```

csolve_amd/solver.py:

```python
from __future__ import annotations

import ctypes as C

import numpy as np
import torch

from ._lib import (PLAN_FAMILIES, CsolveError, ManyOptions, ManyResult, Node, Result, SearchStats, Val, check, demangle,
                   load_library)

STATUS_FAIL = -1


def _stream_ptr(stream) -> int:
    if stream is None:
        stream = torch.cuda.current_stream()
    return int(stream.cuda_stream)


class Model:

    def __init__(self, handle):
        self._h = handle
        self.finalized = False

    @classmethod
    def from_text(cls, text: str, weights_on: bool = True) -> "Model":
        L = load_library()
        h = C.c_void_p()
        check(L.csgpu_model_from_text(text.encode(), int(weights_on), C.byref(h)))
        return cls(h)

    @classmethod
    def from_file(cls, path: str, weights_on: bool = True) -> "Model":
        L = load_library()
        h = C.c_void_p()
        check(L.csgpu_model_from_file(path.encode(), int(weights_on), C.byref(h)))
        return cls(h)

    @classmethod
    def from_dump(cls, path: str) -> "Model":
        L = load_library()
        h = C.c_void_p()
        check(L.csgpu_model_from_dump(path.encode(), C.byref(h)))
        return cls(h)

    def close(self):
        if self._h:
            load_library().csgpu_model_free(self._h)
            self._h = None

    def __del__(self):
        try:
            self.close()
        except Exception:
            pass

    @property
    def n_vars(self) -> int:
        return check(load_library().csgpu_model_num_vars(self._h))

    @property
    def n_clauses(self) -> int:
        return check(load_library().csgpu_model_num_clauses(self._h))

    @property
    def objective(self) -> int:
        return check(load_library().csgpu_model_objective(self._h))

    @property
    def objective_var(self) -> int:
        return load_library().csgpu_model_objective_var(self._h)

    def var_names(self):
        L = load_library()
        return [L.csgpu_model_var_name(self._h, i).decode() for i in range(self.n_vars)]

    def domains(self) -> np.ndarray:
        out = np.empty((self.n_vars, 2), dtype=np.int32)
        check(load_library().csgpu_model_get_domains(self._h, out.ctypes.data))
        return out

    def set_domains(self, dom: np.ndarray):
        dom = np.ascontiguousarray(dom, dtype=np.int32)
        assert dom.shape == (self.n_vars, 2)
        check(load_library().csgpu_model_set_domains(self._h, dom.ctypes.data))

    def device_info(self) -> dict:
        info = (C.c_int64 * 8)()
        check(load_library().csgpu_model_device_info(self._h, info))
        keys = ("adjacency_entries", "ne_clauses", "tree_clauses", "tree_nodes", "lds_bytes_per_node",
                "max_list", "skipped_clauses", "max_tree")
        return dict(zip(keys, [int(x) for x in info]))

    def root_propagate(self) -> int:
        st = C.c_int32()
        check(load_library().csgpu_model_root_propagate(self._h, C.byref(st)))
        return st.value

    def eval_clauses_host(self) -> np.ndarray:
        out = np.empty((max(1, self.n_clauses), 2), dtype=np.int32)
        check(load_library().csgpu_model_eval_clauses_host(self._h, out.ctypes.data))
        return out[: self.n_clauses]

    def build_tables(self):
        check(load_library().csgpu_model_build_tables(self._h))
        return self

    def normalize(self):
        check(load_library().csgpu_model_normalize(self._h))
        return self

    def specialize(self, state, build_only: bool = False) -> "Model":
        state = np.ascontiguousarray(np.asarray(state.cpu() if hasattr(state, "cpu") else state), dtype=np.int32)
        state = state.reshape(-1, self.n_vars, 2)
        assert state.shape[0] == 1, "one state (a common prefix), not a batch"
        state = np.ascontiguousarray(state[0])
        h = C.c_void_p()
        check(load_library().csgpu_model_specialize(self._h, state.ctypes.data, C.byref(h)))
        m = Model(h)
        m.normalize()
        if build_only:
            return m.build_tables()
        if m.root_propagate() < 0:
            raise ValueError("INFEASIBLE PROBLEM")
        return m.finalize()

    def add_conflict(self, elems):
        vs = np.ascontiguousarray([e[0] for e in elems], dtype=np.int32)
        cs = np.ascontiguousarray([e[1] for e in elems], dtype=np.int32)
        check(load_library().csgpu_model_add_conflict(self._h, len(elems), vs.ctypes.data, cs.ctypes.data))
        return self

    def finalize(self):
        check(load_library().csgpu_model_finalize(self._h))
        self.finalized = True
        return self

    def set_kernel(self, which: int):
        check(load_library().csgpu_model_set_kernel(self._h, which))
        return self

    def qualifies(self, which: int) -> bool:
        return bool(load_library().csgpu_model_qualifies(self._h, which))

    def plan(self) -> dict:
        buf = C.create_string_buffer(1024)
        out = {}
        for i, fam in enumerate(PLAN_FAMILIES):
            check(load_library().csgpu_internal_plan_symbol(self._h, i, buf, len(buf)))
            out[fam] = demangle(buf.value.decode()) if buf.value else None
        return out

    def kernel(self) -> int:
        return check(load_library().csgpu_model_get_kernel(self._h))

    def root_state(self, device="cuda") -> torch.Tensor:
        return torch.from_numpy(self.domains()).to(device).unsqueeze(0).contiguous()

    def propagate(self, states_in: torch.Tensor, nodes: torch.Tensor, states_out: torch.Tensor = None,
                  results: torch.Tensor = None, stream=None):
        n = self.n_vars
        assert states_in.is_cuda and nodes.is_cuda, "device tensors required"
        assert states_in.dtype == torch.int32 and nodes.dtype == torch.int32
        assert states_in.is_contiguous() and nodes.is_contiguous()
        assert states_in.shape[-2:] == (n, 2) and nodes.shape[-1] == 4
        B = nodes.shape[0]
        if states_out is None:
            states_out = torch.empty((B, n, 2), dtype=torch.int32, device=nodes.device)
        if results is None:
            results = torch.empty((B, 4), dtype=torch.int32, device=nodes.device)
        assert states_out.is_contiguous() and results.is_contiguous()
        assert states_out.shape == (B, n, 2) and results.shape == (B, 4)
        check(load_library().csgpu_propagate_batch(self._h, states_in.data_ptr(), nodes.data_ptr(),
                                                   states_out.data_ptr(), results.data_ptr(), B,
                                                   _stream_ptr(stream)))
        return states_out, results

    MANY_OBJECTIVES = {"ANY": 0, "ALL": 1, "MIN": 2, "MAX": 3}

    def solve_many(self, roots, objective="ANY", *, max_nodes, solutions=True, stream=None) -> dict:
        L = load_library()
        n = self.n_vars
        obj = self.MANY_OBJECTIVES[objective] if isinstance(objective, str) else int(objective)
        opt = ManyOptions(obj, 0, int(max_nodes))
        if not torch.is_tensor(roots):
            roots = np.ascontiguousarray(roots, dtype=np.int32)
            assert roots.ndim == 3 and roots.shape[1:] == (n, 2), "roots is [K, n_vars, 2]"
            if not self.qualifies(7):
                check(L.csgpu_solve_many(self._h, roots.ctypes.data, roots.shape[0], C.byref(opt), roots.ctypes.data,
                                         None, None))
            roots = torch.from_numpy(roots).cuda()
        assert roots.is_cuda and roots.dtype == torch.int32 and roots.is_contiguous()
        assert roots.dim() == 3 and tuple(roots.shape[1:]) == (n, 2), "roots is [K, n_vars, 2]"
        K = roots.shape[0]
        buf = torch.zeros((max(K, 1), 5), dtype=torch.int64, device=roots.device)
        res = buf[:K]
        first = torch.zeros((K, n), dtype=torch.int32, device=roots.device) if solutions else None
        check(L.csgpu_solve_many(self._h, roots.data_ptr() if K else buf.data_ptr(), K, C.byref(opt), buf.data_ptr(),
                                 first.data_ptr() if solutions and K else None, _stream_ptr(stream)))
        head = res.view(torch.int32)
        out = {"status": head[:, 0], "root_props": head[:, 1], "nodes": res[:, 1], "cuts": res[:, 2], "props": res[:, 3],
               "solutions": res[:, 4]}
        if solutions:
            out["first"] = first
        return out

    def many_kernel(self):
        buf = C.create_string_buffer(1024)
        check(load_library().csgpu_internal_many_symbol(self._h, buf, len(buf)))
        return demangle(buf.value.decode()) if buf.value else None

    def many_waves(self, count: int) -> int:
        return int(load_library().csgpu_internal_many_waves(self._h, int(count)))

    def forbidden_words(self) -> int:
        return load_library().csgpu_model_forbidden_words(self._h)

    def propagate_fb(self, states_in, nodes, forb_in=None, states_out=None, forb_out=None, results=None,
                     want_forb=True, stream=None):
        n, fw = self.n_vars, self.forbidden_words()
        assert fw > 0, "model does not qualify for the forbidden-set kernel"
        assert states_in.is_cuda and states_in.dtype == torch.int32 and states_in.is_contiguous()
        assert nodes.is_cuda and nodes.dtype == torch.int32 and nodes.is_contiguous()
        B = nodes.shape[0]
        if states_out is None:
            states_out = torch.empty((B, n, 2), dtype=torch.int32, device=nodes.device)
        if results is None:
            results = torch.empty((B, 4), dtype=torch.int32, device=nodes.device)
        if forb_out is None and want_forb:
            forb_out = torch.empty((B, n, fw), dtype=torch.int64, device=nodes.device)
        if forb_in is not None:
            assert forb_in.dtype == torch.int64 and forb_in.is_contiguous() and forb_in.shape[-2:] == (n, fw)
            assert forb_in.shape[0] == states_in.shape[0]
        check(load_library().csgpu_propagate_batch_fb(
            self._h, states_in.data_ptr(), 0 if forb_in is None else forb_in.data_ptr(), nodes.data_ptr(),
            states_out.data_ptr(), 0 if forb_out is None else forb_out.data_ptr(), results.data_ptr(), B,
            _stream_ptr(stream)))
        return states_out, forb_out, results

    def pack_sets(self, states: torch.Tensor, stream=None) -> torch.Tensor:
        n, fw = self.n_vars, self.forbidden_words()
        assert states.is_cuda and states.dtype == torch.int32 and states.is_contiguous() and states.shape[-2:] == (n, 2)
        sets = torch.empty((states.shape[0], n, fw), dtype=torch.int64, device=states.device)
        check(load_library().csgpu_sets_pack(self._h, states.data_ptr(), sets.data_ptr(), states.shape[0], _stream_ptr(stream)))
        return sets
# ... 232 lines not shown
```

include/csolve_gpu.h:

```cpp
#ifndef CSOLVE_GPU_H
#define CSOLVE_GPU_H

#include <stddef.h>
#include <stdint.h>

#ifdef __cplusplus
extern "C" {
#endif

#define CSGPU_OK 0
#define CSGPU_E_ARG (-1)
#define CSGPU_E_PARSE (-2)
#define CSGPU_E_HIP (-3)
#define CSGPU_E_LIMIT (-4)
#define CSGPU_E_STATE (-5)
#define CSGPU_E_UNBOUNDED (-6)

typedef struct csgpu_val {
  int32_t lo, hi;
} csgpu_val;

typedef struct csgpu_node {
  int32_t var, lo, hi, parent;
} csgpu_node;

typedef struct csgpu_result {
  int32_t status, props, revisions, rounds;
} csgpu_result;

typedef struct csgpu_model csgpu_model;

const char *csgpu_last_error(void);
int csgpu_device_count(void);
int csgpu_set_device(int device);

int csgpu_model_from_text(const char *text, int weights_on, csgpu_model **out);
int csgpu_model_from_file(const char *path, int weights_on, csgpu_model **out);
int csgpu_model_from_dump(const char *path, csgpu_model **out);
void csgpu_model_free(csgpu_model *m);

int csgpu_model_num_vars(const csgpu_model *m);
int csgpu_model_num_clauses(const csgpu_model *m);
int csgpu_model_objective(const csgpu_model *m);
int csgpu_model_objective_var(const csgpu_model *m);
const char *csgpu_model_var_name(const csgpu_model *m, int var);
int csgpu_model_get_domains(const csgpu_model *m, csgpu_val *out);
int csgpu_model_set_domains(csgpu_model *m, const csgpu_val *in);
int csgpu_model_device_info(const csgpu_model *m, int64_t info[8]);

int csgpu_model_root_propagate(csgpu_model *m, int32_t *status);
int csgpu_model_root_propagate_limit(csgpu_model *m, int64_t limit, int32_t *status, int32_t *rounds);

int csgpu_model_normalize(csgpu_model *m);
int csgpu_model_specialize(const csgpu_model *m, const csgpu_val *state, csgpu_model **out);
int csgpu_model_add_conflict(csgpu_model *m, int32_t count, const int32_t *vars, const int32_t *values);

int csgpu_model_eval_clauses_host(csgpu_model *m, csgpu_val *vals);

int csgpu_model_build_tables(csgpu_model *m);

int csgpu_model_finalize(csgpu_model *m);

int csgpu_sets_pack(const csgpu_model *m, const csgpu_val *d_states, uint64_t *d_sets, int64_t count, void *stream);
int csgpu_sets_unpack(const csgpu_model *m, const uint64_t *d_sets, csgpu_val *d_states, int64_t count, void *stream);
int csgpu_propagate_batch_sets(const csgpu_model *m, const uint64_t *d_sets_in, const csgpu_node *d_nodes,
                               uint64_t *d_sets_out, csgpu_result *d_results, int64_t batch, void *stream);

int csgpu_model_set_kernel(csgpu_model *m, int which);
void csgpu_set_linear_fast_paths(int on);
int csgpu_model_qualifies(const csgpu_model *m, int which);
int csgpu_model_get_kernel(const csgpu_model *m);

int csgpu_propagate_batch(const csgpu_model *m, const csgpu_val *d_states_in, const csgpu_node *d_nodes,
                          csgpu_val *d_states_out, csgpu_result *d_results, int64_t batch, void *stream);

int csgpu_propagate_batch_obj(const csgpu_model *m, const csgpu_val *d_states_in, const csgpu_node *d_nodes,
                              csgpu_val *d_states_out, csgpu_result *d_results, int64_t batch, int32_t obj_lo,
                              int32_t obj_hi, void *stream);

int csgpu_model_forbidden_words(const csgpu_model *m);
int csgpu_propagate_batch_fb(const csgpu_model *m, const csgpu_val *d_states_in, const uint64_t *d_forb_in,
                             const csgpu_node *d_nodes, csgpu_val *d_states_out, uint64_t *d_forb_out,
                             csgpu_result *d_results, int64_t batch, void *stream);

#define CSGPU_MANY_DONE 0
#define CSGPU_MANY_LIMIT 1
#define CSGPU_MANY_BAD_ROOT 2
typedef struct csgpu_many_result {
  int32_t status, root_props;
  int64_t nodes, cuts, props, solutions;
} csgpu_many_result;
typedef struct csgpu_many_options {
  int32_t objective;
  int32_t reserved;
  int64_t max_nodes;
} csgpu_many_options;
int csgpu_solve_many(const csgpu_model *m, const csgpu_val *d_roots, int64_t count, const csgpu_many_options *options,
                     csgpu_many_result *d_results, int32_t *d_solutions, void *stream);

int csgpu_eval_batch(const csgpu_model *m, const csgpu_val *d_states, int32_t *d_truth, int64_t batch,
                     void *stream);

int csgpu_eval_clauses(const csgpu_model *m, const csgpu_val *d_state, csgpu_val *d_vals, void *stream);

typedef struct csgpu_search csgpu_search;

typedef struct csgpu_search_stats {
  uint64_t nodes;
  uint64_t cuts;
  uint64_t props;
  uint64_t revisions;
  uint64_t solutions;
  uint64_t iterations;
  uint64_t restarts;
  int64_t pool;
  int64_t pool_peak;
  int32_t best;
  int32_t done;
} csgpu_search_stats;

int csgpu_search_create(const csgpu_model *m, int64_t pool_capacity, int64_t max_children, csgpu_search **out);
void csgpu_search_free(csgpu_search *s);
int csgpu_search_reset(csgpu_search *s);
int csgpu_search_put(csgpu_search *s, const csgpu_val *d_states, int64_t count);
int csgpu_search_put_host(csgpu_search *s, const csgpu_val *states, int64_t count);
int csgpu_search_take(csgpu_search *s, csgpu_val *d_states, int64_t max, int64_t *count);
int csgpu_search_take_host(csgpu_search *s, csgpu_val *states, int64_t max, int64_t *count);
int csgpu_search_set_parents(csgpu_search *s, int64_t parents_per_iteration);
int csgpu_search_set_restart(csgpu_search *s, int64_t iterations);
int csgpu_search_set_strategy(csgpu_search *s, int order, int prefer_failing);
int csgpu_search_set_restart_on_improvement(csgpu_search *s, int on);
int csgpu_search_put_cost(const csgpu_search *s, double *seconds, int64_t *states);
int csgpu_objective_better(int objective, csgpu_val value, int32_t best);
csgpu_val csgpu_objective_bound(int objective, csgpu_val value, int32_t best);
int32_t csgpu_objective_best(int objective, csgpu_val value, int32_t best);
void csgpu_luby_next(uint64_t *threshold, uint64_t *counter);
int csgpu_step_check(csgpu_val bounds, uint32_t iter);
int32_t csgpu_step_val(csgpu_val bounds, uint32_t iter, uint32_t seed);
uint64_t csgpu_branch_key(int order, int prefer_failing, csgpu_val value, int64_t prio, int32_t index);

int csgpu_search_set_best(csgpu_search *s, int32_t best);
int csgpu_search_share_incumbent(csgpu_search *s, csgpu_search *with);
int csgpu_search_run(csgpu_search *s, int64_t max_iterations, csgpu_search_stats *stats);
int64_t csgpu_search_solutions(const csgpu_search *s, int32_t *values, int64_t max);

int csgpu_search_set_solution_stream(csgpu_search *s, int64_t rows);
int csgpu_search_drain_solutions(csgpu_search *s, int32_t *values, int64_t max, int64_t *count);
int csgpu_search_drain_solutions_device(csgpu_search *s, int32_t *d_values, int64_t max, int64_t *count, void *stream);
int csgpu_search_pending_solutions(const csgpu_search *s, int64_t *rows, int64_t *room);

int csgpu_search_best_solution(const csgpu_search *s, int32_t *values);

int csgpu_plan_transfers(const int64_t *pools, int world, int64_t low_water, int64_t max_give, int64_t *plan,
                         int *count);
#define CSGPU_SHARD_MAX_WORLD 8
int csgpu_shard_region_size(int world, int n_vars, int64_t inbox_rows, size_t *bytes);
int csgpu_shard_region_init(void *region, size_t bytes, int world, int n_vars, int64_t inbox_rows);
int csgpu_shard_barrier(void *region);
int csgpu_text_num_vars(const char *text, int weights_on, int *n_vars);

typedef void (*csgpu_shard_solution_fn)(void *user, int rank, const int32_t *rows, int64_t count, int32_t best);

typedef struct csgpu_shard_options {
  int64_t slice_iterations;
  int64_t poll_iterations;
  int64_t seed_states_per_rank;
  int64_t low_water;
  double time_limit;
  csgpu_shard_solution_fn on_solution;
  void *user;
} csgpu_shard_options;
void csgpu_shard_default_options(csgpu_shard_options *options);

int csgpu_shard_run(csgpu_search *s, void *region, int rank, const csgpu_val *root, const csgpu_shard_options *options,
                    csgpu_search_stats *local, csgpu_search_stats *totals);

int csgpu_propagate_values(const csgpu_model *m, const csgpu_val *state, int32_t var, const int32_t *values,
                           int32_t count, csgpu_val *states_out, csgpu_result *results);

int csgpu_propagate_one(const csgpu_model *m, const csgpu_val *state, csgpu_node node, csgpu_val *state_out,
                        csgpu_result *result);
int csgpu_propagate_one_traced(const csgpu_model *m, const csgpu_val *state, csgpu_node node, csgpu_val *state_out,
                               csgpu_result *result, int32_t *trace, int32_t cap, int32_t *count);
int csgpu_propagate_one_causes(const csgpu_model *m, const csgpu_val *state, csgpu_node node, csgpu_val *state_out,
                               csgpu_result *result, int32_t *trace, int32_t cap, int32_t *count);
int csgpu_propagate_one_chain(const csgpu_model *m, const csgpu_val *state, csgpu_node node, int32_t *status,
                              int32_t *props, int32_t *bumps, int32_t cap, int32_t *count);
int csgpu_debug_one_timing(const csgpu_model *m, double *seconds, uint64_t *calls, uint64_t *starts);

#ifdef __cplusplus
}
#endif
#endif
```

Baseline: 21.04 billion.

## Replace dense pair table lookups with offset-clique potential keys in shave kernel

```diff
diff --git a/csolve_amd/_lib.py b/csolve_amd/_lib.py
--- a/csolve_amd/_lib.py
+++ b/csolve_amd/_lib.py
@@ -125,6 +125,8 @@
     L.csgpu_model_get_domains.argtypes = [vp, vp]
     L.csgpu_model_set_domains.argtypes = [vp, vp]
     L.csgpu_model_device_info.argtypes = [vp, C.POINTER(i64)]
+    if hasattr(L, "csgpu_model_offset_clique"):
+        L.csgpu_model_offset_clique.argtypes = [vp, C.POINTER(i64), vp, i64]
     L.csgpu_model_root_propagate.argtypes = [vp, C.POINTER(i32)]
     L.csgpu_model_finalize.argtypes = [vp]
     L.csgpu_model_normalize.argtypes = [vp]
diff --git a/csolve_amd/csrc/cs_capi.hip b/csolve_amd/csrc/cs_capi.hip
--- a/csolve_amd/csrc/cs_capi.hip
+++ b/csolve_amd/csrc/cs_capi.hip
@@ -85,6 +85,7 @@
   int lds_adj_global;
   int k2_csz;
   int shave_static;
+  int *d_dense_pot;
   int step_chunk_max;
   size_t k1_tab_bytes;
   int fb_words;
@@ -271,6 +272,8 @@
   (void)hipFree(m->d_sym_off);
   (void)hipFree(m->d_sym_packed);
   (void)hipFree(m->d_dense_tab);
+  (void)hipFree(m->d_dense_pot);
+  m->d_dense_pot = NULL;
   (void)hipFree(m->d_packed_tab);
   m->d_packed_tab = NULL;
   (void)hipFree(m->d_tickets);
@@ -348,6 +351,19 @@
   info[5] = m->img->max_list;
   info[6] = m->img->n_skip;
   info[7] = m->img->max_tree;
+  return CSGPU_OK;
+}
+
+extern "C" int csgpu_model_offset_clique(const csgpu_model *m, int64_t info[2], int32_t *potentials, int64_t cap) {
+  if (m == NULL || info == NULL) return set_err(CSGPU_E_ARG, "null argument");
+  if (m->img == NULL) return set_err(CSGPU_E_STATE, "device tables are not built");
+  const int64_t count = m->img->dense_pot != NULL ? (int64_t)m->img->dense_slots * m->img->dense_cols : 0;
+  info[0] = count ? m->img->dense_slots : 0;
+  info[1] = m->d_dense_pot != NULL;
+  if (potentials != NULL && count != 0) {
+    if (cap < count) return set_err(CSGPU_E_LIMIT, "%lld potentials, room for %lld", (long long)count, (long long)cap);
+    memcpy(potentials, m->img->dense_pot, (size_t)count * sizeof(int32_t));
+  }
   return CSGPU_OK;
 }
 
@@ -995,6 +1011,10 @@
   HIP_TRY(hipMemset(m->d_tickets, 0, (size_t)CS_TICKET_SLOTS * CS_TICKET_SLOT_WORDS * sizeof(unsigned)));
   m->ticket_slots = CS_TICKET_SLOTS;
   m->shave_static = getenv("CSGPU_SHAVE_STATIC") != NULL;
+  if (m->img->dense_pot != NULL && CS_SHAVE_KEYS(slots == 1 || slots == 3 ? slots : 0, cs_dense_strides(n)) &&
+      getenv("CSGPU_SHAVE_TABLE") == NULL &&
+      (rc = upload(m->img->dense_pot, (size_t)slots * m->img->dense_cols * sizeof(int32_t), &m->d_dense_pot)))
+    return rc;
   return CSGPU_OK;
 }
 
@@ -1368,11 +1388,12 @@
   const int *root_lo_d = m->d_root_lo, *sym_off = m->d_sym_off;
   long long nb_d = (long long)batch;
   unsigned *tickets = m->shave_static ? NULL : ticket_slot((csgpu_model *)m, stream);
+  const int *pot_d = m->d_dense_pot;
   int4 *no_trace = NULL;
   unsigned *no_trace_n = NULL;
   unsigned no_trace_cap = 0u;
   void *args[] = { &n, &tab_d, &slots, &dmin_d, &root_lo_d, &sym_off, &d_states_in, &d_nodes, &d_states_out, &d_results,
-                   &nb_d, &d_batch, &csz, &tickets, &no_trace, &no_trace_n, &no_trace_cap };
+                   &nb_d, &d_batch, &csz, &tickets, &no_trace, &no_trace_n, &no_trace_cap, &pot_d };
   HIP_TRY(hipLaunchKernel(k->fn, dim3((unsigned)g), dim3((unsigned)(k->waves * CS_WAVE)), args, k->lds, (hipStream_t)stream));
   return CSGPU_OK;
 }
@@ -1839,7 +1860,8 @@
   unsigned cap = CS_SHAVE_TRACE_LDS;
   unsigned long long idle = 200000ull;
   { const char *e = getenv("CSGPU_SERVER_IDLE_US"); if (e != NULL && atoll(e) > 0) idle = (unsigned long long)atoll(e) * 100ull; }
-  void *args[] = { &n, &tab_d, &slots, &dmin_d, &root_lo_d, &sym_off, &d_box, &d_in, &d_out, &d_trace, &cap, &idle };
+  const int *pot_d = m->d_dense_pot;
+  void *args[] = { &n, &tab_d, &slots, &dmin_d, &root_lo_d, &sym_off, &d_box, &d_in, &d_out, &d_trace, &cap, &idle, &pot_d };
   const cs_planned *k = &m->plan.server;
   HIP_TRY(hipLaunchKernel(k->fn, dim3(1), dim3((unsigned)(k->waves * CS_WAVE)), args, k->lds, m->srv_stream));
   m->srv_launched = 1;
@@ -1968,12 +1990,13 @@
   long long nb_d = 1;
   const uint64_t *d_batch = NULL;
   unsigned *tickets = NULL;
+  const int *pot_d = m->d_dense_pot;
   const csgpu_val *d_in = (const csgpu_val *)m->d_one_in;
   const csgpu_node *d_node = (const csgpu_node *)m->d_one_node;
   csgpu_val *d_out = (csgpu_val *)m->d_one_out;
   csgpu_result *d_res = (csgpu_result *)m->d_one_res;
   void *args[] = { &n, &tab_d, &slots, &dmin_d, &root_lo_d, &sym_off, &d_in, &d_node, &d_out, &d_res,
-                   &nb_d, &d_batch, &csz, &tickets, &d_trace, &d_trace_n, &ucap };
+                   &nb_d, &d_batch, &csz, &tickets, &d_trace, &d_trace_n, &ucap, &pot_d };
   const cs_planned *k = &m->plan.shave_trace;
   if (k->fn == NULL) return set_err(CSGPU_E_LIMIT, "no room in LDS for the trail next to the pair table");
   const double tl1 = srv_now();
diff --git a/csolve_amd/csrc/cs_device.c b/csolve_amd/csrc/cs_device.c
--- a/csolve_amd/csrc/cs_device.c
+++ b/csolve_amd/csrc/cs_device.c
@@ -163,8 +163,35 @@
 
 void cs_dev_image_free(cs_dev_image *g) {
   if (g == NULL) return;
-  free(g->adj_off); free(g->adj); free(g->adj_clause); free(g->clause); free(g->tree_off); free(g->tnode); free(g->tkid); free(g->tree_want); free(g->lit); free(g->adj_packed); free(g->sym_off); free(g->sym_packed); free(g->dense_tab);
+  free(g->adj_off); free(g->adj); free(g->adj_clause); free(g->clause); free(g->tree_off); free(g->tnode); free(g->tkid); free(g->tree_want); free(g->lit); free(g->adj_packed); free(g->sym_off); free(g->sym_packed); free(g->dense_tab); free(g->dense_pot);
   free(g);
+}
+
+static int32_t *dense_potentials(const cs_dev_image *g, const cs_model *m) {
+  const int32_t n = g->n_vars, slots = g->dense_slots, cols = g->dense_cols;
+  if (n < 2) return NULL;
+  const uint32_t sentinel = g->dense_width == 1 ? 0xffu : 0xffffu;
+  int32_t *pot = (int32_t *)calloc((size_t)slots * cols, sizeof(int32_t));
+  int ok = 1;
+  for (int pass = 0; pass < 2 && ok; pass++)
+    for (int32_t u = 0; u < (pass == 0 ? 1 : n) && ok; u++)
+      for (int32_t k = 0; k < slots && ok; k++)
+        for (int32_t w = 0; w < n; w++) {
+          if (w == u) continue;
+          const size_t i = ((size_t)u * slots + k) * cols + w;
+          const uint32_t e = g->dense_width == 1 ? ((const uint8_t *)g->dense_tab)[i] : ((const uint16_t *)g->dense_tab)[i];
+          if (e == sentinel) { ok = 0; break; }
+          const int32_t d = (int32_t)e - m->dom[w].lo + g->dense_dmin;
+          if (pass == 0) pot[(size_t)k * cols + w] = d;
+          else if (d != pot[(size_t)k * cols + w] - pot[(size_t)k * cols + u]) { ok = 0; break; }
+        }
+  for (int32_t v = 0; v < n && ok; v++) {
+    if (m->dom[v].lo <= -(1 << 28) || m->dom[v].hi >= (1 << 28)) ok = 0;
+    for (int32_t k = 0; k < slots; k++)
+      if (pot[(size_t)k * cols + v] <= -(1 << 28) || pot[(size_t)k * cols + v] >= (1 << 28)) ok = 0;
+  }
+  if (!ok) { free(pot); return NULL; }
+  return pot;
 }
 
 cs_dev_image *cs_dev_image_build(const cs_model *m, int with_lists, const unsigned char *entailed, char *err,
@@ -398,6 +425,7 @@
           if (dw == 1) { ((uint8_t *)g->dense_tab)[ia] = (uint8_t)ea; ((uint8_t *)g->dense_tab)[ib] = (uint8_t)eb; }
           else { ((uint16_t *)g->dense_tab)[ia] = (uint16_t)ea; ((uint16_t *)g->dense_tab)[ib] = (uint16_t)eb; }
         }
+        g->dense_pot = dense_potentials(g, m);
       }
       free(mult);
     }
diff --git a/csolve_amd/csrc/cs_device.h b/csolve_amd/csrc/cs_device.h
--- a/csolve_amd/csrc/cs_device.h
+++ b/csolve_amd/csrc/cs_device.h
@@ -39,6 +39,7 @@
   void *sym_packed;
   int32_t dense_width, dense_slots, dense_cols, dense_dmin;
   void *dense_tab;
+  int32_t *dense_pot;
 } cs_dev_image;
 
 extern int cs_dev_linear_fast_paths;
diff --git a/csolve_amd/csrc/cs_shave.hip.h b/csolve_amd/csrc/cs_shave.hip.h
--- a/csolve_amd/csrc/cs_shave.hip.h
+++ b/csolve_amd/csrc/cs_shave.hip.h
@@ -21,6 +21,27 @@
   int r;
   asm("v_cmp_eq_u32 vcc, %1, %2\n\tv_subb_co_u32 %0, vcc, %1, 0, vcc" : "=v"(r) : "v"(x), "v"(f) : "vcc");
   return r;
+}
+
+__device__ __forceinline__ int cs_sadd(int a, int b) {
+  int r;
+  asm("s_add_i32 %0, %1, %2" : "=s"(r) : "s"(a), "s"(b) : "scc");
+  return r;
+}
+
+__device__ __forceinline__ int cs_sle(int a, int b) {
+  int r;
+  asm("s_cmp_le_i32 %1, %2\n\ts_cselect_b32 %0, 1, 0" : "=s"(r) : "s"(a), "s"(b) : "scc");
+  return r;
+}
+
+#define CS_SHAVE_OFF(f) "v_cmp_eq_u32 vcc, %0, " f "\n\tv_addc_co_u32 %0, vcc, 0, %0, vcc\n\tv_cmp_eq_u32 vcc, %1, " f "\n\tv_subb_co_u32 %1, vcc, %1, 0, vcc\n\t"
+__device__ __forceinline__ void cs_shave_off_except(int &lo, int &hi, const int (&f)[1], int ul) {
+  asm("s_bitset0_b64 exec, %3\n\t" CS_SHAVE_OFF("%2") "s_bitset1_b64 exec, %3" : "+v"(lo), "+v"(hi) : "v"(f[0]), "s"(ul) : "vcc");
+}
+__device__ __forceinline__ void cs_shave_off_except(int &lo, int &hi, const int (&f)[3], int ul) {
+  asm("s_bitset0_b64 exec, %5\n\t" CS_SHAVE_OFF("%2") CS_SHAVE_OFF("%3") CS_SHAVE_OFF("%4") "s_bitset1_b64 exec, %5"
+      : "+v"(lo), "+v"(hi) : "v"(f[0]), "v"(f[1]), "v"(f[2]), "s"(ul) : "vcc");
 }
 
 template <int L>
@@ -43,6 +64,10 @@
 #define CS_SHAVE_CHUNK 2
 #define CS_SHAVE_SHARDS 64
 #define CS_SHAVE_TICKET_STRIDE 16
+#define CS_SHAVE_KEYS(SL, R) ((SL) != 0 && (R) <= 2)
+#define CS_SHAVE_NO_KEY (-(1 << 30))
+
+template <bool KEY> struct cs_shave_form { static constexpr bool value = KEY; };
 
 template <typename E, int R, int SL, bool TRACE>
 struct cs_shave_core {
@@ -52,6 +77,9 @@
   int slots, lane;
   int kb[R], deg[R], b0[R];
   u64 livemask[R];
+  static constexpr int SLK = SL ? SL : 1;
+  int pk[SLK][R];
+  int degu;
   int4 *s_trace;
   unsigned tcount;
 
@@ -102,6 +130,41 @@
     }
   }
 
+  __device__ __forceinline__ void push_key(int r, int ul, int cd, int (&rlo)[R], int (&rhi)[R], u64 (&dl)[R], u64 (&dh)[R],
+                                           int &revisions) {
+    revisions += degu;
+    int s[SLK];
+#pragma unroll
+    for (int k = 0; k < SLK; k++) s[k] = cs_sadd(cd, __builtin_amdgcn_readlane(pk[k][r], ul));
+    int plo[R], phi[R];
+#pragma unroll
+    for (int r2 = 0; r2 < R; r2++) { plo[r2] = rlo[r2]; phi[r2] = rhi[r2]; }
+#pragma unroll
+    for (int r2 = 0; r2 < R; r2++) {
+      int f[SLK];
+#pragma unroll
+      for (int k = 0; k < SLK; k++) f[k] = s[k] - pk[k][r2];
+      if (r2 == r) cs_shave_off_except(rlo[r2], rhi[r2], f, ul);
+      else {
+#pragma unroll
+        for (int k = 0; k < SLK; k++) {
+          rlo[r2] = cs_inc_if_eq(rlo[r2], f[k]);
+          rhi[r2] = cs_dec_if_eq(rhi[r2], f[k]);
+        }
+      }
+    }
+#pragma unroll
+    for (int r2 = 0; r2 < R; r2++) {
+      const u64 ml = __ballot(rlo[r2] != plo[r2]), mh = __ballot(rhi[r2] != phi[r2]);
+      dl[r2] |= ml;
+      dh[r2] |= mh;
+      if (TRACE) {
+        trace_lanes(ml, r2, 0, rlo[r2], ul + r * CS_WAVE);
+        trace_lanes(mh, r2, 1, rhi[r2], ul + r * CS_WAVE);
+      }
+    }
+  }
+
   __device__ __forceinline__ int settle(const int (&rlo)[R], const int (&rhi)[R], u64 (&val)[R]) const {
     int bad = -1;
 #pragma unroll
@@ -113,13 +176,15 @@
     return bad;
   }
 
+  template <bool KEY_ = false>
   __device__ __forceinline__ int fixpoint(int (&rlo)[R], int (&rhi)[R], u64 (&pushed)[R], u64 (&push)[R], u64 (&dl)[R],
                                           u64 (&dh)[R], u64 (&val)[R], int &rounds, int &revisions) {
+    constexpr bool KEY = KEY_ && CS_SHAVE_KEYS(SL, R);
     int fail_v = -1;
     for (;;) {
       int cdv[R];
 #pragma unroll
-      for (int r = 0; r < R; r++) cdv[r] = rlo[r] + kb[r];
+      for (int r = 0; r < R; r++) cdv[r] = KEY ? rlo[r] : rlo[r] + kb[r];
 #pragma unroll
       for (int r = 0; r < R; r++) {
         u64 bits = push[r];
@@ -127,7 +192,8 @@
         while (bits != 0ull) {
           const int ul = __builtin_ctzll(bits);
           bits = cs_bitset0(bits, ul);
-          push_var(r, ul, __builtin_amdgcn_readlane(cdv[r], ul), rlo, rhi, dl, dh, revisions);
+          if (KEY) push_key(r, ul, __builtin_amdgcn_readlane(cdv[r], ul), rlo, rhi, dl, dh, revisions);
+          else push_var(r, ul, __builtin_amdgcn_readlane(cdv[r], ul), rlo, rhi, dl, dh, revisions);
         }
       }
       fail_v = settle(rlo, rhi, val);
@@ -136,9 +202,9 @@
         int n_dirty = 0, n_val = 0;
 #pragma unroll
         for (int r = 0; r < R; r++) { n_dirty += __popcll(dl[r] | dh[r]); n_val += __popcll(val[r]); }
-        if (n_dirty <= n_val) break;
-#pragma unroll
-        for (int r = 0; r < R; r++) { cdv[r] = rlo[r] + kb[r]; dl[r] = 0ull; dh[r] = 0ull; }
+        if (cs_sle(n_dirty, n_val)) break;
+#pragma unroll
+        for (int r = 0; r < R; r++) { cdv[r] = KEY ? rlo[r] : rlo[r] + kb[r]; dl[r] = 0ull; dh[r] = 0ull; }
 #pragma unroll
         for (int r = 0; r < R; r++) {
           u64 bits = val[r];
@@ -146,7 +212,8 @@
           while (bits != 0ull) {
             const int ul = __builtin_ctzll(bits);
             bits = cs_bitset0(bits, ul);
-            push_var(r, ul, __builtin_amdgcn_readlane(cdv[r], ul), rlo, rhi, dl, dh, revisions);
+            if (KEY) push_key(r, ul, __builtin_amdgcn_readlane(cdv[r], ul), rlo, rhi, dl, dh, revisions);
+            else push_var(r, ul, __builtin_amdgcn_readlane(cdv[r], ul), rlo, rhi, dl, dh, revisions);
           }
         }
         fail_v = settle(rlo, rhi, val);
@@ -154,6 +221,18 @@
       }
 #pragma unroll
       for (int side = 0; side < 2; side++) {
+        int key[SLK][R];
+        if (KEY) {
+          u64 any = 0ull;
+#pragma unroll
+          for (int r = 0; r < R; r++) any |= side == 0 ? dl[r] : dh[r];
+          if (any != 0ull) {
+#pragma unroll
+            for (int r = 0; r < R; r++)
+#pragma unroll
+              for (int k = 0; k < SLK; k++) key[k][r] = (side == 0 ? rlo[r] : rhi[r]) + pk[k][r];
+          }
+        }
 #pragma unroll
         for (int r = 0; r < R; r++) {
           u64 bits = side == 0 ? dl[r] : dh[r];
@@ -161,6 +240,48 @@
           while (bits != 0ull) {
             const int wl = __builtin_ctzll(bits);
             bits = cs_bitset0(bits, wl);
+            if (KEY) {
+              revisions += degu;
+              int s[SLK];
+#pragma unroll
+              for (int k = 0; k < SLK; k++) s[k] = __builtin_amdgcn_readlane(key[k][r], wl);
+              u64 vm[R], hit = 0ull;
+              int cause = -1;
+#pragma unroll
+              for (int r2 = 0; r2 < R; r2++) {
+                vm[r2] = r2 == r ? cs_bitset0(val[r2], wl) : val[r2];
+                u64 h = 0ull;
+#pragma unroll
+                for (int k = 0; k < SLK; k++) h |= __ballot(key[k][r2] == s[k]);
+                hit |= h & vm[r2];
+                if (TRACE && cause < 0 && (h & vm[r2]) != 0ull) cause = __builtin_ctzll(h & vm[r2]) + r2 * CS_WAVE;
+              }
+              if (hit == 0ull) continue;
+              int cand = __builtin_amdgcn_readlane(side == 0 ? rlo[r] : rhi[r], wl);
+              const int other = __builtin_amdgcn_readlane(side == 0 ? rhi[r] : rlo[r], wl);
+              int step = 0;
+              for (;;) {
+                step++;
+                if (side == 0 ? cand + step > other : cand - step < other) break;
+                hit = 0ull;
+#pragma unroll
+                for (int r2 = 0; r2 < R; r2++) {
+                  u64 h = 0ull;
+#pragma unroll
+                  for (int k = 0; k < SLK; k++) h |= __ballot(key[k][r2] == s[k] + (side == 0 ? step : -step));
+                  hit |= h & vm[r2];
+                }
+                if (hit == 0ull) break;
+              }
+              cand += side == 0 ? step : -step;
+              if (lane == wl) { if (side == 0) rlo[r] = cand; else rhi[r] = cand; }
+              if (TRACE) trace_lanes(1ull << wl, r, side, cand, cause);
+              if (side == 0 ? cand > other : cand < other) fail_v = wl + r * CS_WAVE;
+              if (cand == other) val[r] |= 1ull << wl;
+#pragma unroll
+              for (int k = 0; k < SLK; k++) key[k][r] = (side == 0 ? rlo[r] : rhi[r]) + pk[k][r];
+              continue;
+            }
             int cand = __builtin_amdgcn_readlane(side == 0 ? rlo[r] : rhi[r], wl);
             const int ckw = cand + __builtin_amdgcn_readlane(kb[r], wl);
             revisions += __builtin_amdgcn_readlane(deg[r], wl);
@@ -253,7 +374,8 @@
     const int *__restrict__ sym_off, const cs_val *__restrict__ states_in, const cs_node_in *__restrict__ nodes,
     cs_val *__restrict__ states_out, cs_node_out *__restrict__ results, long long batch,
     const unsigned long long *__restrict__ batch_dev, int csz , unsigned *tickets,
-    int4 *__restrict__ trace, unsigned *__restrict__ trace_n, unsigned trace_cap) {
+    int4 *__restrict__ trace, unsigned *__restrict__ trace_n, unsigned trace_cap,
+    const int *__restrict__ pot ) {
   extern __shared__ __attribute__((aligned(16))) unsigned char cs_lds[];
   typedef unsigned long long u64;
   constexpr int W = CS_WAVE * R;
@@ -272,9 +394,10 @@
   const bool dynamic = tickets != nullptr && count_x > waves_x;
   if ((int)(blockIdx.x / nsh) * waves_per_block >= count_x) return;
   if (SL != 0) slots = SL;
+  const bool keyed = CS_SHAVE_KEYS(SL, R) && pot != nullptr;
   const E *s_tab = (const E *)cs_lds;
   int4 *s_trace = (int4 *)(cs_lds + ((((size_t)n * slots * W * sizeof(E)) + 15) & ~(size_t)15));
-  {
+  if (!keyed) {
     const int vecs = (int)(((size_t)n * slots * W * sizeof(E)) / 16);
     const uint4 *src = (const uint4 *)tab_g;
     uint4 *dst = (uint4 *)cs_lds;
@@ -282,11 +405,15 @@
   }
 #ifdef CS_SHAVE_TIMELINE
   const unsigned long long tl_start = __builtin_amdgcn_s_memrealtime();
-  unsigned long long tl_nodes = 0;
 #endif
   __syncthreads();
   if (wave_local >= count_x) return;
 
+#ifdef CS_SHAVE_TIMELINE
+  unsigned long long tl_nodes = 0;
+#endif
+  auto run = [&](auto form) __attribute__((always_inline)) {
+  constexpr bool KEY = decltype(form)::value;
   int b0[R], kb[R], deg[R], vcl[R];
   bool live[R];
 #pragma unroll
@@ -294,9 +421,9 @@
     const int v = lane + r * CS_WAVE;
     live[r] = FULL || v < n;
     vcl[r] = live[r] ? v : n - 1;
-    b0[r] = live[r] ? root_lo[vcl[r]] : 0;
+    b0[r] = !KEY && live[r] ? root_lo[vcl[r]] : 0;
     kb[r] = b0[r] - dmin;
-    deg[r] = live[r] ? sym_off[vcl[r] + 1] - sym_off[vcl[r]] : 0;
+    deg[r] = !KEY && live[r] ? sym_off[vcl[r] + 1] - sym_off[vcl[r]] : 0;
   }
   u64 livemask[R];
 #pragma unroll
@@ -305,6 +432,11 @@
   C.s_tab = s_tab; C.slots = slots; C.lane = lane; C.s_trace = s_trace; C.tcount = 0u;
 #pragma unroll
   for (int r = 0; r < R; r++) { C.kb[r] = kb[r]; C.deg[r] = deg[r]; C.b0[r] = b0[r]; C.livemask[r] = livemask[r]; }
+  C.degu = slots * (n - 1);
+#pragma unroll
+  for (int r = 0; r < R; r++)
+#pragma unroll
+    for (int k = 0; k < (SL ? SL : 1); k++) C.pk[k][r] = KEY && live[r] ? pot[k * W + vcl[r]] : CS_SHAVE_NO_KEY;
   unsigned *my_ticket = tickets + (size_t)shard * CS_SHAVE_TICKET_STRIDE;
 
   auto load_rec = [&](int i) {
@@ -346,10 +478,6 @@
     have_next = i_next < count_x;
     if (have_next && dynamic) tk = draw();
     cs_val pn[D][R];
-#pragma unroll
-    for (int d = 0; d < D; d++)
-#pragma unroll
-      for (int r = 0; r < R; r++) pn[d][r] = pd[d][r];
     if (have_next) {
 #pragma unroll
       for (int d = 0; d < D; d++) {
@@ -393,9 +521,9 @@
           if (nlo != nhi) { dl[r] |= bit; dh[r] |= bit; }
         }
       }
-      int lo0[R], hi0[R];
-#pragma unroll
-      for (int r = 0; r < R; r++) { lo0[r] = rlo[r]; hi0[r] = rhi[r]; }
+      int w0[R];
+#pragma unroll
+      for (int r = 0; r < R; r++) w0[r] = rhi[r] - rlo[r];
       u64 val[R];
 #pragma unroll
       for (int r = 0; r < R; r++) {
@@ -405,7 +533,7 @@
 
       C.tcount = 0u;
       int rounds = 0, revisions = 0;
-      const int fail_var = C.fixpoint(rlo, rhi, pushed, push, dl, dh, val, rounds, revisions);
+      const int fail_var = C.template fixpoint<KEY>(rlo, rhi, pushed, push, dl, dh, val, rounds, revisions);
       const int failed = fail_var >= 0;
       if (TRACE) {
         const unsigned keep = C.tcount < CS_SHAVE_TRACE_LDS ? C.tcount : CS_SHAVE_TRACE_LDS;
@@ -418,7 +546,7 @@
 #pragma unroll
       for (int r = 0; r < R; r++) {
         open_vars += __popcll(__ballot(rlo[r] != rhi[r]));
-        shaved += (rlo[r] - lo0[r]) + (hi0[r] - rhi[r]);
+        shaved += w0[r] - (rhi[r] - rlo[r]);
       }
       const int props = cs_wave_sum(shaved);
       const size_t orow = (size_t)(unsigned)(base + j) * (unsigned)n;
@@ -453,6 +581,8 @@
     i_next = i_nn;
     have_next = have_nn;
   }
+  };
+  if (keyed) run(cs_shave_form<CS_SHAVE_KEYS(SL, R)>()); else run(cs_shave_form<false>());
 #ifdef CS_SHAVE_TIMELINE
   if (lane == 0) {
     const size_t w = ((size_t)blockIdx.x * (blockDim.x >> 6) + (threadIdx.x >> 6)) % 65536;
@@ -476,13 +606,15 @@
                                                         const int *__restrict__ root_lo, const int *__restrict__ sym_off,
                                                         cs_mailbox_head *box, unsigned long long *state_in ,
                                                         unsigned long long *state_out , int4 *trace ,
-                                                        unsigned trace_cap, unsigned long long idle_ticks) {
+                                                        unsigned trace_cap, unsigned long long idle_ticks,
+                                                        const int *__restrict__ pot ) {
   extern __shared__ __attribute__((aligned(16))) unsigned char cs_lds[];
   typedef unsigned long long u64;
   constexpr int W = CS_WAVE * R;
   const int lane = threadIdx.x & (CS_WAVE - 1);
   if (SL != 0) slots = SL;
-  {
+  const bool keyed = CS_SHAVE_KEYS(SL, R) && pot != nullptr;
+  if (!keyed) {
     const int vecs = (int)(((size_t)n * slots * W * sizeof(E)) / 16);
     const uint4 *src = (const uint4 *)tab_g;
     uint4 *dst = (uint4 *)cs_lds;
@@ -501,12 +633,15 @@
     const int v = lane + r * CS_WAVE;
     live[r] = v < n;
     const int vc = live[r] ? v : n - 1;
-    b0[r] = live[r] ? root_lo[vc] : 0;
+    b0[r] = !keyed && live[r] ? root_lo[vc] : 0;
     C.b0[r] = b0[r];
     C.kb[r] = b0[r] - dmin;
     C.deg[r] = live[r] ? sym_off[vc + 1] - sym_off[vc] : 0;
     C.livemask[r] = __ballot(live[r]);
-  }
+#pragma unroll
+    for (int k = 0; k < (SL ? SL : 1); k++) C.pk[k][r] = keyed && live[r] ? pot[k * W + vc] : CS_SHAVE_NO_KEY;
+  }
+  C.degu = slots * (n - 1);
   unsigned last = __hip_atomic_load(&box->ack_seq, __ATOMIC_RELAXED, __HIP_MEMORY_SCOPE_SYSTEM);
   if (lane == 0) __hip_atomic_store(&box->alive, 1u, __ATOMIC_RELEASE, __HIP_MEMORY_SCOPE_SYSTEM);
   u64 idle_since = __builtin_amdgcn_s_memrealtime();
@@ -554,7 +689,8 @@
     }
     C.tcount = 0u;
     int rounds = 0, revisions = 0;
-    const int fail_var = C.fixpoint(rlo, rhi, pushed, push, dl, dh, val, rounds, revisions);
+    const int fail_var = keyed ? C.template fixpoint<true>(rlo, rhi, pushed, push, dl, dh, val, rounds, revisions)
+                               : C.template fixpoint<false>(rlo, rhi, pushed, push, dl, dh, val, rounds, revisions);
     if (rounds != 0) __builtin_amdgcn_s_setprio(0);
     const int failed = fail_var >= 0;
     int open_vars = 0, shaved = 0;
diff --git a/csolve_amd/solver.py b/csolve_amd/solver.py
--- a/csolve_amd/solver.py
+++ b/csolve_amd/solver.py
@@ -90,7 +90,22 @@
         check(load_library().csgpu_model_device_info(self._h, info))
         keys = ("adjacency_entries", "ne_clauses", "tree_clauses", "tree_nodes", "lds_bytes_per_node",
                 "max_list", "skipped_clauses", "max_tree")
-        return dict(zip(keys, [int(x) for x in info]))
+        out = dict(zip(keys, [int(x) for x in info]))
+        clique = (C.c_int64 * 2)()
+        if hasattr(load_library(), "csgpu_model_offset_clique"):
+            check(load_library().csgpu_model_offset_clique(self._h, clique, None, 0))
+        out["offset_clique_slots"], out["shave_key_form"] = int(clique[0]), int(clique[1])
+        return out
+
+    def offset_clique_potentials(self):
+        slots = self.device_info()["offset_clique_slots"]
+        if slots == 0:
+            return None
+        cols = 64 * (1 if self.n_vars <= 64 else 2 if self.n_vars <= 128 else 4)
+        pot = np.zeros((slots, cols), dtype=np.int32)
+        clique = (C.c_int64 * 2)()
+        check(load_library().csgpu_model_offset_clique(self._h, clique, pot.ctypes.data, pot.size))
+        return pot[:, : self.n_vars]
 
     def root_propagate(self) -> int:
         st = C.c_int32()
diff --git a/include/csolve_gpu.h b/include/csolve_gpu.h
--- a/include/csolve_gpu.h
+++ b/include/csolve_gpu.h
@@ -47,6 +47,7 @@
 int csgpu_model_get_domains(const csgpu_model *m, csgpu_val *out);
 int csgpu_model_set_domains(csgpu_model *m, const csgpu_val *in);
 int csgpu_model_device_info(const csgpu_model *m, int64_t info[8]);
+int csgpu_model_offset_clique(const csgpu_model *m, int64_t info[2], int32_t *potentials, int64_t cap);
 
 int csgpu_model_root_propagate(csgpu_model *m, int32_t *status);
 int csgpu_model_root_propagate_limit(csgpu_model *m, int64_t limit, int32_t *status, int32_t *rounds);
```

After: 19.15 billion. -9.0%, worse.
